# zsc/MOSS-TTSD

Hardware: AMD Instinct MI355X
Metric: audio codec tokens/sec/node (decode, bf16, batch 32 @ 4k ctx) (higher is better)
Workload: dtype bf16; 1 GPU; configs[2]: batch 32 synthetic dialogues/GPU, 4k-token KV context, top-k/top-p sampling on 8 channels, decode steps at full context; batch_per_gpu=32, context=4096, prompt=512, layers=28, hidden=2048, parallelism=dp1 (batch shard, no per-step collective)

## Files before the change

include/mtts.h:

```cpp
#ifndef MTTS_H
#define MTTS_H

#include <stdint.h>

#ifdef __cplusplus
extern "C" {
#endif

#define MTTS_OK 0
#define MTTS_EINVAL (-1)
#define MTTS_EHIP (-2)
#define MTTS_ENOMEM (-3)
#define MTTS_ESTATE (-4)

#define MTTS_CHANNELS 8

typedef struct MttsConfig {
    int32_t vocab_size;
    int32_t hidden_size;
    int32_t intermediate_size;
    int32_t num_hidden_layers;
    int32_t num_attention_heads;
    int32_t num_key_value_heads;
    int32_t head_dim;
    int32_t channels;
    int32_t speech_vocab_size;
    int32_t speech_pad_token;
    int32_t speech_range_lo;
    int32_t speech_range_hi;
    int32_t eos_token_id;
    int32_t max_position;
    float rms_norm_eps;
    int32_t max_batch;
    int32_t max_seq_len;
    int32_t kv_pool_pages;
    int32_t dtype;
} MttsConfig;
#define MTTS_DTYPE_BF16 0
#define MTTS_DTYPE_F32 1
#define MTTS_DTYPE_F16 2

typedef struct MttsSamplerCfg {
    int32_t do_sample;
    int32_t top_k;
    float top_p;
    float one_minus_top_p;
    float temperature;
    float repetition_penalty;
} MttsSamplerCfg;

typedef struct MttsEngine MttsEngine;

const char* mtts_last_error(void);
int32_t mtts_version(void);

int32_t mtts_engine_create(const MttsConfig* cfg, int32_t device, MttsEngine** out);
int32_t mtts_engine_destroy(MttsEngine* e);

int32_t mtts_bind_weight(MttsEngine* e, const char* name, const void* dev_bf16,
                         int64_t rows, int64_t cols, void* stream);
int32_t mtts_bind_rope(MttsEngine* e, const void* dev_cos_bf16, const void* dev_sin_bf16,
                       int32_t rows, void* stream);
int32_t mtts_weights_ready(MttsEngine* e);

int32_t mtts_generate(MttsEngine* e, const int64_t* host_input_ids, const uint8_t* host_attention_mask,
                      int32_t B, int32_t T, int32_t max_length,
                      const MttsSamplerCfg* sampler, uint64_t seed,
                      int64_t* host_out_ids, int32_t out_capacity, int32_t* out_len,
                      const int64_t* host_forced, int32_t forced_len, int64_t* host_decisions,
                      void* stream);

int32_t mtts_begin(MttsEngine* e, const int64_t* host_input_ids, const uint8_t* host_attention_mask,
                   int32_t B, int32_t T, int32_t max_length,
                   const MttsSamplerCfg* sampler, uint64_t seed, void* stream);
int32_t mtts_step(MttsEngine* e, int32_t n_steps, void* stream);
int32_t mtts_sync_state(MttsEngine* e, int32_t* steps_done, int32_t* all_finished, void* stream);
int32_t mtts_read_generated(MttsEngine* e, int64_t* host_gen, int32_t capacity_steps, int32_t* n_steps);
int32_t mtts_set_output_scores(MttsEngine* e, int32_t on);
int32_t mtts_read_scores(MttsEngine* e, float* host_lp, int32_t capacity_steps, int32_t* n_steps);
int32_t mtts_slot_read_scores(MttsEngine* e, int32_t slot, float* host_rows, int32_t capacity_steps, int32_t* n_steps);
int32_t mtts_read_logits(MttsEngine* e, uint16_t* host_logits0, uint16_t* host_logits17, void* stream);
int32_t mtts_read_logits_f32(MttsEngine* e, float* host_logits0, float* host_logits17, void* stream);
int32_t mtts_sched_open(MttsEngine* e, int32_t B, int32_t gen_cap, const MttsSamplerCfg* sampler, void* stream);
int32_t mtts_slot_submit(MttsEngine* e, int32_t slot, const int64_t* host_ids, int32_t T, int32_t max_length, uint64_t seed,
                         void* stream);
int32_t mtts_slot_submit_row(MttsEngine* e, int32_t slot, const int64_t* host_ids, int32_t T, int32_t max_length, uint64_t seed,
                             int32_t row_id, void* stream);
int32_t mtts_set_row_ids(MttsEngine* e, const int32_t* host_row_ids, int32_t n);
int32_t mtts_set_takes(MttsEngine* e, int32_t n);
int32_t mtts_slot_fork(MttsEngine* e, int32_t src_slot, int32_t dst_slot, uint64_t seed, int32_t row_id, void* stream);
int32_t mtts_slot_states(MttsEngine* e, int32_t* host_state, void* stream);
int32_t mtts_slot_read(MttsEngine* e, int32_t slot, int64_t* host_rows, int32_t capacity_steps, int32_t* n_steps);
int32_t mtts_read_seq_state(MttsEngine* e, int32_t* host_nas, int32_t* host_unfinished, int32_t* host_kv_len, void* stream);
int32_t mtts_slot_evict(MttsEngine* e, int32_t slot, void* stream);
int32_t mtts_kv_pool_state(MttsEngine* e, int32_t* total_pages, int32_t* free_pages, int32_t* max_pages_per_seq);
int32_t mtts_read_page_table(MttsEngine* e, int32_t* host_table, int32_t* host_n_pages);
int32_t mtts_set_forced_mode(MttsEngine* e, int32_t as_draw);
int32_t mtts_debug_read_device_page_table(MttsEngine* e, int32_t* host_table, void* stream);
int32_t mtts_export_codes(MttsEngine* e, int32_t first, int32_t n, int64_t* dev_codes, void* stream);
int32_t mtts_profile_enable(MttsEngine* e, int32_t on);
int32_t mtts_profile_read(MttsEngine* e, int32_t which, double* total_ms, int64_t* launches, int64_t* bytes);

int32_t mtts_debug_set_kv_len(MttsEngine* e, int32_t kv_len);
int32_t mtts_debug_kv_pack_stats(MttsEngine* e, int64_t* out6);
int32_t mtts_k_attn_bench(MttsEngine* e, int32_t phase, int32_t iters, float* avg_ms, int64_t* bytes_per_launch);
int32_t mtts_k_gemm_bench(int32_t N, int32_t K, int32_t epi, int32_t ksplit, int32_t waves, int32_t copies,
                          int32_t iters, float* avg_us);

int32_t mtts_k_gemm_bf16(const void* dev_w, const void* dev_x, void* dev_y,
                         int32_t M, int32_t N, int32_t K, int32_t ksplit, void* stream);
int64_t mtts_debug_gemm_depth_launches(void);
int32_t mtts_k_gemm_swiglu_bf16(const void* dev_w, const void* dev_x, void* dev_y,
                                int32_t M, int32_t N, int32_t K, void* stream);
int32_t mtts_k_rmsnorm(const void* dev_x, const void* dev_w, void* dev_y,
                       int32_t rows, int32_t n, float eps, void* stream);
int32_t mtts_k_rope_kvwrite(const void* dev_qkv, const int32_t* host_pos, const void* dev_qnorm, const void* dev_knorm,
                            const void* dev_cos, const void* dev_sin, int32_t R, int32_t nq, int32_t nkv, float eps,
                            void* dev_q, void* dev_k, void* dev_v, void* stream);
int32_t mtts_k_paged_attn_decode(const void* dev_q, const void* dev_k, const void* dev_v, const int32_t* host_lens,
                                 const int32_t* host_page_table, int32_t R, int32_t Lmax, int32_t nq, int32_t nkv,
                                 void* dev_out, void* stream);
int32_t mtts_k_kv_seal(const void* dev_pages, int32_t npages, void* dev_sealed, int32_t as_k, void* stream);
int32_t mtts_k_sample(const void* dev_logits_bf16, int32_t rows, int32_t vocab,
                      const void* dev_history_bitmap, const MttsSamplerCfg* cfg,
                      int32_t mask_id, uint64_t seed, int32_t step, int32_t channel,
                      int32_t* dev_tokens, void* stream);
int32_t mtts_k_sample_scores(const void* dev_logits_bf16, int32_t rows, int32_t vocab,
                             const void* dev_history_bitmap, const MttsSamplerCfg* cfg,
                             int32_t mask_id, uint64_t seed, int32_t step, int32_t channel,
                             int32_t* dev_tokens, float* dev_logp, void* stream);

typedef struct MttsCodecConfig {
    int32_t nq, codebook_size, rvq_dim, quant_out_dim;
    int32_t adapter_layers, adapter_dim, adapter_heads, adapter_ffn, adapter_max_pos;
    int32_t up_stride;
    int32_t dec_layers, dec_dim, dec_heads, dec_ffn, dec_max_pos, mel_bins;
    int32_t voc_dim, voc_inter, voc_layers, n_fft, hop;
    int32_t mel_n_fft, mel_hop, mel_frames;
    int32_t enc_layers, enc_dim, enc_heads, enc_ffn, enc_max_pos;
    int32_t sem_adapter_layers, pre_rvq_layers, down_pool;
} MttsCodecConfig;

typedef struct MttsCodec MttsCodec;
const char* mtts_codec_last_error(void);
int32_t mtts_codec_create(const MttsCodecConfig* cfg, int32_t device, MttsCodec** out);
int32_t mtts_codec_destroy(MttsCodec* c);
int32_t mtts_codec_bind(MttsCodec* c, const char* role, const float* dev_f32, int64_t n, void* stream);
int32_t mtts_codec_detokenize(MttsCodec* c, const int64_t* dev_codes, const int32_t* host_lens, int32_t B, int32_t T,
                              float* dev_wav, void* stream);
int32_t mtts_codec_detokenize_async(MttsCodec* c, const int64_t* dev_codes, const int32_t* host_lens, int32_t B, int32_t T,
                                    float* dev_wav, void* stream);
int32_t mtts_codec_check(MttsCodec* c, void* stream);
int32_t mtts_codec_tokenize(MttsCodec* c, const float* dev_wav, const int32_t* host_lens, int32_t B, int32_t nsamp,
                            int64_t* dev_codes, int32_t* host_code_lens, void* stream);
int32_t mtts_k_gemm_f32(const float* dev_a, const float* dev_w, const float* dev_bias, float* dev_c,
                        int32_t M, int32_t N, int32_t K, int32_t act, void* stream);
int32_t mtts_k_gemm_planes_bench(int32_t M, int32_t N, int32_t K, int32_t flags, int32_t tile_code, int32_t iters,
                                 float* avg_us, int32_t* code_used);

#ifdef __cplusplus
}
#endif
#endif
```

moss-ttsd_amd/csrc/attn.hip:

```cpp
#include "launch.h"
#include <cstdlib>
#ifndef MTTS_PK_WAVES
#define MTTS_PK_WAVES 0
#endif
#if MTTS_PK_WAVES
#define PK_OCC(PK) __attribute__((amdgpu_waves_per_eu((PK) ? MTTS_PK_WAVES : 1, (PK) ? MTTS_PK_WAVES : 8)))
#else
#define PK_OCC(PK)
#endif

__device__ __forceinline__ uint32_t u4c(const u32x4_t& v, int c) { return c == 0 ? v.x : c == 1 ? v.y : c == 2 ? v.z : v.w; }
__device__ __forceinline__ void pk_unit(const u32x4_t* pk, int j, uint32_t w[4]) {
    const uint32_t L0 = u4c(pk[j >> 1], 2 * (j & 1)), L1 = u4c(pk[j >> 1], 2 * (j & 1) + 1);
    const uint32_t N = u4c(pk[8 + (j >> 2)], j & 3);
    const uint32_t lo = pk[12].x, hi = pk[12].y;
    const uint32_t HA = ((N & 0x08080808u) << 4) | __builtin_amdgcn_perm(hi, lo, N & 0x07070707u);
    const uint32_t HB = (N & 0x80808080u) | __builtin_amdgcn_perm(hi, lo, (N >> 4) & 0x07070707u);
    w[0] = __builtin_amdgcn_perm(HA, L0, 0x05010400u);
    w[1] = __builtin_amdgcn_perm(HA, L0, 0x07030602u);
    w[2] = __builtin_amdgcn_perm(HB, L1, 0x05010400u);
    w[3] = __builtin_amdgcn_perm(HB, L1, 0x07030602u);
}

__host__ __device__ constexpr int pk_order(int i) { return i == 0 ? 12 : (i - 1) % 3 == 0 ? 8 + (i - 1) / 3 : 2 * ((i - 1) / 3) + (i - 1) % 3 - 1; }
__device__ bool seal_encode(const u32x4_t (&v)[16], u32x4_t* __restrict__ pk, uint32_t spare, bool unfit) {
    unsigned long long b0 = 0ull, b1 = 0ull;
#pragma unroll
    for (int j = 0; j < 16; ++j)
#pragma unroll
        for (int c = 0; c < 4; ++c)
#pragma unroll
            for (int h = 0; h < 2; ++h) {
                const uint32_t e = (u4c(v[j], c) >> (8 + 16 * h)) & 0x7fu;
                if (e & 64u) b1 |= 1ull << (e & 63u);
                else b0 |= 1ull << e;
            }
    const int n0 = __popcll(b0), n = n0 + __popcll(b1);
    if (n > 8 || unfit) {
        pk[12 * 64] = u32x4_t{0u, 0u, spare, 1u};
        return false;
    }
    unsigned long long dict = 0ull;
    {
        unsigned long long t0 = b0, t1 = b1;
        for (int i = 0; i < n; ++i) {
            uint32_t e;
            if (t0) { e = __ffsll((long long)t0) - 1; t0 &= t0 - 1; }
            else { e = 64 + __ffsll((long long)t1) - 1; t1 &= t1 - 1; }
            dict |= (unsigned long long)e << (8 * i);
        }
    }
    auto code = [&](uint32_t half) -> uint32_t {
        const uint32_t e = (half >> 8) & 0x7fu;
        const uint32_t rank = (e & 64u) ? n0 + __popcll(b1 & ((1ull << (e & 63u)) - 1ull)) : __popcll(b0 & ((1ull << e) - 1ull));
        return ((half >> 12) & 8u) | rank;
    };
    uint32_t lowp[32], nib[16];
#pragma unroll
    for (int j = 0; j < 16; ++j) {
        uint32_t N = 0u;
#pragma unroll
        for (int g = 0; g < 2; ++g) {
            uint32_t L = 0u;
#pragma unroll
            for (int k = 0; k < 4; ++k) {
                const uint32_t half = (u4c(v[j], 2 * g + (k >> 1)) >> (16 * (k & 1))) & 0xffffu;
                L |= (half & 0xffu) << (8 * k);
                N |= code(half) << (8 * k + 4 * g);
            }
            lowp[2 * j + g] = L;
        }
        nib[j] = N;
    }
#pragma unroll
    for (int u = 0; u < 8; ++u) pk[u * 64] = u32x4_t{lowp[4 * u], lowp[4 * u + 1], lowp[4 * u + 2], lowp[4 * u + 3]};
#pragma unroll
    for (int u = 0; u < 4; ++u) pk[(8 + u) * 64] = u32x4_t{nib[4 * u], nib[4 * u + 1], nib[4 * u + 2], nib[4 * u + 3]};
    pk[12 * 64] = u32x4_t{(uint32_t)dict, (uint32_t)(dict >> 32), spare, 0u};
    return true;
}
__device__ bool seal_lane(const u32x4_t* __restrict__ raw, u32x4_t* __restrict__ pk) {
    u32x4_t v[16];
#pragma unroll
    for (int j = 0; j < 16; ++j) v[j] = raw[j * 64];
    return seal_encode(v, pk, 0u, false);
}
__device__ bool seal_lane_k(const u32x4_t* __restrict__ raw, u32x4_t* __restrict__ pk, uint8_t* __restrict__ lds, int lane) {
    u32x4_t v[16];
#pragma unroll
    for (int j = 0; j < 16; ++j) v[j] = raw[j * 64];
    __builtin_amdgcn_wave_barrier();
    uint32_t* row = (uint32_t*)(lds + lane * 128);
#pragma unroll
    for (int j = 0; j < 16; ++j)
#pragma unroll
        for (int c = 0; c < 4; c += 2) {
            const uint32_t a = u4c(v[j], c), b = u4c(v[j], c + 1);
            row[2 * j + (c >> 1)] = ((a >> 7) & 0xffu) | (((a >> 23) & 0xffu) << 8) | (((b >> 7) & 0xffu) << 16) | (((b >> 23) & 0xffu) << 24);
        }
    __builtin_amdgcn_wave_barrier();
    uint32_t a0 = 0u, a1 = 0u, n0 = 0u, n1 = 0u;
    for (int t = 0; t < 64; ++t) {
        const uint32_t e = *(const uint16_t*)(lds + t * 128 + 2 * lane);
        a0 += e & 0xffu; n0 += (e & 0xffu) ? 1u : 0u;
        a1 += e >> 8; n1 += (e >> 8) ? 1u : 0u;
    }
    const int s0 = n0 ? min(max((int)((a0 + n0 / 2) / n0) - 125, -127), 127) : 0;
    const int s1 = n1 ? min(max((int)((a1 + n1 / 2) / n1) - 125, -127), 127) : 0;
    int8_t* sv = (int8_t*)(lds + 8192);
    sv[2 * lane] = (int8_t)s0;
    sv[2 * lane + 1] = (int8_t)s1;
    __builtin_amdgcn_wave_barrier();
    bool unfit = false;
#pragma unroll
    for (int j = 0; j < 16; ++j) {
        uint32_t w[4] = {v[j].x, v[j].y, v[j].z, v[j].w};
#pragma unroll
        for (int c = 0; c < 4; ++c) {
            const uint32_t sh = *(const uint16_t*)(sv + 8 * j + 2 * c);
            uint32_t out = 0u;
#pragma unroll
            for (int h = 0; h < 2; ++h) {
                uint32_t b = (w[c] >> (16 * h)) & 0xffffu;
                const int sft = (int)(int8_t)((sh >> (8 * h)) & 0xffu);
                const int e = (int)((b >> 7) & 0xffu);
                if (e == 0) {
                    if ((b & 0x7fu) && sft) unfit = true;
                } else {
                    const int e2 = e - sft;
                    if (e == 255 ? sft != 0 : (e2 < 1 || e2 > 254)) unfit = true;
                    else b = (b - ((uint32_t)sft << 7)) & 0xffffu;
                }
                out |= b << (16 * h);
            }
            w[c] = out;
        }
        v[j] = u32x4_t{w[0], w[1], w[2], w[3]};
    }
    return seal_encode(v, pk, ((uint32_t)s0 & 0xffu) | (((uint32_t)s1 & 0xffu) << 8), unfit);
}
__device__ bool seal_lane_v(const u32x4_t* __restrict__ raw, u32x4_t* __restrict__ pk, uint8_t* __restrict__ lds, int lane) {
    u32x4_t v[16];
#pragma unroll
    for (int j = 0; j < 16; ++j) v[j] = raw[j * 64];
    const int sub = lane >> 5;
    __builtin_amdgcn_wave_barrier();
    uint32_t* row = (uint32_t*)(lds + lane * 128);
#pragma unroll
    for (int it = 0; it < 16; ++it)
#pragma unroll
        for (int h = 0; h < 2; ++h) {
            uint32_t sum = 0u, cnt = 0u;
#pragma unroll
// ... 442 lines not shown
    if (pre_v) fuse_reduce_request(f, r, (nq + nkv + kvh) * MTTS_HD, lane, vta, vtb);
    if (pg < npages) load_page();
    if (own_wave) {
        float a, b;
        if (pre_v) fuse_reduce_sum(f, vta, vtb, a, b);
        else fuse_reduce(f, r, (nq + nkv + kvh) * MTTS_HD, lane, a, b);
        vnew[lane] = f2bf(a);
        vnew[lane + 64] = f2bf(b);
        const int page = page_table[(size_t)m.seq * max_pages + own_pg];
        const int tok = m.pos & 63;
        uint16_t* dst = (uint16_t*)vcache + ((size_t)kvh * total_pages + page) * (MTTS_PAGE * MTTS_HD) + (size_t)(tok >> 1) * (MTTS_HD * 2) + (tok & 1);
        dst[2 * lane] = f2bf(a);
        dst[2 * (lane + 64)] = f2bf(b);
    }
    float M[G], S[G];
#pragma unroll
    for (int g = 0; g < G; ++g) {
        const float* st = stats + ((size_t)r * nq + kvh * G + g) * max_pages * 2;
        float mx = -INFINITY;
        if (SF) mx = fmaxf(mx, s0[g].x);
        for (int p = lane + (SF ? 64 : 0); p < npages; p += 64) mx = fmaxf(mx, st[2 * p]);
        mx = wave_max(mx);
        float sm = 0.f;
        if (SF && lane < npages) sm += s0[g].y * expf(s0[g].x - mx);
        for (int p = lane + (SF ? 64 : 0); p < npages; p += 64) sm += st[2 * p + 1] * expf(st[2 * p] - mx);
        sm = wave_sum(sm);
        M[g] = mx;
        S[g] = sm;
    }
    float acc[G][4];
#pragma unroll
    for (int g = 0; g < G; ++g)
#pragma unroll
        for (int i = 0; i < 4; ++i) acc[g][i] = 0.f;
#pragma unroll 1
    for (int pp = 0; pp < ATT_PB / PV_WAVES; ++pp, ++pg) {
        if (pg >= npages) break;
        if (pp > 0) load_page();
        if (own_wave && pg == own_pg) {
            __builtin_amdgcn_wave_barrier();
            const int tp = (m.pos & 63) >> 1;
            if (sub == (tp & 1)) {
                const uint32_t w01 = ((const uint32_t*)vnew)[2 * dl], w23 = ((const uint32_t*)vnew)[2 * dl + 1];
                const uint32_t nv[4] = {w01 & 0xffffu, w01 >> 16, w23 & 0xffffu, w23 >> 16};
                const bool hi = m.pos & 1;
#pragma unroll
                for (int it = 0; it < 16; ++it)
                    if (it == (tp >> 1)) {
                        vv[it].x = hi ? (vv[it].x & 0xffffu) | (nv[0] << 16) : (vv[it].x & 0xffff0000u) | nv[0];
                        vv[it].y = hi ? (vv[it].y & 0xffffu) | (nv[1] << 16) : (vv[it].y & 0xffff0000u) | nv[1];
                        vv[it].z = hi ? (vv[it].z & 0xffffu) | (nv[2] << 16) : (vv[it].z & 0xffff0000u) | nv[2];
                        vv[it].w = hi ? (vv[it].w & 0xffffu) | (nv[3] << 16) : (vv[it].w & 0xffff0000u) | nv[3];
                    }
            }
        }
        uint16_t pun[G];
        bool pok = true;
        {
            const int tok = pg * MTTS_PAGE + lane;
            const int sv = (PK && packed) ? (int)(vv[12].z & 0xffu) : 0;
#pragma unroll
            for (int g = 0; g < G; ++g) {
                float p = 0.f;
                if (tok < len) {
                    float s = bf2f(SF ? sraw[g] : scores[((size_t)r * nq + kvh * G + g) * Lmax + tok]);
                    p = expf(s - M[g]) / S[g];
                }
                uint32_t pb = f2bf(p);
                pun[g] = (uint16_t)pb;
                if (sv && (pb & 0x7fffu)) {
                    if (((pb >> 7) & 0xffu) == 0u) pok = false;
                    else pb += (uint32_t)sv << 7;
                }
                pbuf[wave][g][lane] = (uint16_t)pb;
            }
        }
        __builtin_amdgcn_wave_barrier();
        if (PK && packed && __any(vv[12].w != 0u || !pok)) {
            packed = false;
#pragma unroll
            for (int it = 0; it < 16; ++it) vv[it] = __builtin_nontemporal_load(vp + it * 64);
#pragma unroll
            for (int g = 0; g < G; ++g) pbuf[wave][g][lane] = pun[g];
            __builtin_amdgcn_wave_barrier();
        }
        if (PK && packed) {
#pragma unroll
            for (int it = 0; it < 16; ++it) {
                uint32_t w[4];
                pk_unit(vv, it, w);
#pragma unroll
                for (int g = 0; g < G; ++g) {
                    const uint32_t pp2 = ((const uint32_t*)&pbuf[wave][g][0])[it * 2 + sub];
                    acc[g][0] = dot2bf(w[0], pp2, acc[g][0]);
                    acc[g][1] = dot2bf(w[1], pp2, acc[g][1]);
                    acc[g][2] = dot2bf(w[2], pp2, acc[g][2]);
                    acc[g][3] = dot2bf(w[3], pp2, acc[g][3]);
                }
            }
        } else {
#pragma unroll
            for (int it = 0; it < 16; ++it) {
#pragma unroll
                for (int g = 0; g < G; ++g) {
                    const uint32_t pp2 = ((const uint32_t*)&pbuf[wave][g][0])[it * 2 + sub];
                    acc[g][0] = dot2bf(vv[it].x, pp2, acc[g][0]);
                    acc[g][1] = dot2bf(vv[it].y, pp2, acc[g][1]);
                    acc[g][2] = dot2bf(vv[it].z, pp2, acc[g][2]);
                    acc[g][3] = dot2bf(vv[it].w, pp2, acc[g][3]);
                }
            }
        }
        __builtin_amdgcn_wave_barrier();
    }
#pragma unroll
    for (int g = 0; g < G; ++g)
#pragma unroll
        for (int i = 0; i < 4; ++i) {
            float v = acc[g][i];
            v = add_xor32(v);
            if (sub == 0) red[wave][g][dl * 4 + i] = v;
        }
    __syncthreads();
    for (int i = threadIdx.x; i < G * MTTS_HD; i += PV_WAVES * 64) {
        int g = i / MTTS_HD, d = i % MTTS_HD;
        float v = red[0][g][d];
#pragma unroll
        for (int w = 1; w < PV_WAVES; ++w) v += red[w][g][d];
        opart[(((size_t)r * nq + kvh * G + g) * nchunks_max + chunk) * MTTS_HD + d] = v;
    }
}

__global__ __launch_bounds__(512) void attn_combine_kernel(const float* __restrict__ opart, const RowMeta* __restrict__ meta,
                                                           uint16_t* __restrict__ out_packed, int nchunks_max, int nq,
                                                           int pages_per_chunk) {
    const int r = blockIdx.x, h = blockIdx.y * 4 + (threadIdx.x >> 7), d = threadIdx.x & 127;
    if (h >= nq) return;
    const RowMeta m = meta[r];
    float s = 0.f;
    const int npages = m.seq >= 0 ? (m.pos + 1 + MTTS_PAGE - 1) / MTTS_PAGE : 0;
    const int nch = (npages + pages_per_chunk - 1) / pages_per_chunk;
    const float* p = opart + ((size_t)r * nq + h) * nchunks_max * MTTS_HD + d;
    for (int c0 = 0; c0 < nch; c0 += 8) {
        float t[8];
#pragma unroll
        for (int j = 0; j < 8; ++j) t[j] = p[(size_t)min(c0 + j, nch - 1) * MTTS_HD];
#pragma unroll
        for (int j = 0; j < 8; ++j)
            if (c0 + j < nch) s += t[j];
    }
    out_packed[xpack_off(r, h * MTTS_HD + d, nq * MTTS_HD)] = f2bf(s);
}


template <int G>
__global__ __launch_bounds__(256) void attn_prefill_scores_kernel(
    const uint16_t* __restrict__ qbuf, const u32x4_t* __restrict__ kcache, const int32_t* __restrict__ page_table,
    const RowMeta* __restrict__ meta, uint16_t* __restrict__ scores, float* __restrict__ stats, int max_pages,
    int total_pages, int nq, int nkv, float scale) {
    const int tile = blockIdx.z, kvh = blockIdx.y;
    const int wave = threadIdx.x >> 6, lane = threadIdx.x & 63;
    const int row = tile * MTTS_MAXR + (lane & 31);
    const RowMeta m0 = meta[tile * MTTS_MAXR];
    if (m0.seq < 0) return;
    const RowMeta mr = meta[row];
    const int pos = mr.seq >= 0 ? mr.pos : -1;
    int maxpos = pos;
#pragma unroll
    for (int o = 16; o > 0; o >>= 1) maxpos = max(maxpos, __shfl_xor(maxpos, o, 64));
    const int npages = (maxpos + 1 + MTTS_PAGE - 1) / MTTS_PAGE;
    const int pg = blockIdx.x * 4 + wave;
    if (pg >= npages) return;
    const int page = page_table[(size_t)m0.seq * max_pages + pg];
    const u32x4_t* kp = kcache + ((size_t)kvh * total_pages + page) * (MTTS_PAGE * MTTS_HD / 8);
    u32x4_t ka[2][8];
#pragma unroll
    for (int th = 0; th < 2; ++th)
#pragma unroll
        for (int ks = 0; ks < 8; ++ks) ka[th][ks] = kp[(2 * ks + (lane >> 5)) * 64 + th * 32 + (lane & 31)];
    const int Lmax = max_pages * MTTS_PAGE;
#pragma unroll 1
    for (int g = 0; g < G; ++g) {
        const int h = kvh * G + g;
        const u32x4_t* qp = (const u32x4_t*)(qbuf + ((size_t)row * nq + h) * MTTS_HD);
        u32x4_t qb[8];
#pragma unroll
        for (int ks = 0; ks < 8; ++ks) qb[ks] = qp[2 * ks + (lane >> 5)];
        float mx = -INFINITY;
        f32x16_t acc[2];
#pragma unroll
        for (int th = 0; th < 2; ++th) {
#pragma unroll
            for (int i = 0; i < 16; ++i) acc[th][i] = 0.f;
#pragma unroll
            for (int ks = 0; ks < 8; ++ks)
                acc[th] = __builtin_amdgcn_mfma_f32_32x32x16_bf16(*(bf16x8_t*)&ka[th][ks], *(bf16x8_t*)&qb[ks], acc[th], 0, 0, 0);
#pragma unroll
            for (int i = 0; i < 16; ++i) {
                const int tok = pg * MTTS_PAGE + th * 32 + (i & 3) + 8 * (i >> 2) + 4 * (lane >> 5);
                const float sc = rbf(rbf(acc[th][i]) * scale);
                const bool valid = tok <= pos;
                if (valid) scores[((size_t)row * nq + h) * Lmax + tok] = f2bf(sc);
                acc[th][i] = valid ? sc : -INFINITY;
                mx = fmaxf(mx, acc[th][i]);
            }
        }
        mx = max_xor32(mx);
        float sm = 0.f;
#pragma unroll
        for (int th = 0; th < 2; ++th)
#pragma unroll
            for (int i = 0; i < 16; ++i) sm += (acc[th][i] > -INFINITY) ? expf(acc[th][i] - mx) : 0.f;
        sm = add_xor32(sm);
        if (lane < 32 && mr.seq >= 0) {
            float* st = stats + (((size_t)row * nq + h) * max_pages + pg) * 2;
            st[0] = mx;
            st[1] = sm;
        }
    }
}

template <int G>
__global__ __launch_bounds__(256) void attn_prefill_pv_kernel(
    const uint16_t* __restrict__ scores, const float* __restrict__ stats, const uint32_t* __restrict__ vcache,
    const int32_t* __restrict__ page_table, const RowMeta* __restrict__ meta, float* __restrict__ opart,
    int max_pages, int total_pages, int nchunks_pf, int nq, int nkv) {
    constexpr int GP = G > 2 ? 2 : G;
    const int tile = blockIdx.z, kvh = blockIdx.y;
    const int wave = threadIdx.x >> 6, lane = threadIdx.x & 63, half = lane >> 5;
    const int chunk = blockIdx.x * 4 + wave;
    const int row = tile * MTTS_MAXR + (lane & 31);
    const RowMeta m0 = meta[tile * MTTS_MAXR];
    if (m0.seq < 0) return;
    const RowMeta mr = meta[row];
    const int pos = mr.seq >= 0 ? mr.pos : -1;
    int maxpos = pos;
#pragma unroll
    for (int o = 16; o > 0; o >>= 1) maxpos = max(maxpos, __shfl_xor(maxpos, o, 64));
    const int npages = (maxpos + 1 + MTTS_PAGE - 1) / MTTS_PAGE;
    if (chunk * ATT_PF >= npages) return;
    const int rpages = (pos + 1 + MTTS_PAGE - 1) / MTTS_PAGE;
    const int Lmax = max_pages * MTTS_PAGE;
    const int pg_end = min(npages, (chunk + 1) * ATT_PF);
#pragma unroll 1
    for (int g0 = 0; g0 < G; g0 += GP) {
        float M[GP], S[GP];
#pragma unroll
        for (int g = 0; g < GP; ++g) {
            const float* st = stats + ((size_t)row * nq + kvh * G + g0 + g) * max_pages * 2;
            float mx = -INFINITY;
            for (int p = half; p < rpages; p += 8) {
                float t[4];
#pragma unroll
                for (int j = 0; j < 4; ++j) t[j] = st[2 * min(p + 2 * j, rpages - 1)];
#pragma unroll
                for (int j = 0; j < 4; ++j) mx = fmaxf(mx, t[j]);
            }
            mx = max_xor32(mx);
            float sm = 0.f;
            for (int p = half; p < rpages; p += 8) {
                float2 t[4];
#pragma unroll
                for (int j = 0; j < 4; ++j) t[j] = *(const float2*)(st + 2 * min(p + 2 * j, rpages - 1));
#pragma unroll
                for (int j = 0; j < 4; ++j)
                    if (p + 2 * j < rpages) sm += t[j].y * expf(t[j].x - mx);
            }
            sm = add_xor32(sm);
            M[g] = mx;
            S[g] = sm;
        }
        f32x16_t acc[GP][4];
#pragma unroll
        for (int g = 0; g < GP; ++g)
#pragma unroll
            for (int db = 0; db < 4; ++db)
#pragma unroll
                for (int i = 0; i < 16; ++i) acc[g][db][i] = 0.f;
#pragma unroll 1
        for (int pg = chunk * ATT_PF; pg < pg_end; ++pg) {
            const int page = page_table[(size_t)m0.seq * max_pages + pg];
            const uint32_t* vp = vcache + ((size_t)kvh * total_pages + page) * (MTTS_PAGE * MTTS_HD / 2) + (lane & 31);
            u32x4_t sv[4][GP];
#pragma unroll
            for (int ts = 0; ts < 4; ++ts) {
                const int tok0 = pg * MTTS_PAGE + ts * 16 + 8 * half;
#pragma unroll
                for (int g = 0; g < GP; ++g) {
                    sv[ts][g] = u32x4_t{0u, 0u, 0u, 0u};
                    if (tok0 <= pos) sv[ts][g] = *(const u32x4_t*)(scores + ((size_t)row * nq + kvh * G + g0 + g) * Lmax + tok0);
                }
            }
#pragma unroll
            for (int ts = 0; ts < 4; ++ts) {
                const int t0 = ts * 16 + 8 * half;
                u32x4_t va[4];
#pragma unroll
                for (int db = 0; db < 4; ++db) {
                    const uint32_t* q = vp + db * 32 + (size_t)(t0 / 2) * MTTS_HD;
                    va[db].x = q[0];
                    va[db].y = q[MTTS_HD];
                    va[db].z = q[2 * MTTS_HD];
                    va[db].w = q[3 * MTTS_HD];
                }
                const int tok0 = pg * MTTS_PAGE + t0;
#pragma unroll
                for (int g = 0; g < GP; ++g) {
                    const uint32_t sw[4] = {sv[ts][g].x, sv[ts][g].y, sv[ts][g].z, sv[ts][g].w};
                    uint32_t pw[4];
#pragma unroll
                    for (int j = 0; j < 4; ++j) {
                        const float p0 = (tok0 + 2 * j <= pos) ? expf(bflo(sw[j]) - M[g]) / S[g] : 0.f;
                        const float p1 = (tok0 + 2 * j + 1 <= pos) ? expf(bfhi(sw[j]) - M[g]) / S[g] : 0.f;
                        pw[j] = pack2(p0, p1);
                    }
                    u32x4_t pb = {pw[0], pw[1], pw[2], pw[3]};
#pragma unroll
                    for (int db = 0; db < 4; ++db)
                        acc[g][db] = __builtin_amdgcn_mfma_f32_32x32x16_bf16(*(bf16x8_t*)&va[db], *(bf16x8_t*)&pb, acc[g][db], 0, 0, 0);
                }
            }
        }
        if (mr.seq >= 0) {
#pragma unroll
            for (int g = 0; g < GP; ++g) {
                float* o = opart + (((size_t)row * nq + kvh * G + g0 + g) * nchunks_pf + chunk) * MTTS_HD + 4 * half;
#pragma unroll
                for (int db = 0; db < 4; ++db)
#pragma unroll
                    for (int q = 0; q < 4; ++q) {
                        const float4 v4 = make_float4(acc[g][db][4 * q], acc[g][db][4 * q + 1], acc[g][db][4 * q + 2], acc[g][db][4 * q + 3]);
                        *(float4*)(o + db * 32 + 8 * q) = v4;
                    }
            }
        }
    }
}

static bool pv_stats_first() {
    static int v = -1;
    if (v < 0) {
        const char* g = getenv("MTTS_PV_STATS_FIRST");
        v = (g && atoi(g) == 0) ? 0 : 1;
    }
    return v != 0;
}
template <int G>
static void launch_attn_g(const void* qbuf, void* kcache, void* vcache, const int32_t* page_table,
                          const RowMeta* meta, void* scores, float* stats, float* opart, void* out_packed, int R,
                          int pages_bound, int max_pages, int total_pages, int nchunks_max, int nq, int nkv, float scale,
                          const QkvFuse* fuse, AttnPhase phase, hipStream_t st, const KvPack* pack) {
    if (phase == ATTN_PF_SCORES) {
        dim3 ga((pages_bound + 3) / 4, nkv, R / MTTS_MAXR);
        hipLaunchKernelGGL((attn_prefill_scores_kernel<G>), ga, dim3(256), 0, st, (const uint16_t*)qbuf, (const u32x4_t*)kcache,
                           page_table, meta, (uint16_t*)scores, stats, max_pages, total_pages, nq, nkv, scale);
        return;
    }
    const int nchunks_pf = (max_pages + ATT_PF - 1) / ATT_PF;
    if (phase == ATTN_PF_PV) {
        dim3 gb((pages_bound + 4 * ATT_PF - 1) / (4 * ATT_PF), nkv, R / MTTS_MAXR);
        hipLaunchKernelGGL((attn_prefill_pv_kernel<G>), gb, dim3(256), 0, st, (const uint16_t*)scores, (const float*)stats,
                           (const uint32_t*)vcache, page_table, meta, opart, max_pages, total_pages, nchunks_pf, nq, nkv);
        return;
    }
    if (phase == ATTN_PF_COMBINE) {
        hipLaunchKernelGGL(attn_combine_kernel, dim3(R, (nq + 3) / 4), dim3(512), 0, st, (const float*)opart, meta,
                           (uint16_t*)out_packed, nchunks_pf, nq, ATT_PF);
        return;
    }
    const QkvFuse f = fuse ? *fuse : QkvFuse{nullptr, 0, 0, nullptr, nullptr, nullptr, nullptr, 0.f};
    const u32x4_t* kpk = pack ? (const u32x4_t*)pack->k : nullptr;
    const u32x4_t* vpk = pack ? (const u32x4_t*)pack->v : nullptr;
#define MTTS_SC(FU, PK)                                                                                                  \
    hipLaunchKernelGGL((attn_scores_kernel<G, FU, PK>), ga, dim3(256), 0, st, (const uint16_t*)qbuf, (u32x4_t*)kcache, \
                       page_table, meta, (uint16_t*)scores, stats, max_pages, total_pages, nq, nkv, scale, f, kpk)
#define MTTS_PV2(FU, PK, SF)                                                                                                        \
    hipLaunchKernelGGL((attn_pv_kernel<G, FU, PK, SF>), gb, dim3(PV_WAVES * 64), 0, st, (const uint16_t*)scores, (const float*)stats, \
                       (u32x4_t*)vcache, page_table, meta, opart, max_pages, total_pages, nchunks_max, nq, nkv, f, vpk)
#define MTTS_PV(FU, PK)                        \
    do {                                       \
        if (pv_stats_first()) MTTS_PV2(FU, PK, true); \
        else MTTS_PV2(FU, PK, false);          \
    } while (0)
    if (phase == ATTN_ALL || phase == ATTN_SCORES) {
        dim3 ga((pages_bound + 3) / 4, nkv, R);
        if (fuse) { if (kpk) MTTS_SC(true, true); else MTTS_SC(true, false); }
        else { if (kpk) MTTS_SC(false, true); else MTTS_SC(false, false); }
    }
    if (phase == ATTN_ALL || phase == ATTN_PV) {
        dim3 gb((pages_bound + ATT_PB - 1) / ATT_PB, nkv, R);
        if (fuse) { if (vpk) MTTS_PV(true, true); else MTTS_PV(true, false); }
        else { if (vpk) MTTS_PV(false, true); else MTTS_PV(false, false); }
    }
#undef MTTS_SC
#undef MTTS_PV
#undef MTTS_PV2
    if (phase == ATTN_ALL || phase == ATTN_COMBINE)
        hipLaunchKernelGGL(attn_combine_kernel, dim3(R, (nq + 3) / 4), dim3(512), 0, st, (const float*)opart, meta,
                           (uint16_t*)out_packed, nchunks_max, nq, ATT_PB);
}

int launch_attn(const void* qbuf, void* kcache, void* vcache, const int32_t* page_table,
                const RowMeta* meta, void* scores, float* stats, float* opart, void* out_packed, int R,
                int pages_bound, int max_pages, int total_pages, int nchunks_max, int nq, int nkv, float scale,
                const QkvFuse* fuse, AttnPhase phase, hipStream_t st, const KvPack* pack) {
    int G = nq / nkv;
#define MTTS_ATT(GG)                                                                                              \
    launch_attn_g<GG>(qbuf, kcache, vcache, page_table, meta, scores, stats, opart, out_packed, R, pages_bound,   \
                      max_pages, total_pages, nchunks_max, nq, nkv, scale, fuse, phase, st, pack)
    if (G == 1) MTTS_ATT(1);
    else if (G == 2) MTTS_ATT(2);
    else if (G == 4) MTTS_ATT(4);
    else return -1;
#undef MTTS_ATT
    return 0;
}
```

moss-ttsd_amd/csrc/engine.h:

```cpp
#pragma once
#include <hip/hip_runtime.h>

#include <algorithm>
#include <cstdarg>
#include <cstdio>
#include <cstdlib>
#include <cstring>
#include <memory>
#include <string>
#include <vector>

#include "launch.h"

#define MTTS_LOCAL __attribute__((visibility("hidden")))
extern MTTS_LOCAL thread_local char g_err[512];
MTTS_LOCAL int fail(int code, const char* fmt, ...) __attribute__((format(printf, 2, 3)));
#define HIPCHK(x)                                                                          \
    do {                                                                                   \
        hipError_t _e = (x);                                                               \
        if (_e != hipSuccess) return fail(MTTS_EHIP, "%s: %s (%s:%d)", #x, hipGetErrorString(_e), __FILE__, __LINE__); \
    } while (0)
#define TRY(x)             \
    do {                   \
        int _r = (x);      \
// ... 19 lines not shown
    std::vector<Buf> bufs;
    std::string free_error;
    DevBufs() = default;
    DevBufs(const DevBufs&) = delete;
    DevBufs& operator=(const DevBufs&) = delete;
    ~DevBufs() { free_all(); }
    template <typename T>
    int get(T** out, size_t n, bool zero = true) {
        TRY(dalloc(out, n, zero));
        bufs.push_back({(void*)*out, false});
        return 0;
    }
    template <typename T>
    int get_pinned(T** out, size_t n) {
        HIPCHK(hipHostMalloc((void**)out, n * sizeof(T)));
        bufs.push_back({(void*)*out, true});
        memset((void*)*out, 0, n * sizeof(T));
        return 0;
    }
    template <typename T>
    void release(T*& p) {
        if (!p) return;
        auto it = std::find_if(bufs.begin(), bufs.end(), [&](const Buf& b) { return b.p == (void*)p; });
        if (it == bufs.end()) note(hipErrorInvalidValue, (void*)p);
        else { free_one(*it); bufs.erase(it); }
        p = nullptr;
    }
    void free_all() {
        for (const Buf& b : bufs) free_one(b);
        bufs.clear();
    }
private:
    void free_one(const Buf& b) {
        const hipError_t r = b.pinned ? hipHostFree(b.p) : hipFree(b.p);
        if (r != hipSuccess) note(r, b.p);
    }
    void note(hipError_t r, void* p) {
        if (!free_error.empty()) return;
        char msg[160];
        snprintf(msg, sizeof(msg), "freeing %p: %s", p, hipGetErrorString(r));
        free_error = msg;
    }
};

static inline int full_cap_for(int vocab) { int p = 1; while (p < vocab) p <<= 1; return vocab > SAMP_CAND ? p : 0; }
static inline int alloc_scratch(DevBufs& m, SampleScratch& sc, int rows, int vocab) {
    const int fc = full_cap_for(vocab);
    TRY(m.get(&sc.overflow, (size_t)rows));
    if (fc) {
        TRY(m.get(&sc.full_val, (size_t)rows * fc, false));
        TRY(m.get(&sc.full_idx, (size_t)rows * fc, false));
        TRY(m.get(&sc.nuc_cnt, (size_t)rows * 2048));
        TRY(m.get(&sc.nuc_mass, (size_t)rows * 2048));
    }
    TRY(m.get(&sc.hist, (size_t)rows * 2048));
    TRY(m.get(&sc.slice_val, (size_t)rows * SAMP_NS));
    TRY(m.get(&sc.slice_idx, (size_t)rows * SAMP_NS));
    TRY(m.get(&sc.cand_val, (size_t)rows * SAMP_CAND));
    TRY(m.get(&sc.cand_idx, (size_t)rows * SAMP_CAND));
    TRY(m.get(&sc.cand_n, (size_t)rows));
    return 0;
}
static inline int alloc_lp_scratch(DevBufs& m, SampleScratch& sc, int rows) {
    if (sc.lp) return 0;
    TRY(m.get(&sc.slice_sum, (size_t)rows * SAMP_NS));
    TRY(m.get(&sc.lp, (size_t)rows * 8));
    return 0;
}

struct Layer {
    void *wqkv = nullptr, *wo = nullptr, *wgu = nullptr, *wd = nullptr;
    void *ln_in = nullptr, *ln_post = nullptr, *qn = nullptr, *kn = nullptr;
    int bound = 0;
};

enum { PROF_SCORES = 0, PROF_PV = 1, PROF_GEMM = 2, PROF_STEP = 3, PROF_N = 4 };

struct MttsEngine {
    DevBufs mem;
    MttsConfig cfg;
    int device = 0;
    int H, I, L, nq, nkv, V0, Vs, Vs_pad, V0_pad, qkv_rows;
    std::vector<Layer> layers;
    void* emb[8] = {nullptr};
    void* head0 = nullptr;
    void* heads17 = nullptr;
    void* final_norm = nullptr;
    uint16_t *rope_cos = nullptr, *rope_sin = nullptr;
    int rope_rows = 0;
    int emb_bound = 0, norm_bound = 0;
    const uint16_t** d_tables = nullptr;
    GemmPlan p_qkv, p_o, p_gu, p_d, p_h0, p_h17;
    float* partial = nullptr;
    float* partial2 = nullptr;
    void *x2 = nullptr, *act_rm = nullptr;
    int small_rows = SMALL_RP;
    int gemm_depth = 1;
    void *x = nullptr, *xn = nullptr, *attn_p = nullptr, *act_p = nullptr, *qbuf = nullptr, *hlast = nullptr, *xh = nullptr;
    void *logits0 = nullptr, *logits17 = nullptr, *join_logits0 = nullptr, *join_logits17 = nullptr;
    void* scores = nullptr;
    float *stats = nullptr, *opart = nullptr;
    void *kcache = nullptr, *vcache = nullptr;
    size_t layer_stride = 0;
    int total_pages = 0, max_pages = 0, nchunks_max = 0;
    int32_t* d_page_table = nullptr;
    std::vector<int32_t> h_page_table;
    std::vector<int32_t> free_pages;
    std::vector<int32_t> n_pages;
    std::vector<int32_t> page_owners;
    std::vector<char> slot_live;
    PageEdits pending_edits;
    int forced_draw = 0;
    std::vector<int32_t> next_row_ids;
    int next_takes = 1;
    int takes = 1;
    bool f32 = false;
    int h16 = 0;
    struct LayerF32 { float *wqkv = nullptr, *wo = nullptr, *wgu = nullptr, *wd = nullptr, *ln_in = nullptr, *ln_post = nullptr, *qn = nullptr, *kn = nullptr; };
    std::vector<LayerF32> lf;
    float* embf[8] = {nullptr};
    const float** d_tables_f = nullptr;
    float *final_norm_f = nullptr, *rope_cos_f = nullptr, *rope_sin_f = nullptr;
    float *kcache_f = nullptr, *vcache_f = nullptr;
    float *xf = nullptr, *xnf = nullptr, *qkvf = nullptr, *qbuf_f = nullptr, *attnf = nullptr, *yf = nullptr, *guf = nullptr,
          *actf = nullptr, *hlast_f = nullptr, *scores_f = nullptr;
    SeqState* d_seqs = nullptr;
    RowMeta* d_meta = nullptr;
    LoopState* d_ls = nullptr;
    LoopState* h_ls = nullptr;
    SeqState* h_seqs = nullptr;
    int32_t *d_decisions = nullptr, *d_cur = nullptr, *d_gen = nullptr, *d_declog = nullptr, *d_forced = nullptr,
            *d_tf = nullptr;
    uint32_t* d_bitmaps = nullptr;
    int bm_words = 0;
    MttsSamplerCfg* d_scfg = nullptr;
    SampleScratch sscr;
    int ch0_sampled = 0;
    float* d_lp = nullptr;
    int lp_cap = 0;
    int scores_next = 0;
    int scores_on = 0;
    bool run_open = false;
    int32_t* d_pf_tokens = nullptr;
    RowMeta* d_pf_meta = nullptr;
    size_t pf_cap_rows = 0;
    int gen_cap = 0;
    int B = 0, T = 0, base_length = 0, max_length = 0, max_steps = 0, steps_issued = 0;
    bool continuous = false;
    std::vector<int> join_step;
    std::vector<int> n_real;
    int max_real = 0;
    uint64_t seed = 0;
    bool began = false, has_forced = false;
    struct StepGraph { int B, pages, forced, ch0, scores; hipGraphExec_t exec; };
    std::vector<StepGraph> graphs;
    hipStream_t cap_stream = nullptr;
    bool use_graphs = true;
    int kv_pack = 1;
    void *kpack = nullptr, *vpack = nullptr;
    size_t pk_layer_stride = 0;
    unsigned long long *d_seal_cnt = nullptr, *h_seal_cnt = nullptr;
    std::vector<char> pack_k_on, pack_v_on;
    int pack_min_work = 512;
    int fuse_qkv_max = 2560;
    int pf_mfma_pages = 0;
    bool prof = false;
    std::vector<std::pair<hipEvent_t, hipEvent_t>> ev[PROF_N];
    int64_t prof_bytes[PROF_N] = {0, 0, 0, 0};
};

static inline KvPack layer_pack(MttsEngine* e, int n, int pages_bound) {
    KvPack pk{nullptr, nullptr};
    if (e->B * pages_bound < e->pack_min_work) return pk;
    if (e->kpack && e->pack_k_on[n]) pk.k = (uint8_t*)e->kpack + e->pk_layer_stride * n;
    if (e->vpack && e->pack_v_on[n]) pk.v = (uint8_t*)e->vpack + e->pk_layer_stride * n;
    return pk;
}
```

moss-ttsd_amd/csrc/engine.hip:

```cpp
#include "engine.h"

#define FLUSH_STEPS 7
#define LINGER_STEPS 14
static inline int linger_bound(int B) { return 6 * B + 8; }

thread_local char g_err[512] = "";
int fail(int code, const char* fmt, ...) {
    va_list ap;
    va_start(ap, fmt);
    vsnprintf(g_err, sizeof(g_err), fmt, ap);
    va_end(ap);
    return code;
}

const char* mtts_last_error(void) { return g_err; }
int32_t mtts_version(void) { return 202; }

static void pool_reset(MttsEngine* e) {
    e->free_pages.resize(e->total_pages);
    for (int i = 0; i < e->total_pages; ++i) e->free_pages[i] = e->total_pages - 1 - i;
    if (const char* g = getenv("MTTS_PAGE_SHUFFLE")) {
        uint64_t x = 0x9E3779B97F4A7C15ull ^ (uint64_t)atoll(g);
        for (int i = e->total_pages - 1; i > 0; --i) {
            x = x * 6364136223846793005ull + 1442695040888963407ull;
// ... 3 lines not shown
    std::fill(e->n_pages.begin(), e->n_pages.end(), 0);
    e->page_owners.assign(e->total_pages, 0);
    e->pending_edits.n = 0;
}
static int pool_flush(MttsEngine* e, hipStream_t st) {
    if (e->pending_edits.n) {
        launch_set_pages(e->d_page_table, e->pending_edits, st);
        e->pending_edits.n = 0;
        HIPCHK(hipGetLastError());
    }
    return 0;
}
static int pool_append(MttsEngine* e, int b, int page, hipStream_t st) {
    const int at = b * e->max_pages + e->n_pages[b]++;
    e->h_page_table[at] = page;
    for (int i = 0; i < e->pending_edits.n; ++i)
        if (e->pending_edits.idx[i] == at) { e->pending_edits.val[i] = page; return 0; }
    if (e->pending_edits.n == 31) TRY(pool_flush(e, st));
    e->pending_edits.idx[e->pending_edits.n] = at;
    e->pending_edits.val[e->pending_edits.n++] = page;
    return 0;
}
static int pool_grow(MttsEngine* e, int b, int need, hipStream_t st) {
    if (need > e->max_pages) return fail(MTTS_ENOMEM, "slot %d needs %d KV pages, a sequence holds at most %d (max_seq_len %d)", b, need, e->max_pages, e->cfg.max_seq_len);
    while (e->n_pages[b] < need) {
        if (e->free_pages.empty()) return fail(MTTS_ENOMEM, "KV page pool exhausted (%d pages of %d tokens): slot %d needs page %d", e->total_pages, MTTS_PAGE, b, e->n_pages[b]);
        const int page = e->free_pages.back();
        e->free_pages.pop_back();
        e->page_owners[page] = 1;
        TRY(pool_append(e, b, page, st));
    }
    return 0;
}
static int pool_share(MttsEngine* e, int src, int dst, int npages, hipStream_t st) {
    for (int i = 0; i < npages; ++i) {
        const int page = e->h_page_table[(size_t)src * e->max_pages + i];
        e->page_owners[page]++;
        TRY(pool_append(e, dst, page, st));
    }
    return 0;
}
static void pool_release(MttsEngine* e, int b) {
    for (int i = e->n_pages[b] - 1; i >= 0; --i) {
        const int page = e->h_page_table[(size_t)b * e->max_pages + i];
        if (--e->page_owners[page] == 0) e->free_pages.push_back(page);
    }
    e->n_pages[b] = 0;
    int k = 0;
    for (int i = 0; i < e->pending_edits.n; ++i)
        if (e->pending_edits.idx[i] / e->max_pages != b) {
            e->pending_edits.idx[k] = e->pending_edits.idx[i];
            e->pending_edits.val[k++] = e->pending_edits.val[i];
        }
    e->pending_edits.n = k;
}

static int create_f32(MttsEngine* e) {
    const size_t H = e->H, I = e->I, D = MTTS_HD;
    e->lf.resize(e->L);
    for (auto& l : e->lf) {
        TRY(e->mem.get(&l.wqkv, (size_t)e->qkv_rows * H, false));
        TRY(e->mem.get(&l.wo, H * e->nq * D, false));
        TRY(e->mem.get(&l.wgu, 2 * I * H, false));
        TRY(e->mem.get(&l.wd, H * I, false));
        TRY(e->mem.get(&l.ln_in, H)); TRY(e->mem.get(&l.ln_post, H)); TRY(e->mem.get(&l.qn, D)); TRY(e->mem.get(&l.kn, D));
    }
    TRY(e->mem.get(&e->embf[0], (size_t)e->V0 * H, false));
    for (int ch = 1; ch < 8; ++ch) TRY(e->mem.get(&e->embf[ch], (size_t)e->Vs * H, false));
    TRY(e->mem.get(&e->final_norm_f, H));
    TRY(e->mem.get(&e->d_tables_f, 8));
    HIPCHK(hipMemcpy((void*)e->d_tables_f, e->embf, 8 * sizeof(void*), hipMemcpyHostToDevice));
    const size_t P = MTTS_PF32CAP;
    TRY(e->mem.get(&e->xf, P * H)); TRY(e->mem.get(&e->xnf, P * H)); TRY(e->mem.get(&e->yf, P * H));
    TRY(e->mem.get(&e->qkvf, P * e->qkv_rows)); TRY(e->mem.get(&e->qbuf_f, P * e->nq * D)); TRY(e->mem.get(&e->attnf, P * e->nq * D));
    TRY(e->mem.get(&e->guf, P * 2 * I)); TRY(e->mem.get(&e->actf, P * I));
    TRY(e->mem.get(&e->hlast_f, (size_t)MTTS_RCAP * H));
    TRY(e->mem.get((float**)&e->logits0, (size_t)MTTS_RCAP * e->V0_pad));
    TRY(e->mem.get((float**)&e->logits17, (size_t)MTTS_RCAP * 7 * e->Vs_pad));
    return 0;
}

static int forward_rows_f32(MttsEngine* e, const int32_t* d_tokens, const RowMeta* d_meta, int R, int heads, hipStream_t st) {
    const int H = e->H, I = e->I, nq = e->nq, nkv = e->nkv;
    const float eps = e->cfg.rms_norm_eps, scale = 1.0f / sqrtf((float)MTTS_HD);
    const int Lmax = e->max_pages * MTTS_PAGE, h16 = e->h16;
    const bool dec = heads == 1;
    launch_f32_embed_norm(d_tokens, d_meta, e->d_tables_f, e->lf[0].ln_in, e->xf, e->xnf, R, H, eps, h16, st);
    for (int n = 0; n < e->L; ++n) {
        auto& l = e->lf[n];
        float* kc = e->kcache_f + e->layer_stride * n;
        float* vc = e->vcache_f + e->layer_stride * n;
        launch_f32_linear(l.wqkv, e->xnf, e->qkvf, R, e->qkv_rows, H, e->qkv_rows, h16, dec, st);
        launch_f32_qkv_post(e->qkvf, e->qkv_rows, d_meta, l.qn, l.kn, e->rope_cos_f, e->rope_sin_f, e->qbuf_f, kc, vc,
                            e->d_page_table, e->max_pages, e->total_pages, R, nq, nkv, eps, h16, st);
        launch_f32_attn(e->qbuf_f, kc, vc, e->d_page_table, d_meta, e->scores_f, e->attnf, R, e->max_pages, e->total_pages, nq,
                        nkv, scale, Lmax, h16, st);
        launch_f32_linear(l.wo, e->attnf, e->yf, R, H, nq * MTTS_HD, H, h16, dec, st);
        launch_f32_resid_norm(e->yf, e->xf, l.ln_post, e->xnf, nullptr, d_meta, R, H, eps, h16, st);
        launch_f32_linear(l.wgu, e->xnf, e->guf, R, 2 * I, H, 2 * I, h16, dec, st);
        launch_f32_swiglu(e->guf, e->actf, R, I, h16, st);
        launch_f32_linear(l.wd, e->actf, e->yf, R, H, I, H, h16, dec, st);
        const bool lastl = n == e->L - 1;
        launch_f32_resid_norm(e->yf, e->xf, lastl ? e->final_norm_f : e->lf[n + 1].ln_in, e->xnf, lastl ? e->hlast_f : nullptr,
                              d_meta, R, H, eps, h16, st);
    }
    if (heads) {
        const float* xin = heads == 1 ? e->xnf : e->hlast_f;
        launch_f32_linear(e->embf[0], xin, (float*)e->logits0, e->B, e->V0, H, e->V0_pad, h16, true, st);
        for (int c = 1; c < 8; ++c)
            launch_f32_linear(e->embf[c], xin, (float*)e->logits17 + (size_t)(c - 1) * e->Vs_pad, e->B, e->Vs, H, 7 * e->Vs_pad, h16, true, st);
    }
    HIPCHK(hipGetLastError());
    return MTTS_OK;
}

static void drop_graphs(MttsEngine* e) {
    for (auto& g : e->graphs) hipGraphExecDestroy(g.exec);
    e->graphs.clear();
}

int32_t mtts_engine_create(const MttsConfig* c, int32_t device, MttsEngine** out) {
    if (!c || !out) return fail(MTTS_EINVAL, "null argument");
    if (c->head_dim != MTTS_HD) return fail(MTTS_EINVAL, "head_dim must be 128 (got %d)", c->head_dim);
    if (c->channels != 8) return fail(MTTS_EINVAL, "channels must be 8");
    if (c->hidden_size % 16 || c->intermediate_size % 16) return fail(MTTS_EINVAL, "hidden/intermediate must be multiples of 16");
    if (c->hidden_size > 8192) return fail(MTTS_EINVAL, "hidden_size > 8192 not built (resid_norm keeps a row in registers)");
    if (c->num_attention_heads % c->num_key_value_heads) return fail(MTTS_EINVAL, "bad GQA ratio");
    int G = c->num_attention_heads / c->num_key_value_heads;
    if (G != 1 && G != 2 && G != 4) return fail(MTTS_EINVAL, "GQA group %d not built (1,2,4)", G);
    if (c->max_batch < 1 || c->max_batch > MTTS_RCAP) return fail(MTTS_EINVAL, "max_batch must be 1..128");
    if (c->vocab_size <= 152694 || c->speech_vocab_size <= 1024)
        return fail(MTTS_EINVAL, "vocab too small for the reference's hard-coded mask ids 152694 / 1024");
    if (c->dtype != MTTS_DTYPE_BF16 && c->dtype != MTTS_DTYPE_F32 && c->dtype != MTTS_DTYPE_F16)
        return fail(MTTS_EINVAL, "dtype %d not built (bf16 = 0, fp32 = 1, fp16 = 2)", c->dtype);
    if (c->kv_pool_pages < 0) return fail(MTTS_EINVAL, "kv_pool_pages must be >= 0");
    HIPCHK(hipSetDevice(device));
    struct Destroy {
        void operator()(MttsEngine* p) const {
            const std::string keep = g_err;
            mtts_engine_destroy(p);
            snprintf(g_err, sizeof(g_err), "%s", keep.c_str());
        }
    };
    std::unique_ptr<MttsEngine, Destroy> holder(new MttsEngine());
    MttsEngine* e = holder.get();
    DevBufs& m = e->mem;
    e->cfg = *c;
    e->device = device;
    if (const char* g = getenv("MTTS_GRAPHS")) e->use_graphs = atoi(g) != 0;
    if (const char* g = getenv("MTTS_FUSE_QKV_MAX")) e->fuse_qkv_max = atoi(g);
    if (const char* g = getenv("MTTS_KV_PACK")) e->kv_pack = atoi(g);
    if (const char* g = getenv("MTTS_KV_PACK_MIN")) e->pack_min_work = atoi(g);
    if (const char* g = getenv("MTTS_PREFILL_MFMA_PAGES")) e->pf_mfma_pages = atoi(g);
    if (const char* g = getenv("MTTS_SMALL_ROWS")) e->small_rows = std::min(std::max(atoi(g), 0), SMALL_RP);
    e->gemm_depth = gemm_depth_env();
    e->H = c->hidden_size; e->I = c->intermediate_size; e->L = c->num_hidden_layers;
    e->nq = c->num_attention_heads; e->nkv = c->num_key_value_heads;
    e->V0 = c->vocab_size; e->Vs = c->speech_vocab_size;
    e->V0_pad = round_up(e->V0, 32); e->Vs_pad = round_up(e->Vs, 32);
    e->qkv_rows = (e->nq + 2 * e->nkv) * MTTS_HD;
    e->layers.resize(e->L);
    const int H = e->H, I = e->I;
    e->f32 = c->dtype != MTTS_DTYPE_BF16;
    e->h16 = c->dtype == MTTS_DTYPE_F16;
    if (e->f32) TRY(create_f32(e));
    if (!e->f32) {
        for (auto& l : e->layers) {
            TRY(m.get((uint16_t**)&l.wqkv, (size_t)e->qkv_rows * H));
            TRY(m.get((uint16_t**)&l.wo, (size_t)H * e->nq * MTTS_HD));
            TRY(m.get((uint16_t**)&l.wgu, (size_t)2 * I * H));
            TRY(m.get((uint16_t**)&l.wd, (size_t)round_up(H, 32) * I));
            TRY(m.get((uint16_t**)&l.ln_in, (size_t)H));
            TRY(m.get((uint16_t**)&l.ln_post, (size_t)H));
            TRY(m.get((uint16_t**)&l.qn, (size_t)MTTS_HD));
            TRY(m.get((uint16_t**)&l.kn, (size_t)MTTS_HD));
        }
        TRY(m.get((uint16_t**)&e->emb[0], (size_t)e->V0 * H, false));
        for (int ch = 1; ch < 8; ++ch) TRY(m.get((uint16_t**)&e->emb[ch], (size_t)e->Vs * H, false));
        TRY(m.get((uint16_t**)&e->head0, (size_t)e->V0_pad * H));
        TRY(m.get((uint16_t**)&e->heads17, (size_t)7 * e->Vs_pad * H));
        TRY(m.get((uint16_t**)&e->final_norm, (size_t)H));
        TRY(m.get(&e->d_tables, 8));
        HIPCHK(hipMemcpy((void*)e->d_tables, e->emb, 8 * sizeof(void*), hipMemcpyHostToDevice));
    }
    e->p_qkv = mtts_plan_gemm(e->qkv_rows, H, 0);
    e->p_o = mtts_plan_gemm(round_up(H, 32), e->nq * MTTS_HD, 0);
    e->p_gu = mtts_plan_gemm(2 * I, H, 1);
    e->p_d = mtts_plan_gemm(round_up(H, 32), I, 0);
    e->p_h0 = mtts_plan_gemm(e->V0_pad, H, 1);
    e->p_h17 = mtts_plan_gemm(7 * e->Vs_pad, H, 1);
    for (GemmPlan* p : {&e->p_qkv, &e->p_o, &e->p_gu, &e->p_d, &e->p_h0, &e->p_h17}) p->depth = e->gemm_depth;
    size_t pmax = (size_t)8 * std::max(e->qkv_rows, round_up(H, 32));
    if (!e->f32) {
        TRY(m.get(&e->partial, pmax * MTTS_PFCAP));
        TRY(m.get(&e->partial2, (size_t)8 * round_up(H, 32) * MTTS_PFCAP));
        TRY(m.get((uint16_t**)&e->x2, (size_t)MTTS_MAXR * H));
        TRY(m.get((uint16_t**)&e->act_rm, (size_t)MTTS_MAXR * I));
        TRY(m.get((uint16_t**)&e->x, (size_t)MTTS_PFCAP * H));
        TRY(m.get((uint16_t**)&e->xn, (size_t)MTTS_PFCAP * H));
        TRY(m.get((uint16_t**)&e->xh, (size_t)MTTS_RCAP * H));
        TRY(m.get((uint16_t**)&e->hlast, (size_t)MTTS_RCAP * H));
        TRY(m.get((uint16_t**)&e->attn_p, (size_t)MTTS_PFCAP * e->nq * MTTS_HD));
        TRY(m.get((uint16_t**)&e->act_p, (size_t)MTTS_PFCAP * I));
        TRY(m.get((uint16_t**)&e->qbuf, (size_t)MTTS_PFCAP * e->nq * MTTS_HD));
        TRY(m.get((uint16_t**)&e->logits0, (size_t)MTTS_RCAP * e->V0_pad));
        TRY(m.get((uint16_t**)&e->logits17, (size_t)MTTS_RCAP * 7 * e->Vs_pad));
        TRY(m.get((uint16_t**)&e->join_logits0, (size_t)MTTS_MAXR * e->V0_pad));
        TRY(m.get((uint16_t**)&e->join_logits17, (size_t)MTTS_MAXR * 7 * e->Vs_pad));
    }
    e->max_pages = (c->max_seq_len + MTTS_PAGE - 1) / MTTS_PAGE + 1;
    e->total_pages = c->kv_pool_pages > 0 ? c->kv_pool_pages : e->max_pages * c->max_batch;
    e->nchunks_max = (e->max_pages + ATT_PB - 1) / ATT_PB;
    e->layer_stride = (size_t)e->total_pages * e->nkv * MTTS_PAGE * MTTS_HD;
    if (e->f32) {
        TRY(m.get(&e->kcache_f, e->layer_stride * e->L));
        TRY(m.get(&e->vcache_f, e->layer_stride * e->L));
        TRY(m.get(&e->scores_f, (size_t)MTTS_PF32CAP * e->nq * e->max_pages * MTTS_PAGE, false));
    } else {
        TRY(m.get((uint16_t**)&e->kcache, e->layer_stride * e->L));
        TRY(m.get((uint16_t**)&e->vcache, e->layer_stride * e->L));
        if (e->kv_pack) {
            e->pk_layer_stride = (size_t)e->total_pages * e->nkv * MTTS_PKU * 64 * 16;
            size_t free_b = 0, total_b = 0;
            const size_t need = 2 * e->pk_layer_stride * e->L;
            if (hipMemGetInfo(&free_b, &total_b) != hipSuccess || need + ((size_t)8 << 30) > free_b) {
                fprintf(stderr, "mtts: sealed KV pages off: %.1f GB needed, %.1f GB free (8 GB kept for the run)\n", need / 1e9, free_b / 1e9);
                e->kv_pack = 0;
            }
        }
        if (e->kv_pack) {
            TRY(m.get((uint8_t**)&e->kpack, e->pk_layer_stride * e->L));
            TRY(m.get((uint8_t**)&e->vpack, e->pk_layer_stride * e->L));
            TRY(m.get(&e->d_seal_cnt, (size_t)e->L * 4));
            TRY(m.get_pinned(&e->h_seal_cnt, (size_t)e->L * 4));
            e->pack_k_on.assign(e->L, 1);
            e->pack_v_on.assign(e->L, 1);
        }
    }
    TRY(m.get(&e->d_page_table, (size_t)c->max_batch * e->max_pages));
    e->h_page_table.assign((size_t)c->max_batch * e->max_pages, 0);
    e->n_pages.assign(c->max_batch, 0);
    e->slot_live.assign(c->max_batch, 0);
    e->pending_edits.n = 0;
    pool_reset(e);
    if (!e->f32) {
        TRY(m.get((uint16_t**)&e->scores, (size_t)MTTS_PFCAP * e->nq * e->max_pages * MTTS_PAGE));
        TRY(m.get(&e->stats, (size_t)MTTS_PFCAP * e->nq * e->max_pages * 2));
        TRY(m.get(&e->opart, (size_t)MTTS_PFCAP * e->nq * ((e->max_pages + ATT_PF - 1) / ATT_PF) * MTTS_HD));
    }
    TRY(m.get(&e->d_seqs, MTTS_RCAP));
    TRY(m.get(&e->d_meta, MTTS_RCAP));
    TRY(m.get(&e->d_ls, 1));
    TRY(m.get_pinned(&e->h_ls, 1));
    TRY(m.get_pinned(&e->h_seqs, MTTS_RCAP));
    TRY(m.get(&e->d_decisions, MTTS_RCAP * 8));
    TRY(m.get(&e->d_cur, MTTS_RCAP * 8));
    TRY(m.get(&e->d_tf, MTTS_RCAP * 7 * 8));
    e->bm_words = (e->V0 + 31) / 32;
    TRY(m.get(&e->d_bitmaps, (size_t)MTTS_RCAP * 8 * e->bm_words));
    TRY(m.get(&e->d_scfg, 8));
    TRY(alloc_scratch(m, e->sscr, c->max_batch, e->V0));
    *out = holder.release();
    return MTTS_OK;
}

int32_t mtts_engine_destroy(MttsEngine* e) {
    if (!e) return MTTS_OK;
    hipSetDevice(e->device);
    hipDeviceSynchronize();
    drop_graphs(e);
    if (e->cap_stream) hipStreamDestroy(e->cap_stream);
    for (int w = 0; w < PROF_N; ++w) for (auto& pr : e->ev[w]) { hipEventDestroy(pr.first); hipEventDestroy(pr.second); }
    e->mem.free_all();
    const std::string err = e->mem.free_error;
    delete e;
    return err.empty() ? MTTS_OK : fail(MTTS_EHIP, "mtts_engine_destroy: %s", err.c_str());
}

struct WeightSlot {
    int64_t rows = 0, cols = 0;
    void* copy_to = nullptr;
    void* pack_to = nullptr;
    int rows_pad = 0, row_mul = 1, row_off = 0;
    float* f32_to = nullptr;
    int64_t f32_row = 0;
    int* bound = nullptr;
    int bit = 0;
};

static int resolve_weight(MttsEngine* e, const char* name_c, WeightSlot& w) {
    const std::string name(name_c);
    const int64_t H = e->H, I = e->I, D = MTTS_HD, Hp = round_up(e->H, 32), QD = e->nq * D, KD = e->nkv * D;
    int ch = -1;
    if (sscanf(name_c, "model.embedding_list.%d.weight", &ch) == 1 && name.size() > 7 && name.compare(name.size() - 7, 7, ".weight") == 0) {
        if (ch < 0 || ch > 7) return fail(MTTS_EINVAL, "bad channel in %s", name_c);
        w.rows = ch == 0 ? e->V0 : e->Vs; w.cols = H;
        w.copy_to = e->emb[ch]; w.f32_to = e->embf[ch];
        w.pack_to = ch == 0 ? e->head0 : e->heads17;
        w.rows_pad = ch == 0 ? e->V0_pad : 7 * e->Vs_pad;
        w.row_off = ch == 0 ? 0 : (ch - 1) * e->Vs_pad;
        w.bound = &e->emb_bound; w.bit = 1 << ch;
        return MTTS_OK;
    }
    if (name == "model.language_model.norm.weight") {
        w.rows = H; w.cols = 1; w.copy_to = e->final_norm; w.f32_to = e->final_norm_f; w.bound = &e->norm_bound; w.bit = 1;
        return MTTS_OK;
    }
    if (name.find("lm_heads.") == 0 || name == "model.language_model.embed_tokens.weight") return MTTS_OK;
    int n = -1;
    char rest[128];
    if (sscanf(name_c, "model.language_model.layers.%d.%127s", &n, rest) != 2) return fail(MTTS_EINVAL, "unknown tensor %s", name_c);
    if (n < 0 || n >= e->L) return fail(MTTS_EINVAL, "layer index out of range in %s", name_c);
    Layer& l = e->layers[n];
    const MttsEngine::LayerF32 f = e->f32 ? e->lf[n] : MttsEngine::LayerF32{};
    const struct { const char* name; int64_t rows, cols; void* bf; float* f32; int rows_pad, row_mul, row_off; int64_t f32_row; } t[] = {
        {"input_layernorm.weight", H, 1, l.ln_in, f.ln_in, 0, 1, 0, 0},
        {"post_attention_layernorm.weight", H, 1, l.ln_post, f.ln_post, 0, 1, 0, 0},
        {"self_attn.q_norm.weight", D, 1, l.qn, f.qn, 0, 1, 0, 0},
        {"self_attn.k_norm.weight", D, 1, l.kn, f.kn, 0, 1, 0, 0},
        {"self_attn.q_proj.weight", QD, H, l.wqkv, f.wqkv, e->qkv_rows, 1, 0, 0},
        {"self_attn.k_proj.weight", KD, H, l.wqkv, f.wqkv, e->qkv_rows, 1, (int)QD, QD},
        {"self_attn.v_proj.weight", KD, H, l.wqkv, f.wqkv, e->qkv_rows, 1, (int)(QD + KD), QD + KD},
        {"self_attn.o_proj.weight", H, QD, l.wo, f.wo, (int)Hp, 1, 0, 0},
        {"mlp.gate_proj.weight", I, H, l.wgu, f.wgu, (int)(2 * I), 2, 0, 0},
        {"mlp.up_proj.weight", I, H, l.wgu, f.wgu, (int)(2 * I), 2, 1, I},
        {"mlp.down_proj.weight", H, I, l.wd, f.wd, (int)Hp, 1, 0, 0},
    };
    for (int i = 0; i < 11; ++i)
        if (!strcmp(rest, t[i].name)) {
            w.rows = t[i].rows; w.cols = t[i].cols;
            (t[i].cols == 1 ? w.copy_to : w.pack_to) = t[i].bf;
            w.rows_pad = t[i].rows_pad; w.row_mul = t[i].row_mul; w.row_off = t[i].row_off;
            w.f32_to = t[i].f32; w.f32_row = t[i].f32_row;
            w.bound = &l.bound; w.bit = 1 << i;
            return MTTS_OK;
        }
    return fail(MTTS_EINVAL, "unknown tensor %s", name_c);
}

int32_t mtts_bind_weight(MttsEngine* e, const char* name_c, const void* src, int64_t rows, int64_t cols, void* stream) {
    if (!e || !name_c || !src) return fail(MTTS_EINVAL, "null argument");
    HIPCHK(hipSetDevice(e->device));
    drop_graphs(e);
    hipStream_t st = S(stream);
    WeightSlot w;
    TRY(resolve_weight(e, name_c, w));
    if (!w.bound) return MTTS_OK;
    const bool shape_ok = w.cols == 1 ? (rows == w.rows && cols == 1) || (rows == 1 && cols == w.rows) : rows == w.rows && cols == w.cols;
    if (!shape_ok)
        return fail(MTTS_EINVAL, "%s: expected [%lld,%lld] got [%lld,%lld]", name_c, (long long)w.rows, (long long)w.cols, (long long)rows, (long long)cols);
    const size_t n = (size_t)w.rows * w.cols;
    if (e->f32) {
        HIPCHK(hipMemcpyAsync(w.f32_to + w.f32_row * w.cols, src, n * 4, hipMemcpyDeviceToDevice, st));
    } else {
        if (w.copy_to) HIPCHK(hipMemcpyAsync(w.copy_to, src, n * 2, hipMemcpyDeviceToDevice, st));
        if (w.pack_to) launch_pack_weight(src, w.pack_to, (int)w.rows, (int)w.cols, w.rows_pad, w.row_mul, w.row_off, st);
        HIPCHK(hipGetLastError());
    }
    *w.bound |= w.bit;
    return MTTS_OK;
}

template <typename T>
static int bind_rope_tables(MttsEngine* e, T*& c, T*& s, const void* cosb, const void* sinb, int rows, hipStream_t st) {
    e->mem.release(c);
    e->mem.release(s);
    TRY(e->mem.get(&c, (size_t)rows * 64, false));
    TRY(e->mem.get(&s, (size_t)rows * 64, false));
    HIPCHK(hipMemcpyAsync(c, cosb, (size_t)rows * 64 * sizeof(T), hipMemcpyDeviceToDevice, st));
    HIPCHK(hipMemcpyAsync(s, sinb, (size_t)rows * 64 * sizeof(T), hipMemcpyDeviceToDevice, st));
    e->rope_rows = rows;
    return MTTS_OK;
}
int32_t mtts_bind_rope(MttsEngine* e, const void* cosb, const void* sinb, int32_t rows, void* stream) {
    if (!e || !cosb || !sinb || rows < 1) return fail(MTTS_EINVAL, "bad rope table");
    HIPCHK(hipSetDevice(e->device));
    drop_graphs(e);
    if (e->f32) return bind_rope_tables(e, e->rope_cos_f, e->rope_sin_f, cosb, sinb, rows, S(stream));
    return bind_rope_tables(e, e->rope_cos, e->rope_sin, cosb, sinb, rows, S(stream));
}

int32_t mtts_weights_ready(MttsEngine* e) {
    if (!e) return fail(MTTS_EINVAL, "null engine");
    if (e->emb_bound != 0xff) return fail(MTTS_ESTATE, "embedding tables missing (mask %x)", e->emb_bound);
    if (!e->norm_bound) return fail(MTTS_ESTATE, "final norm missing");
    if (!e->rope_rows) return fail(MTTS_ESTATE, "rope table missing");
    for (int n = 0; n < e->L; ++n)
        if (e->layers[n].bound != 2047) return fail(MTTS_ESTATE, "layer %d incomplete (mask %x)", n, e->layers[n].bound);
    return MTTS_OK;
}

static void prof_begin(MttsEngine* e, int which, hipStream_t st, hipEvent_t* a) {
    if (!e->prof) return;
    hipEvent_t s0, s1;
    hipEventCreate(&s0); hipEventCreate(&s1);
    hipEventRecord(s0, st);
    e->ev[which].push_back({s0, s1});
    *a = s1;
}
static void prof_end(MttsEngine* e, hipStream_t st, hipEvent_t a) {
    if (!e->prof) return;
    hipEventRecord(a, st);
}

static int pack_policy_reset(MttsEngine* e, hipStream_t st) {
    if (!e->d_seal_cnt) return 0;
    HIPCHK(hipMemsetAsync(e->d_seal_cnt, 0, (size_t)e->L * 4 * sizeof(unsigned long long), st));
    bool changed = false;
    for (int n = 0; n < e->L; ++n) { changed |= !e->pack_k_on[n] || !e->pack_v_on[n]; e->pack_k_on[n] = 1; e->pack_v_on[n] = 1; }
    if (changed) drop_graphs(e);
    return 0;
}
static int attend_layer(MttsEngine* e, int n, const RowMeta* d_meta, int R, int pages_bound, int ks_qkv, int nphases, bool prefill,
                        bool fused, bool sealed, hipStream_t st, int64_t kv_tokens_hint) {
    static const AttnPhase decode_ph[3] = {ATTN_SCORES, ATTN_PV, ATTN_COMBINE}, prefill_ph[3] = {ATTN_PF_SCORES, ATTN_PF_PV, ATTN_PF_COMBINE};
    Layer& l = e->layers[n];
    const float eps = e->cfg.rms_norm_eps, scale = 1.0f / sqrtf((float)MTTS_HD);
    uint16_t* kc = (uint16_t*)e->kcache + e->layer_stride * n;
    uint16_t* vc = (uint16_t*)e->vcache + e->layer_stride * n;
    const QkvFuse fz{e->partial, ks_qkv, e->qkv_rows, (const uint16_t*)l.qn, (const uint16_t*)l.kn, e->rope_cos, e->rope_sin, eps};
    const KvPack pk = layer_pack(e, n, pages_bound);
    if (!fused)
        launch_qkv_post(e->partial, ks_qkv, e->qkv_rows, d_meta, l.qn, l.kn, e->rope_cos, e->rope_sin, e->qbuf,
                        kc, vc, e->d_page_table, e->max_pages, e->total_pages, R, e->nq, e->nkv, eps, st);
    for (int i = 0; i < nphases; ++i) {
        hipEvent_t ev = nullptr;
        if (i < 2) prof_begin(e, i == 0 ? PROF_SCORES : PROF_PV, st, &ev);
        if (launch_attn(e->qbuf, kc, vc, e->d_page_table, d_meta, e->scores, e->stats, e->opart, e->attn_p, R,
                        pages_bound, e->max_pages, e->total_pages, e->nchunks_max, e->nq, e->nkv, scale,
                        fused ? &fz : nullptr, (prefill ? prefill_ph : decode_ph)[i], st, (sealed && (pk.k || pk.v)) ? &pk : nullptr))
            return fail(MTTS_EINVAL, "attention group size not built");
        if (i < 2) prof_end(e, st, ev);
    }
    if (e->prof) {
        e->prof_bytes[PROF_SCORES] += kv_tokens_hint * e->nkv * MTTS_HD * 2;
        e->prof_bytes[PROF_PV] += kv_tokens_hint * e->nkv * MTTS_HD * 2;
    }
    return 0;
}
static bool small_path_fits(MttsEngine* e) {
    const int H = e->H;
    if (H > 8192 || H % 8 || e->I % 8) return false;
    const int lim = 64 * 1024 - 33 * 1024;
    return mtts_small_lds_bytes(e->p_qkv, H, PRO_NORM) <= lim && mtts_small_lds_bytes(e->p_d, e->I, PRO_ROWS) <= lim &&
           mtts_small_lds_bytes(e->p_o, e->nq * MTTS_HD, PRO_COMBINE) <= lim;
}
static int forward_small(MttsEngine* e, const RowMeta* d_meta, int pages_bound, hipStream_t st, int64_t kv_tokens_hint) {
    const int H = e->H, I = e->I, nq = e->nq, nkv = e->nkv, Hp = round_up(H, 32), R = MTTS_MAXR;
    const float eps = e->cfg.rms_norm_eps;
    uint16_t* xa = (uint16_t*)e->x;
    uint16_t* xb = (uint16_t*)e->x2;
    SmallPro base{};
    base.rows = e->B; base.eps = eps; base.slab_npad = Hp;
    for (int n = 0; n < e->L; ++n) {
        Layer& l = e->layers[n];
        SmallPro pq = base;
        pq.x_in = xa; pq.x_out = xb; pq.slabs = e->partial2; pq.ksplit = n ? e->p_d.ksplit : 0; pq.norm_w = (const uint16_t*)l.ln_in;
        launch_gemv_small(EPI_PARTIAL, PRO_NORM, e->p_qkv, l.wqkv, H, e->qkv_rows, e->qkv_rows, e->partial, nullptr, pq, st);
        TRY(attend_layer(e, n, d_meta, R, pages_bound, e->p_qkv.ksplit, 2, false, e->B * pages_bound <= e->fuse_qkv_max, true, st,
                         kv_tokens_hint));
        SmallPro po = base;
        po.opart = e->opart; po.meta = d_meta; po.nchunks_max = e->nchunks_max; po.nq = nq; po.pages_per_chunk = ATT_PB;
        launch_gemv_small(EPI_PARTIAL, PRO_COMBINE, e->p_o, l.wo, nq * MTTS_HD, Hp, Hp, e->partial2, nullptr, po, st);
        SmallPro pg = base;
        pg.x_in = xb; pg.x_out = xa; pg.slabs = e->partial2; pg.ksplit = e->p_o.ksplit; pg.norm_w = (const uint16_t*)l.ln_post;
        launch_gemv_small(EPI_SILU_RM, PRO_NORM, e->p_gu, l.wgu, H, 2 * I, 2 * I, nullptr, (uint16_t*)e->act_rm, pg, st);
        SmallPro pd = base;
        pd.xrows = (const uint16_t*)e->act_rm;
        launch_gemv_small(EPI_PARTIAL, PRO_ROWS, e->p_d, l.wd, I, Hp, Hp, e->partial2, nullptr, pd, st);
    }
    if (e->kpack)
        launch_kv_seal_rows(e->kcache, e->vcache, e->kpack, e->vpack, e->d_page_table, d_meta, R, e->max_pages, e->total_pages, nkv, e->L, e->d_seal_cnt, st);
    SmallPro ph = base;
    ph.x_in = xa; ph.x_out = nullptr; ph.slabs = e->partial2; ph.ksplit = e->p_d.ksplit; ph.norm_w = (const uint16_t*)e->final_norm;
    launch_gemv_small(EPI_BF16, PRO_NORM, e->p_h0, e->head0, H, e->V0_pad, e->V0, nullptr, (uint16_t*)e->logits0, ph, st);
    launch_gemv_small(EPI_BF16, PRO_NORM, e->p_h17, e->heads17, H, 7 * e->Vs_pad, 7 * e->Vs_pad, nullptr, (uint16_t*)e->logits17, ph, st);
    HIPCHK(hipGetLastError());
    return MTTS_OK;
}

static int forward_rows(MttsEngine* e, const int32_t* d_tokens, const RowMeta* d_meta, int R, int pages_bound,
                        int heads, hipStream_t st, int64_t kv_tokens_hint) {
    const int H = e->H, I = e->I, nq = e->nq, nkv = e->nkv;
    const float eps = e->cfg.rms_norm_eps;
    const int Hp = round_up(H, 32);
    const int mb = (R + 31) / 32;
    const bool tiled = heads != 1;
    if (e->f32) return forward_rows_f32(e, d_tokens, d_meta, heads == 1 ? e->B : R, heads, st);
    launch_embed_norm(d_tokens, d_meta, e->d_tables, e->layers[0].ln_in, e->x, e->xn, R, H, eps, st);
    if (heads == 1 && e->B <= e->small_rows && small_path_fits(e)) return forward_small(e, d_meta, pages_bound, st, kv_tokens_hint);
    for (int n = 0; n < e->L; ++n) {
        Layer& l = e->layers[n];
        const int ks_qkv = tiled ? mtts_tile_ksplit(e->qkv_rows, H, 1024) : e->p_qkv.ksplit;
        const int ks_o = tiled ? mtts_tile_ksplit(Hp, nq * MTTS_HD, 1024) : e->p_o.ksplit;
        const int ks_d = tiled ? mtts_tile_ksplit(Hp, I, 1024) : e->p_d.ksplit;
        if (tiled) launch_gemm_tile(EPI_PARTIAL, R, ks_qkv, l.wqkv, e->xn, H, e->qkv_rows, e->qkv_rows, e->partial, nullptr, st);
        else launch_gemm(EPI_PARTIAL, mb, e->p_qkv, l.wqkv, e->xn, H, e->qkv_rows, e->qkv_rows, e->partial, nullptr, st);
        TRY(attend_layer(e, n, d_meta, R, pages_bound, ks_qkv, 3, heads != 1 && pages_bound >= e->pf_mfma_pages,
                         heads == 1 && e->B * pages_bound <= e->fuse_qkv_max, heads == 1, st, kv_tokens_hint));
        if (tiled) launch_gemm_tile(EPI_PARTIAL, R, ks_o, l.wo, e->attn_p, nq * MTTS_HD, Hp, Hp, e->partial, nullptr, st);
        else launch_gemm(EPI_PARTIAL, mb, e->p_o, l.wo, e->attn_p, nq * MTTS_HD, Hp, Hp, e->partial, nullptr, st);
        launch_resid_norm(e->partial, ks_o, Hp, e->x, l.ln_post, e->xn, nullptr, d_meta, R, H, eps, st);
        if (tiled) {
            launch_gemm_tile(EPI_SILU, R, 1, l.wgu, e->xn, H, 2 * I, 2 * I, nullptr, (uint16_t*)e->act_p, st);
            launch_gemm_tile(EPI_PARTIAL, R, ks_d, l.wd, e->act_p, I, Hp, Hp, e->partial, nullptr, st);
        } else {
            launch_gemm(EPI_SILU, mb, e->p_gu, l.wgu, e->xn, H, 2 * I, 2 * I, nullptr, (uint16_t*)e->act_p, st);
            launch_gemm(EPI_PARTIAL, mb, e->p_d, l.wd, e->act_p, I, Hp, Hp, e->partial, nullptr, st);
        }
        const bool lastl = (n == e->L - 1);
        const void* nw = lastl ? e->final_norm : e->layers[n + 1].ln_in;
        launch_resid_norm(e->partial, ks_d, Hp, e->x, nw, e->xn, lastl ? e->hlast : nullptr, d_meta, R, H, eps, st);
    }
    if (e->kpack)
        launch_kv_seal_rows(e->kcache, e->vcache, e->kpack, e->vpack, e->d_page_table, d_meta, R, e->max_pages, e->total_pages, nkv, e->L, e->d_seal_cnt, st);
    if (heads) {
        const void* xin = e->xn;
        int hmb = mb;
        if (heads == 2) {
            hmb = (e->B + 31) / 32;
            launch_pack_rows(e->hlast, e->xh, e->B, H, hmb, st);
            xin = e->xh;
        }
        launch_gemm(EPI_BF16, hmb, e->p_h0, e->head0, xin, H, e->V0_pad, e->V0, nullptr, (uint16_t*)e->logits0, st);
        launch_gemm(EPI_BF16, hmb, e->p_h17, e->heads17, xin, H, 7 * e->Vs_pad, 7 * e->Vs_pad, nullptr, (uint16_t*)e->logits17, st);
    }
    HIPCHK(hipGetLastError());
    return MTTS_OK;
}

static int prefill_staged(MttsEngine* e, size_t Mpad, int pages_bound, int last_heads, hipStream_t st) {
    const size_t pfcap = e->f32 ? MTTS_PF32CAP : MTTS_PFCAP;
    for (size_t off = 0; off < Mpad; off += pfcap) {
        const int rows = (int)std::min<size_t>(pfcap, Mpad - off);
        TRY(forward_rows(e, e->d_pf_tokens + off * 8, e->d_pf_meta + off, rows, pages_bound, off + rows >= Mpad ? last_heads : 0, st, 0));
    }
    return 0;
}

static int ensure_gen_storage(MttsEngine* e, int steps) {
    if (steps <= e->gen_cap) return 0;
    e->mem.release(e->d_gen); e->mem.release(e->d_declog); e->mem.release(e->d_forced);
    drop_graphs(e);
    e->gen_cap = steps;
    const size_t n = (size_t)e->cfg.max_batch * steps * 8;
    TRY(e->mem.get(&e->d_gen, n));
    TRY(e->mem.get(&e->d_declog, n));
    TRY(e->mem.get(&e->d_forced, n, false));
    return 0;
}

static int start_scores(MttsEngine* e, hipStream_t st) {
    e->scores_on = e->scores_next;
    if (!e->scores_on) return 0;
    if (!e->sscr.lp) {
        drop_graphs(e);
        TRY(alloc_lp_scratch(e->mem, e->sscr, e->cfg.max_batch));
    }
    const size_t n = (size_t)e->cfg.max_batch * e->gen_cap * 8;
    if (!e->d_lp || e->lp_cap != e->gen_cap) {
        e->mem.release(e->d_lp);
        drop_graphs(e);
        TRY(e->mem.get(&e->d_lp, n, false));
        e->lp_cap = e->gen_cap;
    }
    HIPCHK(hipMemsetAsync(e->d_lp, 0xff, n * sizeof(float), st));
    return 0;
}

static int grow_prefill_staging(MttsEngine* e, size_t rows) {
    if (rows <= e->pf_cap_rows) return 0;
    e->mem.release(e->d_pf_tokens); e->mem.release(e->d_pf_meta);
    e->pf_cap_rows = 0;
    TRY(e->mem.get(&e->d_pf_tokens, rows * 8, false));
    TRY(e->mem.get(&e->d_pf_meta, rows, false));
    e->pf_cap_rows = rows;
    return 0;
}

static const SeqState IDLE_SEQ{-1, 0, 0, 0, 0, 0, 0, 0, 0};
static int reset_run_state(MttsEngine* e, const std::vector<SeqState>& seqs, bool continuous, const MttsSamplerCfg* sampler, hipStream_t st) {
    HIPCHK(hipMemcpyAsync(e->d_seqs, seqs.data(), seqs.size() * sizeof(SeqState), hipMemcpyHostToDevice, st));
    if (continuous) e->forced_draw = 0;
// ... 26 lines not shown
        arr(e->d_tf, (size_t)7 * 8 * 4, (size_t)7 * 8 * 4);
    }
    for (int i = 0; i < job.np; ++i)
        if (job.psrc[i] < 0 || job.psrc[i] >= e->total_pages || job.pdst[i] < 0 || job.pdst[i] >= e->total_pages)
            return fail(MTTS_EINVAL, "fork: page outside the pool");
    for (int i = 0; i < job.nr; ++i)
        if (job.rsrc[i] < 0 || job.rsrc[i] >= e->cfg.max_batch || job.rdst[i] < 0 || job.rdst[i] >= e->cfg.max_batch)
            return fail(MTTS_EINVAL, "fork: row outside the batch");
    const size_t blk = (size_t)MTTS_PAGE * MTTS_HD * (e->f32 ? 4 : 2), layer = e->layer_stride * (e->f32 ? 4 : 2);
    void* kc = e->f32 ? (void*)e->kcache_f : e->kcache;
    void* vc = e->f32 ? (void*)e->vcache_f : e->vcache;
    launch_fork(kc, vc, layer, (size_t)e->total_pages * blk, (int)blk, e->L, e->nkv, job, st);
    HIPCHK(hipGetLastError());
    return 0;
}

static int begin_run(MttsEngine* e, const int64_t* ids, const uint8_t* mask, int32_t B, int32_t T, int32_t max_length,
                     const MttsSamplerCfg* sampler, uint64_t seed, int takes, void* stream) {
    if (!e || !ids || !mask || !sampler) return fail(MTTS_EINVAL, "null argument");
    TRY(mtts_weights_ready(e));
    HIPCHK(hipSetDevice(e->device));
    hipStream_t st = S(stream);
    const int R = B * takes;
    if (B < 1 || B > e->cfg.max_batch || R > e->cfg.max_batch) return fail(MTTS_EINVAL, "batch %d x %d takes exceeds max_batch %d", B, takes, e->cfg.max_batch);
    if (T < 8) return fail(MTTS_EINVAL, "T must be >= 8 (delay pattern adds 7 slots)");
    const int base = T - 7;
    if (max_length <= base) return fail(MTTS_EINVAL, "max_length %d leaves no room to generate (prompt slots %d)", max_length, base);
    int max_steps = max_length - base + LINGER_STEPS;
    e->B = R; e->T = T; e->base_length = base; e->max_length = max_length; e->takes = takes;
    e->seed = seed; e->steps_issued = 0; e->has_forced = false;
    e->n_real.assign(R, 0);
    e->max_real = 0;
    std::vector<int> pad(B, 0);
    for (int b = 0; b < B; ++b) {
        int p = 0;
        while (p < base && !mask[(size_t)b * T + p]) ++p;
        for (int t = p; t < base; ++t)
            if (!mask[(size_t)b * T + t]) return fail(MTTS_EINVAL, "attention_mask of row %d is not left-padded", b);
        if (p >= base) return fail(MTTS_EINVAL, "row %d has no real token in the first T-7 slots", b);
        pad[b] = p;
        for (int j = 0; j < takes; ++j) e->n_real[b * takes + j] = base - p;
        e->max_real = std::max(e->max_real, base - p);
    }
    for (int b = 0; b < e->cfg.max_batch; ++b) { pool_release(e, b); e->slot_live[b] = b < R; }
    e->pending_edits.n = 0;
    TRY(pack_policy_reset(e, st));
    ForkJob fork;
    fork.np = 0; fork.nr = 0;
    for (int b = 0; b < B; ++b) {
        const int src = b * takes, len = e->n_real[src];
        const int need = (len + max_steps + MTTS_PAGE - 1) / MTTS_PAGE;
        if (need > e->max_pages) return fail(MTTS_ENOMEM, "row %d needs %d KV pages, a sequence holds at most %d (max_seq_len %d)", src, need, e->max_pages, e->cfg.max_seq_len);
        TRY(pool_grow(e, src, (len + MTTS_PAGE - 1) / MTTS_PAGE, st));
        for (int j = 1; j < takes; ++j) {
            const int dst = src + j;
            TRY(pool_share(e, src, dst, len / MTTS_PAGE, st));
            if (len % MTTS_PAGE) {
                TRY(pool_grow(e, dst, len / MTTS_PAGE + 1, st));
                fork.psrc[fork.np] = e->h_page_table[(size_t)src * e->max_pages + len / MTTS_PAGE];
                fork.pdst[fork.np++] = e->h_page_table[(size_t)dst * e->max_pages + len / MTTS_PAGE];
            }
            fork.rsrc[fork.nr] = src;
            fork.rdst[fork.nr++] = dst;
        }
    }
    TRY(pool_flush(e, st));
    if (e->max_real + max_steps > e->rope_rows)
        return fail(MTTS_EINVAL, "rope table has %d rows, need %d", e->rope_rows, e->max_real + max_steps);
    max_steps = std::max(max_steps, std::min(max_length - base + linger_bound(R),
                                             std::min(e->max_pages * MTTS_PAGE, e->rope_rows) - e->max_real));
    e->max_steps = max_steps;
    TRY(ensure_gen_storage(e, max_steps));
    TRY(start_scores(e, st));
    size_t Mtot = 0;
    for (int b = 0; b < B; ++b) Mtot += (size_t)round_up(e->n_real[b * takes], MTTS_MAXR);
    size_t Mpad = (Mtot + MTTS_RCAP - 1) / MTTS_RCAP * MTTS_RCAP;
    std::vector<int32_t> toks(Mpad * 8, 0);
    std::vector<RowMeta> metas(Mpad, RowMeta{-1, 0, 0, 0});
    size_t r = 0;
    for (int b = 0; b < B; r = (r + MTTS_MAXR - 1) / MTTS_MAXR * MTTS_MAXR, ++b)
        for (int i = 0; i < e->n_real[b * takes]; ++i, ++r) {
            const int64_t* src = ids + ((size_t)b * T + pad[b] + i) * 8;
            for (int c = 0; c < 8; ++c) {
                int64_t t = src[c];
                int64_t V = c == 0 ? e->V0 : e->Vs;
                if (t < 0 || t >= V) return fail(MTTS_EINVAL, "token %lld out of range on channel %d", (long long)t, c);
                toks[r * 8 + c] = (int32_t)t;
            }
            metas[r] = RowMeta{b * takes, i, i == e->n_real[b * takes] - 1 ? 1 : 0, 0};
        }
    TRY(grow_prefill_staging(e, Mpad));
    HIPCHK(hipMemcpyAsync(e->d_pf_tokens, toks.data(), Mpad * 8 * 4, hipMemcpyHostToDevice, st));
    HIPCHK(hipMemcpyAsync(e->d_pf_meta, metas.data(), Mpad * sizeof(RowMeta), hipMemcpyHostToDevice, st));
    {
        std::vector<uint32_t> bm((size_t)MTTS_RCAP * 8 * e->bm_words, 0u);
        for (int rw = 0; rw < R; ++rw)
            for (int t = 0, b = rw / takes; t < base; ++t)
                for (int c = 0; c < 8; ++c) {
                    int64_t tk = ids[((size_t)b * T + t) * 8 + c];
                    if (tk >= 0 && tk < (int64_t)e->bm_words * 32) bm[((size_t)rw * 8 + c) * e->bm_words + (tk >> 5)] |= 1u << (tk & 31);
                }
        HIPCHK(hipMemcpyAsync(e->d_bitmaps, bm.data(), bm.size() * 4, hipMemcpyHostToDevice, st));
        std::vector<int32_t> tf((size_t)MTTS_RCAP * 7 * 8, 0);
        for (int rw = 0; rw < R; ++rw)
            for (int s = 0, b = rw / takes; s < 7; ++s)
                for (int c = 0; c < 8; ++c) {
                    int64_t tk = ids[((size_t)b * T + base + s) * 8 + c];
                    if (tk < 0 || tk >= (c == 0 ? e->V0 : e->Vs)) return fail(MTTS_EINVAL, "token %lld out of range on channel %d (delayed tail)", (long long)tk, c);
                    tf[((size_t)rw * 7 + s) * 8 + c] = (int32_t)tk;
                }
        HIPCHK(hipMemcpyAsync(e->d_tf, tf.data(), tf.size() * 4, hipMemcpyHostToDevice, st));
        std::vector<SeqState> ss(MTTS_RCAP, IDLE_SEQ);
        if (!e->next_row_ids.empty() && (int)e->next_row_ids.size() != R)
            return fail(MTTS_EINVAL, "mtts_set_row_ids gave %d ids, the batch has %d rows", (int)e->next_row_ids.size(), R);
        for (int b = 0; b < R; ++b)
            ss[b] = SeqState{-1, 1, e->n_real[b], 0, base, max_length, e->next_row_ids.empty() ? b : e->next_row_ids[b], 1, seed};
        e->next_row_ids.clear();
        TRY(reset_run_state(e, ss, false, sampler, st));
    }
    TRY(prefill_staged(e, Mpad, (e->max_real + MTTS_PAGE - 1) / MTTS_PAGE, 2, st));
    if (fork.nr) TRY(launch_fork_job(e, fork, false, st));
    e->began = true;
    e->run_open = true;
    return MTTS_OK;
}

int32_t mtts_set_takes(MttsEngine* e, int32_t n) {
    if (!e) return fail(MTTS_EINVAL, "null engine");
    if (n < 1 || n > MTTS_RCAP) return fail(MTTS_EINVAL, "takes must be 1..%d (got %d)", MTTS_RCAP, n);
    e->next_takes = n;
    return MTTS_OK;
}

int32_t mtts_begin(MttsEngine* e, const int64_t* ids, const uint8_t* mask, int32_t B, int32_t T, int32_t max_length,
                   const MttsSamplerCfg* sampler, uint64_t seed, void* stream) {
    if (!e) return fail(MTTS_EINVAL, "null argument");
    const int takes = e->next_takes;
    e->next_takes = 1;
    return begin_run(e, ids, mask, B, T, max_length, sampler, seed, takes, stream);
}

static int step_body(MttsEngine* e, int pages_bound, hipStream_t st, int64_t kvtok) {
    launch_sample(e->logits0, e->logits17, e->V0, e->Vs, e->Vs_pad, e->d_bitmaps, e->bm_words, e->d_scfg, e->d_ls,
                  e->d_seqs, e->seed, e->d_decisions, &e->d_ls->error, e->B, e->sscr, e->ch0_sampled,
                  full_cap_for(e->V0), e->scores_on, st);
    launch_update(e->d_decisions, e->d_declog, e->has_forced ? e->d_forced : nullptr, e->d_tf, e->d_gen, e->d_cur,
                  e->d_seqs, e->d_meta, e->d_bitmaps, e->bm_words, e->d_ls, e->cfg.eos_token_id,
                  e->cfg.speech_pad_token, e->cfg.speech_range_lo, e->cfg.speech_range_hi,
                  e->scores_on ? e->sscr.lp : nullptr, e->scores_on ? e->d_lp : nullptr, st);
    return forward_rows(e, e->d_cur, e->d_meta, round_up(e->B, 32), pages_bound, 1, st, kvtok);
}

static int step_graph(MttsEngine* e, int pages, hipGraphExec_t* out) {
    const int forced = e->has_forced ? 1 : 0;
    for (auto& g : e->graphs)
        if (g.B == e->B && g.pages == pages && g.forced == forced && g.ch0 == e->ch0_sampled && g.scores == e->scores_on) {
            *out = g.exec;
            return MTTS_OK;
        }
    if (e->graphs.size() >= 256) drop_graphs(e);
    if (!e->cap_stream) HIPCHK(hipStreamCreateWithFlags(&e->cap_stream, hipStreamNonBlocking));
    hipGraph_t g = nullptr;
    HIPCHK(hipStreamBeginCapture(e->cap_stream, hipStreamCaptureModeRelaxed));
    int rc = step_body(e, pages, e->cap_stream, 0);
    hipError_t ce = hipStreamEndCapture(e->cap_stream, &g);
    if (rc) { if (g) hipGraphDestroy(g); return rc; }
    HIPCHK(ce);
    hipGraphExec_t exec = nullptr;
    hipError_t ie = hipGraphInstantiate(&exec, g, nullptr, nullptr, 0);
    hipGraphDestroy(g);
    HIPCHK(ie);
    e->graphs.push_back({e->B, pages, forced, e->ch0_sampled, e->scores_on, exec});
    *out = exec;
    return MTTS_OK;
}

static int issue_steps(MttsEngine* e, int n, hipStream_t st) {
    for (int i = 0; i < n; ++i) {
        if (e->steps_issued >= e->max_steps) break;
        int len_bound = 1;
        for (int b = 0; b < e->B; ++b) {
            if (!e->slot_live[b]) continue;
            const int len = e->n_real[b] + e->steps_issued + 1;
            len_bound = std::max(len_bound, len);
            TRY(pool_grow(e, b, (len + MTTS_PAGE - 1) / MTTS_PAGE, st));
        }
        TRY(pool_flush(e, st));
        const int pages_bound = (len_bound + MTTS_PAGE - 1) / MTTS_PAGE;
        if (e->use_graphs && !e->prof) {
            hipGraphExec_t exec = nullptr;
            TRY(step_graph(e, std::min(round_up(pages_bound, ATT_PB), e->max_pages), &exec));
            HIPCHK(hipGraphLaunch(exec, st));
        } else {
            hipEvent_t ev = nullptr;
            prof_begin(e, PROF_STEP, st, &ev);
            int64_t kvtok = 0;
            for (int b = 0; b < e->B; ++b) if (e->slot_live[b]) kvtok += e->n_real[b] + e->steps_issued + 1;
            TRY(step_body(e, pages_bound, st, kvtok));
            prof_end(e, st, ev);
        }
        e->steps_issued++;
    }
    return MTTS_OK;
}

int32_t mtts_step(MttsEngine* e, int32_t n_steps, void* stream) {
    if (!e || !e->began) return fail(MTTS_ESTATE, "mtts_begin has not run");
    HIPCHK(hipSetDevice(e->device));
    return issue_steps(e, n_steps, S(stream));
}

int32_t mtts_sync_state(MttsEngine* e, int32_t* steps_done, int32_t* all_finished, void* stream) {
    if (!e || !e->began) return fail(MTTS_ESTATE, "mtts_begin has not run");
    HIPCHK(hipSetDevice(e->device));
    HIPCHK(hipMemcpyAsync(e->h_ls, e->d_ls, sizeof(LoopState), hipMemcpyDeviceToHost, S(stream)));
    if (!e->continuous) HIPCHK(hipMemcpyAsync(e->h_seqs, e->d_seqs, e->B * sizeof(SeqState), hipMemcpyDeviceToHost, S(stream)));
    if (e->d_seal_cnt) HIPCHK(hipMemcpyAsync(e->h_seal_cnt, e->d_seal_cnt, (size_t)e->L * 4 * sizeof(unsigned long long), hipMemcpyDeviceToHost, S(stream)));
    HIPCHK(hipStreamSynchronize(S(stream)));
    if (e->d_seal_cnt && e->kv_pack == 1) {
        bool changed = false;
        for (int n = 0; n < e->L; ++n) {
            const unsigned long long* c = e->h_seal_cnt + (size_t)n * 4;
            const bool k_on = c[0] + c[1] < 16 || c[1] * 8 <= c[0] + c[1], v_on = c[2] + c[3] < 16 || c[3] * 8 <= c[2] + c[3];
            changed |= (k_on != (bool)e->pack_k_on[n]) || (v_on != (bool)e->pack_v_on[n]);
            e->pack_k_on[n] = k_on; e->pack_v_on[n] = v_on;
        }
        if (changed) drop_graphs(e);
    }
    if (e->h_ls->error) return fail(MTTS_EINVAL, "device sampler error %d: more than 4096 candidate tokens (set top_k so that the k-th score's radix bin holds <= 4096 tokens)", e->h_ls->error);
    if (!e->continuous) {
        const SeqState* ss = e->h_seqs;
        for (int b = 0; b < e->B; ++b)
            if (e->slot_live[b] && ss[b].step > 0 && !ss[b].unfinished && ss[b].active != 2) { e->slot_live[b] = 0; pool_release(e, b); }
    }
    if (steps_done) *steps_done = e->h_ls->step;
    if (all_finished) *all_finished = e->h_ls->done;
    if (e->h_ls->done && !e->continuous) e->run_open = false;
    return MTTS_OK;
}

template <typename Src, typename Dst>
static int read_slots(MttsEngine* e, const Src* d_src, int slot0, int nslots, int steps, Dst* host) {
    std::vector<Src> tmp((size_t)std::max(steps, 1) * 8);
    for (int b = 0; b < nslots; ++b) {
        if (steps) HIPCHK(hipMemcpy(tmp.data(), d_src + (size_t)(slot0 + b) * e->gen_cap * 8, (size_t)steps * 8 * sizeof(Src), hipMemcpyDeviceToHost));
        for (int s = 0; s < steps; ++s)
            for (int c = 0; c < 8; ++c) host[((size_t)s * nslots + b) * 8 + c] = tmp[(size_t)s * 8 + c];
    }
    return MTTS_OK;
}
template <typename Src, typename Dst>
static int read_rows(MttsEngine* e, const Src* d_src, Dst* host, int capacity_steps, int* n_steps) {
    const int steps = e->h_ls->step;
    if (steps > capacity_steps) return fail(MTTS_EINVAL, "output buffer holds %d steps, need %d", capacity_steps, steps);
    TRY(read_slots(e, d_src, 0, e->B, steps, host));
    if (n_steps) *n_steps = steps;
    return MTTS_OK;
}
template <typename Src, typename Dst>
static int slot_read(MttsEngine* e, const Src* d_src, int slot, Dst* host_rows, int capacity_steps, int* n_steps) {
    HIPCHK(hipSetDevice(e->device));
    HIPCHK(hipDeviceSynchronize());
    SeqState cur;
    HIPCHK(hipMemcpy(&cur, e->d_seqs + slot, sizeof(cur), hipMemcpyDeviceToHost));
    if (cur.step > capacity_steps) return fail(MTTS_EINVAL, "buffer holds %d steps, need %d", capacity_steps, cur.step);
    TRY(read_slots(e, d_src, slot, 1, cur.step, host_rows));
    if (n_steps) *n_steps = cur.step;
    return MTTS_OK;
}
template <typename T>
static int read_logits(MttsEngine* e, T* l0, T* l17, void* stream) {
    HIPCHK(hipSetDevice(e->device));
    HIPCHK(hipStreamSynchronize(S(stream)));
    if (l0) HIPCHK(hipMemcpy2D(l0, (size_t)e->V0 * sizeof(T), e->logits0, (size_t)e->V0_pad * sizeof(T), (size_t)e->V0 * sizeof(T), e->B, hipMemcpyDeviceToHost));
    if (l17) {
        std::vector<T> tmp((size_t)MTTS_RCAP * 7 * e->Vs_pad);
        HIPCHK(hipMemcpy(tmp.data(), e->logits17, tmp.size() * sizeof(T), hipMemcpyDeviceToHost));
        for (int c = 0; c < 7; ++c)
            for (int b = 0; b < e->B; ++b)
                memcpy(l17 + ((size_t)c * e->B + b) * e->Vs, tmp.data() + ((size_t)b * 7 + c) * e->Vs_pad, (size_t)e->Vs * sizeof(T));
    }
    return MTTS_OK;
}

int32_t mtts_read_generated(MttsEngine* e, int64_t* host_gen, int32_t capacity_steps, int32_t* n_steps) {
    if (!e || !e->began || !host_gen) return fail(MTTS_ESTATE, "nothing generated");
    HIPCHK(hipSetDevice(e->device));
    TRY(mtts_sync_state(e, nullptr, nullptr, nullptr));
    return read_rows(e, e->d_gen, host_gen, capacity_steps, n_steps);
}

int32_t mtts_set_output_scores(MttsEngine* e, int32_t on) {
    if (!e) return fail(MTTS_EINVAL, "null engine");
    on = on ? 1 : 0;
    if (on == e->scores_next) return MTTS_OK;
    if (e->run_open) {
        HIPCHK(hipSetDevice(e->device));
        HIPCHK(hipDeviceSynchronize());
        LoopState ls;
        std::vector<SeqState> ss(MTTS_RCAP);
        HIPCHK(hipMemcpy(&ls, e->d_ls, sizeof(ls), hipMemcpyDeviceToHost));
        HIPCHK(hipMemcpy(ss.data(), e->d_seqs, ss.size() * sizeof(SeqState), hipMemcpyDeviceToHost));
        bool live = false;
        for (int b = 0; b < e->B; ++b) live |= ss[b].active != 0;
        if (live && !ls.done)
            return fail(MTTS_ESTATE, "output_scores cannot change while a run is open (it is read when a run begins)");
        e->run_open = false;
    }
    e->scores_next = on;
    return MTTS_OK;
}

int32_t mtts_read_scores(MttsEngine* e, float* host_lp, int32_t capacity_steps, int32_t* n_steps) {
    if (!e || !e->began || !host_lp) return fail(MTTS_ESTATE, "nothing generated");
    if (!e->scores_on) return fail(MTTS_ESTATE, "the run was started with output_scores off (mtts_set_output_scores)");
    HIPCHK(hipSetDevice(e->device));
    TRY(mtts_sync_state(e, nullptr, nullptr, nullptr));
    return read_rows(e, e->d_lp, host_lp, capacity_steps, n_steps);
}

int32_t mtts_read_logits_f32(MttsEngine* e, float* l0, float* l17, void* stream) {
    if (!e || !e->began) return fail(MTTS_ESTATE, "mtts_begin has not run");
    if (!e->f32) return fail(MTTS_ESTATE, "bf16 engine: use mtts_read_logits");
    return read_logits(e, l0, l17, stream);
}
// ... 324 lines not shown
```

moss-ttsd_amd/csrc/hooks.hip:

```cpp
#include "engine.h"

int32_t mtts_k_gemm_bf16(const void* w, const void* x, void* y, int32_t M, int32_t N, int32_t K, int32_t ksplit, void* stream) {
    if (!w || !x || !y || M < 1 || M > MTTS_PFCAP || K % 16 || N < 1) return fail(MTTS_EINVAL, "gemm: need 1<=M<=MTTS_PFCAP, K%%16==0");
    hipStream_t st = S(stream);
    int Npad = round_up(N, 32);
    void *wp = nullptr, *xp = nullptr;
    float* part = nullptr;
    GemmPlan p = mtts_plan_gemm(Npad, K, ksplit);
    p.depth = gemm_depth_env();
    DevBufs hb;
    TRY(hb.get((uint16_t**)&wp, (size_t)Npad * K));
    const bool tiled = M > MTTS_RCAP;
    const int ks = tiled ? (ksplit > 0 ? ksplit : mtts_tile_ksplit(Npad, K, M)) : p.ksplit;
    TRY(hb.get((uint16_t**)&xp, (size_t)MTTS_PFCAP * K));
    TRY(hb.get(&part, (size_t)ks * MTTS_PFCAP * Npad));
    launch_pack_weight(w, wp, N, K, Npad, 1, 0, st);
    const int tiles = (M + 31) / 32;
    launch_pack_rows(x, xp, M, K, tiles == 3 ? 4 : tiles, st);
    if (tiled) launch_gemm_tile(EPI_PARTIAL, M, ks, wp, xp, K, Npad, Npad, part, nullptr, st);
    else launch_gemm(EPI_PARTIAL, tiles, p, wp, xp, K, Npad, Npad, part, nullptr, st);
    launch_reduce_partial_bf16(part, y, ks, Npad, N, M, st);
    HIPCHK(hipGetLastError());
    HIPCHK(hipStreamSynchronize(st));
    return MTTS_OK;
// ... 21 lines not shown
}

int32_t mtts_k_rmsnorm(const void* x, const void* w, void* y, int32_t rows, int32_t n, float eps, void* stream) {
    if (!x || !w || !y || rows < 1 || n < 1) return fail(MTTS_EINVAL, "rmsnorm: bad argument");
    launch_rmsnorm_rows(x, w, y, rows, n, eps, S(stream));
    HIPCHK(hipGetLastError());
    return MTTS_OK;
}

static int k_sample(const void* logits, int32_t rows, int32_t vocab, const void* bitmap, const MttsSamplerCfg* cfg,
                    int32_t mask_id, uint64_t seed, int32_t step, int32_t channel, int32_t* dev_tokens, float* dev_logp, void* stream) {
    if (!logits || !cfg || !dev_tokens || rows < 1 || vocab < 1 || channel < 0 || channel > 7) return fail(MTTS_EINVAL, "sample: bad argument");
    hipStream_t st = S(stream);
    MttsSamplerCfg h[8];
    for (int i = 0; i < 8; ++i) h[i] = *cfg;
    MttsSamplerCfg* d = nullptr;
    int32_t *err = nullptr, *dec = nullptr;
    if (rows > MTTS_RCAP) return fail(MTTS_EINVAL, "sample: at most 128 rows");
    DevBufs hb;
    TRY(hb.get(&d, 8));
    TRY(hb.get(&err, 1));
    TRY(hb.get(&dec, (size_t)rows * 8));
    HIPCHK(hipMemcpy(d, h, sizeof(h), hipMemcpyHostToDevice));
    SampleScratch sc;
    TRY(alloc_scratch(hb, sc, rows, vocab));
    if (dev_logp) TRY(alloc_lp_scratch(hb, sc, rows));
    launch_sample_single(logits, rows, vocab, (const uint32_t*)bitmap, (vocab + 31) / 32, d, mask_id, seed, step, channel, dec, err, sc,
                         full_cap_for(vocab), dev_logp ? 1 : 0, st);
    HIPCHK(hipGetLastError());
    HIPCHK(hipStreamSynchronize(st));
    std::vector<int32_t> hd((size_t)rows * 8);
    int32_t herr = 0;
    HIPCHK(hipMemcpy(hd.data(), dec, hd.size() * 4, hipMemcpyDeviceToHost));
    HIPCHK(hipMemcpy(&herr, err, 4, hipMemcpyDeviceToHost));
    std::vector<int32_t> outv(rows);
    for (int r = 0; r < rows; ++r) outv[r] = hd[(size_t)r * 8 + channel];
    HIPCHK(hipMemcpy(dev_tokens, outv.data(), rows * 4, hipMemcpyHostToDevice));
    if (dev_logp) {
        std::vector<float> hl((size_t)rows * 8), outl(rows);
        HIPCHK(hipMemcpy(hl.data(), sc.lp, hl.size() * 4, hipMemcpyDeviceToHost));
        for (int r = 0; r < rows; ++r) outl[r] = hl[(size_t)r * 8 + channel];
        HIPCHK(hipMemcpy(dev_logp, outl.data(), rows * 4, hipMemcpyHostToDevice));
    }
    if (herr) return fail(MTTS_EINVAL, "sample: more than 4096 candidate tokens");
    return MTTS_OK;
}

int32_t mtts_k_sample(const void* logits, int32_t rows, int32_t vocab, const void* bitmap, const MttsSamplerCfg* cfg,
                      int32_t mask_id, uint64_t seed, int32_t step, int32_t channel, int32_t* dev_tokens, void* stream) {
    return k_sample(logits, rows, vocab, bitmap, cfg, mask_id, seed, step, channel, dev_tokens, nullptr, stream);
}

int32_t mtts_k_sample_scores(const void* logits, int32_t rows, int32_t vocab, const void* bitmap, const MttsSamplerCfg* cfg,
                             int32_t mask_id, uint64_t seed, int32_t step, int32_t channel, int32_t* dev_tokens, float* dev_logp,
                             void* stream) {
    if (!dev_logp) return fail(MTTS_EINVAL, "sample: null dev_logp");
    return k_sample(logits, rows, vocab, bitmap, cfg, mask_id, seed, step, channel, dev_tokens, dev_logp, stream);
}


int32_t mtts_k_rope_kvwrite(const void* dev_qkv, const int32_t* host_pos, const void* dev_qnorm, const void* dev_knorm,
                            const void* dev_cos, const void* dev_sin, int32_t R, int32_t nq, int32_t nkv, float eps,
                            void* dev_q, void* dev_k, void* dev_v, void* stream) {
    if (!dev_qkv || !host_pos || !dev_q || !dev_k || !dev_v || R < 1 || R > MTTS_RCAP || nq < 1 || nkv < 1) return fail(MTTS_EINVAL, "rope_kvwrite: bad argument");
    hipStream_t st = S(stream);
    const int N = (nq + 2 * nkv) * MTTS_HD;
    int maxpos = 0;
    for (int r = 0; r < R; ++r) { if (host_pos[r] < 0) return fail(MTTS_EINVAL, "negative position"); maxpos = std::max(maxpos, host_pos[r]); }
    const int max_pages = maxpos / MTTS_PAGE + 1, total_pages = R * max_pages;
    float* slab = nullptr; RowMeta* meta = nullptr; int32_t* pt = nullptr; uint16_t *kc = nullptr, *vc = nullptr;
    DevBufs hb;
    TRY(hb.get(&slab, (size_t)MTTS_PFCAP * N));
    TRY(hb.get(&meta, R)); TRY(hb.get(&pt, (size_t)R * max_pages));
    TRY(hb.get(&kc, (size_t)total_pages * nkv * MTTS_PAGE * MTTS_HD)); TRY(hb.get(&vc, (size_t)total_pages * nkv * MTTS_PAGE * MTTS_HD));
    std::vector<RowMeta> hm(R);
    std::vector<int32_t> hpt((size_t)R * max_pages);
    for (int r = 0; r < R; ++r) { hm[r] = RowMeta{r, host_pos[r], 1, 0}; for (int p = 0; p < max_pages; ++p) hpt[(size_t)r * max_pages + p] = r * max_pages + p; }
    HIPCHK(hipMemcpy(meta, hm.data(), R * sizeof(RowMeta), hipMemcpyHostToDevice));
    HIPCHK(hipMemcpy(pt, hpt.data(), hpt.size() * 4, hipMemcpyHostToDevice));
    launch_bf16_to_f32(dev_qkv, slab, (size_t)R * N, st);
    launch_qkv_post(slab, 1, N, meta, dev_qnorm, dev_knorm, dev_cos, dev_sin, dev_q, kc, vc, pt, max_pages, total_pages, R, nq, nkv, eps, st);
    HIPCHK(hipGetLastError());
    HIPCHK(hipStreamSynchronize(st));
    std::vector<uint16_t> hk((size_t)total_pages * nkv * MTTS_PAGE * MTTS_HD), hv(hk.size()), ok((size_t)R * nkv * MTTS_HD), ov(ok.size());
    HIPCHK(hipMemcpy(hk.data(), kc, hk.size() * 2, hipMemcpyDeviceToHost));
    HIPCHK(hipMemcpy(hv.data(), vc, hv.size() * 2, hipMemcpyDeviceToHost));
    for (int r = 0; r < R; ++r)
        for (int h = 0; h < nkv; ++h)
            for (int d = 0; d < MTTS_HD; ++d) {
                const int page = r * max_pages + host_pos[r] / MTTS_PAGE, t = host_pos[r] % MTTS_PAGE;
                const size_t base = ((size_t)h * total_pages + page) * (MTTS_PAGE * MTTS_HD);
                ok[((size_t)r * nkv + h) * MTTS_HD + d] = hk[base + (((d >> 3) * 64) + t) * 8 + (d & 7)];
                ov[((size_t)r * nkv + h) * MTTS_HD + d] = hv[base + ((size_t)(t >> 1) * MTTS_HD + d) * 2 + (t & 1)];
            }
    HIPCHK(hipMemcpy(dev_k, ok.data(), ok.size() * 2, hipMemcpyHostToDevice));
    HIPCHK(hipMemcpy(dev_v, ov.data(), ov.size() * 2, hipMemcpyHostToDevice));
    return MTTS_OK;
}

int32_t mtts_k_paged_attn_decode(const void* dev_q, const void* dev_k, const void* dev_v, const int32_t* host_lens,
                                 const int32_t* host_page_table, int32_t R, int32_t Lmax, int32_t nq, int32_t nkv,
                                 void* dev_out, void* stream) {
    if (!dev_q || !dev_k || !dev_v || !host_lens || !dev_out || R < 1 || R > MTTS_MAXR || Lmax < 1 || nq < 1 || nkv < 1 || nq % nkv)
        return fail(MTTS_EINVAL, "paged_attn_decode: bad argument (1..32 rows)");
    hipStream_t st = S(stream);
    const int max_pages = (Lmax + MTTS_PAGE - 1) / MTTS_PAGE, total_pages = R * max_pages, nch = (max_pages + ATT_PB - 1) / ATT_PB;
    std::vector<int32_t> hpt((size_t)R * max_pages);
    std::vector<char> seen(total_pages, 0);
    for (size_t i = 0; i < hpt.size(); ++i) {
        hpt[i] = host_page_table ? host_page_table[i] : (int32_t)i;
        if (hpt[i] < 0 || hpt[i] >= total_pages || seen[hpt[i]]) return fail(MTTS_EINVAL, "page table must be a permutation of 0..%d", total_pages - 1);
        seen[hpt[i]] = 1;
    }
    std::vector<RowMeta> hm(MTTS_MAXR, RowMeta{-1, 0, 0, 0});
    int pages_bound = 1;
    for (int r = 0; r < R; ++r) {
        if (host_lens[r] < 1 || host_lens[r] > Lmax) return fail(MTTS_EINVAL, "row %d: length %d outside 1..%d", r, host_lens[r], Lmax);
        hm[r] = RowMeta{r, host_lens[r] - 1, 1, 0};
        pages_bound = std::max(pages_bound, (host_lens[r] + MTTS_PAGE - 1) / MTTS_PAGE);
    }
    RowMeta* meta = nullptr; int32_t *pt = nullptr, *lens = nullptr; uint16_t *kc = nullptr, *vc = nullptr, *scores = nullptr, *outp = nullptr;
    float *stats = nullptr, *opart = nullptr;
    const size_t cache_n = (size_t)total_pages * nkv * MTTS_PAGE * MTTS_HD;
    DevBufs hb;
    TRY(hb.get(&meta, MTTS_MAXR)); TRY(hb.get(&pt, hpt.size())); TRY(hb.get(&lens, R));
    TRY(hb.get(&kc, cache_n)); TRY(hb.get(&vc, cache_n));
    TRY(hb.get(&scores, (size_t)MTTS_MAXR * nq * max_pages * MTTS_PAGE));
    TRY(hb.get(&stats, (size_t)MTTS_MAXR * nq * max_pages * 2));
    TRY(hb.get(&opart, (size_t)MTTS_MAXR * nq * nch * MTTS_HD));
    TRY(hb.get(&outp, (size_t)MTTS_MAXR * nq * MTTS_HD));
    HIPCHK(hipMemcpy(meta, hm.data(), hm.size() * sizeof(RowMeta), hipMemcpyHostToDevice));
    HIPCHK(hipMemcpy(pt, hpt.data(), hpt.size() * 4, hipMemcpyHostToDevice));
    HIPCHK(hipMemcpy(lens, host_lens, R * 4, hipMemcpyHostToDevice));
    launch_pack_kv_pages(dev_k, dev_v, kc, vc, pt, lens, R, Lmax, nkv, max_pages, total_pages, st);
    KvPack pk{nullptr, nullptr};
    const char* g = getenv("MTTS_KV_PACK");
    if (!g || atoi(g) != 0) {
        uint8_t *kp = nullptr, *vp = nullptr;
        const size_t pk_n = (size_t)total_pages * nkv * MTTS_PKU * 64 * 16;
        TRY(hb.get(&kp, pk_n)); TRY(hb.get(&vp, pk_n));
        launch_kv_seal_all(kc, vc, kp, vp, total_pages, nkv, 1, nullptr, st);
        pk = KvPack{kp, vp};
    }
    const float scale = 1.0f / sqrtf((float)MTTS_HD);
    if (launch_attn(dev_q, kc, vc, pt, meta, scores, stats, opart, outp, MTTS_MAXR, pages_bound, max_pages, total_pages, nch, nq, nkv,
                    scale, nullptr, ATTN_ALL, st, pk.k ? &pk : nullptr))
        return fail(MTTS_EINVAL, "attention group size not built (1, 2, 4)");
    launch_unpack_rows(outp, dev_out, R, nq * MTTS_HD, st);
    HIPCHK(hipGetLastError());
    HIPCHK(hipStreamSynchronize(st));
    return MTTS_OK;
}

int32_t mtts_k_kv_seal(const void* dev_pages, int32_t npages, void* dev_sealed, int32_t as_k, void* stream) {
    if (!dev_pages || !dev_sealed || npages < 1) return fail(MTTS_EINVAL, "kv_seal: bad argument");
    launch_kv_seal_pages(dev_pages, dev_sealed, npages, as_k, S(stream));
    HIPCHK(hipGetLastError());
    HIPCHK(hipStreamSynchronize(S(stream)));
    return MTTS_OK;
}

int32_t mtts_debug_kv_pack_stats(MttsEngine* e, int64_t* out6) {
    if (!e || !out6) return fail(MTTS_EINVAL, "null argument");
    if (!e->kpack) return fail(MTTS_ESTATE, "the engine keeps no sealed pages (fp32 / fp16 engine, or MTTS_KV_PACK=0)");
    HIPCHK(hipSetDevice(e->device));
    HIPCHK(hipDeviceSynchronize());
    std::vector<SeqState> ss(MTTS_RCAP);
    HIPCHK(hipMemcpy(ss.data(), e->d_seqs, ss.size() * sizeof(SeqState), hipMemcpyDeviceToHost));
    std::vector<int32_t> complete(e->B, 0);
    for (int b = 0; b < e->B; ++b)
        if (e->slot_live[b]) complete[b] = std::min(ss[b].kv_len >> 6, e->n_pages[b]);
    DevBufs hb;
    int32_t* dc = nullptr; unsigned long long* dout = nullptr;
    TRY(hb.get(&dc, e->B)); TRY(hb.get(&dout, 4));
    HIPCHK(hipMemcpy(dc, complete.data(), e->B * 4, hipMemcpyHostToDevice));
    HIPCHK(hipMemset(dout, 0, 32));
    launch_kv_pack_count(e->kpack, e->vpack, e->d_page_table, dc, e->B, e->max_pages, e->total_pages, e->nkv, e->L, dout, nullptr);
    HIPCHK(hipGetLastError());
    unsigned long long h[4];
    HIPCHK(hipMemcpy(h, dout, 32, hipMemcpyDeviceToHost));
    for (int i = 0; i < 4; ++i) out6[i] = (int64_t)h[i];
    out6[4] = out6[5] = 0;
    for (int n = 0; n < e->L; ++n) { out6[4] += e->pack_k_on[n]; out6[5] += e->pack_v_on[n]; }
    return MTTS_OK;
}

int32_t mtts_debug_set_kv_len(MttsEngine* e, int32_t kv_len) {
    if (!e || !e->began) return fail(MTTS_ESTATE, "mtts_begin has not run");
    if (e->f32) return fail(MTTS_EINVAL, "measurement hook of the bf16 engine");
    HIPCHK(hipSetDevice(e->device));
    HIPCHK(hipDeviceSynchronize());
    const int cap = std::min(e->max_pages * MTTS_PAGE, e->rope_rows);
    const int limit = cap - MTTS_PAGE;
    if (kv_len < 1 || kv_len > limit) return fail(MTTS_EINVAL, "kv_len %d outside 1..%d", kv_len, limit);
    e->max_steps = std::min(e->max_steps, e->steps_issued + cap - kv_len);
    std::vector<SeqState> ss(MTTS_RCAP);
    HIPCHK(hipMemcpy(ss.data(), e->d_seqs, ss.size() * sizeof(SeqState), hipMemcpyDeviceToHost));
    for (int b = 0; b < e->B; ++b) { ss[b].kv_len = kv_len; e->n_real[b] = kv_len - e->steps_issued; }
    e->max_real = kv_len - e->steps_issued;
    HIPCHK(hipMemcpy(e->d_seqs, ss.data(), ss.size() * sizeof(SeqState), hipMemcpyHostToDevice));
    launch_fill_random_bf16(e->kcache, e->layer_stride * e->L, 0x1234u, nullptr);
    launch_fill_random_bf16(e->vcache, e->layer_stride * e->L, 0x9876u, nullptr);
    if (e->kpack) launch_kv_seal_all(e->kcache, e->vcache, e->kpack, e->vpack, e->total_pages, e->nkv, e->L, nullptr, nullptr);
    HIPCHK(hipDeviceSynchronize());
    return MTTS_OK;
}

int32_t mtts_k_attn_bench(MttsEngine* e, int32_t phase, int32_t iters, float* avg_ms, int64_t* bytes_per_launch) {
    if (!e || !e->began || (phase != ATTN_SCORES && phase != ATTN_PV) || iters < 1 || !avg_ms) return fail(MTTS_EINVAL, "attn_bench: bad argument");
    if (e->f32) return fail(MTTS_EINVAL, "measurement hook of the bf16 engine");
    HIPCHK(hipSetDevice(e->device));
    HIPCHK(hipDeviceSynchronize());
    const float scale = 1.0f / sqrtf((float)MTTS_HD);
    const int R = round_up(e->B, 32);
    const int len_bound = e->max_real + e->steps_issued + 1;
    const int pages_bound = (len_bound + MTTS_PAGE - 1) / MTTS_PAGE;
    hipEvent_t e0, e1;
    hipEventCreate(&e0); hipEventCreate(&e1);
    auto run = [&](int n) {
        for (int i = 0; i < n; ++i) {
            const int layer = i % e->L;
            uint16_t* kc = (uint16_t*)e->kcache + e->layer_stride * layer;
            uint16_t* vc = (uint16_t*)e->vcache + e->layer_stride * layer;
            const QkvFuse fz{e->partial, e->p_qkv.ksplit, e->qkv_rows, (const uint16_t*)e->layers[layer].qn,
                             (const uint16_t*)e->layers[layer].kn, e->rope_cos, e->rope_sin, e->cfg.rms_norm_eps};
            const KvPack pk = layer_pack(e, layer, pages_bound);
            launch_attn(e->qbuf, kc, vc, e->d_page_table, e->d_meta, e->scores, e->stats, e->opart, e->attn_p, R, pages_bound,
                        e->max_pages, e->total_pages, e->nchunks_max, e->nq, e->nkv, scale, e->B * pages_bound <= e->fuse_qkv_max ? &fz : nullptr, (AttnPhase)phase, nullptr,
                        (pk.k || pk.v) ? &pk : nullptr);
        }
    };
    run(e->L);
    hipEventRecord(e0, nullptr);
    run(iters);
    hipEventRecord(e1, nullptr);
    HIPCHK(hipEventSynchronize(e1));
    float ms = 0;
    hipEventElapsedTime(&ms, e0, e1);
    *avg_ms = ms / iters;
    if (bytes_per_launch) {
        std::vector<RowMeta> m(MTTS_RCAP);
        HIPCHK(hipMemcpy(m.data(), e->d_meta, m.size() * sizeof(RowMeta), hipMemcpyDeviceToHost));
        int64_t tok = 0;
        for (int b = 0; b < R; ++b) if (m[b].seq >= 0) tok += m[b].pos + 1;
        *bytes_per_launch = tok * e->nkv * MTTS_HD * 2;
    }
    hipEventDestroy(e0); hipEventDestroy(e1);
    return MTTS_OK;
}

int32_t mtts_k_gemm_bench(int32_t N, int32_t K, int32_t epi, int32_t ksplit, int32_t waves, int32_t copies,
                                     int32_t iters, float* avg_us) {
    if (N % 32 || K % 16 || copies < 1 || iters < 1 || !avg_us) return fail(MTTS_EINVAL, "gemm_bench: bad argument");
    const int tile_rows = waves < 0 ? -waves : 0;
    if (tile_rows > MTTS_PFCAP) return fail(MTTS_EINVAL, "gemm_bench: at most MTTS_PFCAP rows");
    GemmPlan p = (ksplit > 0 && waves > 0) ? mtts_plan_gemm_forced(N, K, ksplit, waves) : mtts_plan_gemm(N, K, tile_rows ? std::max(ksplit, 1) : ksplit);
    if (tile_rows) p.ksplit = std::max(ksplit, 1);
    p.depth = gemm_depth_env();
    DevBufs hb;
    std::vector<uint16_t*> w(copies, nullptr);
    for (auto& q : w) { TRY(hb.get(&q, (size_t)N * K, false)); HIPCHK(hipMemset(q, 0x3c, (size_t)N * K * 2)); }
    uint16_t *x = nullptr, *out = nullptr;
    float* part = nullptr;
    TRY(hb.get(&x, (size_t)MTTS_PFCAP * K, false));
    HIPCHK(hipMemset(x, 0x3c, (size_t)MTTS_PFCAP * K * 2));
    TRY(hb.get(&out, (size_t)MTTS_PFCAP * N));
    TRY(hb.get(&part, (size_t)p.ksplit * MTTS_PFCAP * N));
    hipEvent_t e0, e1;
    hipEventCreate(&e0); hipEventCreate(&e1);
    auto go = [&](int i) {
        if (tile_rows) launch_gemm_tile(epi, tile_rows, p.ksplit, w[i % copies], x, K, N, N, part, out, nullptr);
        else launch_gemm(epi, 1, p, w[i % copies], x, K, N, N, part, out, nullptr);
    };
    for (int i = 0; i < copies; ++i) go(i);
    HIPCHK(hipDeviceSynchronize());
    hipEventRecord(e0, nullptr);
    for (int i = 0; i < iters; ++i) go(i);
    hipEventRecord(e1, nullptr);
    HIPCHK(hipEventSynchronize(e1));
    float ms = 0;
    hipEventElapsedTime(&ms, e0, e1);
    *avg_us = ms * 1000.f / iters;
    hipEventDestroy(e0); hipEventDestroy(e1);
    return MTTS_OK;
}
```

moss-ttsd_amd/csrc/launch.h:

```cpp
#pragma once
#include <type_traits>

#include "../../include/mtts.h"
#include "common.h"

enum { EPI_PARTIAL = 0, EPI_BF16 = 1, EPI_SILU = 2,
       EPI_SILU_RM = 3 };
struct GemmPlan {
    int waves, ksplit, kt_per_split, kt_per_wave;
    int depth;
};
GemmPlan mtts_plan_gemm(int Npad, int K, int want_ksplit);
GemmPlan mtts_plan_gemm_forced(int Npad, int K, int ksplit, int waves);
void launch_gemm(int epi, int mb, const GemmPlan& p, const void* Wp, const void* Xp, int K, int Npad, int n_valid,
                 float* partial, uint16_t* out, hipStream_t st);
int mtts_tile_ksplit(int Npad, int K, int R);
void launch_gemm_tile(int epi, int R, int ksplit, const void* Wp, const void* Xp, int K, int Npad, int n_valid,
                      float* partial, uint16_t* out, hipStream_t st);
int mtts_small_lds_bytes(const GemmPlan& p, int K, int pro);
void launch_gemv_small(int epi, int pro, const GemmPlan& p, const void* Wp, int K, int Npad, int n_valid, float* partial,
                       uint16_t* out, const SmallPro& pr, hipStream_t st);
long long mtts_gemm_depth_launches();
void launch_pack_weight(const void* src, void* dst, int rows, int cols, int rows_pad, int row_mul, int row_off, hipStream_t st);
void launch_pack_rows(const void* src, void* dst, int R, int K, int tiles, hipStream_t st);
void launch_reduce_partial_bf16(const float* partial, void* out, int ksplit, int Npad, int n_valid, int R, hipStream_t st);

struct PageEdits { int32_t n; int32_t idx[31]; int32_t val[31]; };
static_assert(sizeof(PageEdits) == 252, "PageEdits is a kernel argument: one 32-bit count + 31 (index, value) pairs");
void launch_embed_norm(const int32_t* tokens, const RowMeta* meta, const uint16_t* const* tables, const void* norm_w,
                       void* x, void* xn_packed, int R, int H, float eps, hipStream_t st);
void launch_resid_norm(const float* partial, int ksplit, int Npad, void* x, const void* norm_w, void* xn_packed,
                       void* hlast, const RowMeta* meta, int R, int H, float eps, hipStream_t st);
void launch_qkv_post(const float* partial, int ksplit, int Npad, const RowMeta* meta, const void* qnw, const void* knw,
                     const void* cosb, const void* sinb, void* qbuf, void* kcache, void* vcache,
                     const int32_t* page_table, int max_pages, int total_pages, int R, int nq, int nkv, float eps,
                     hipStream_t st);
void launch_rmsnorm_rows(const void* x, const void* w, void* y, int rows, int n, float eps, hipStream_t st);
void launch_fill_random_bf16(void* p, size_t n, uint32_t seed, hipStream_t st);
void launch_set_pages(int32_t* table, const PageEdits& ed, hipStream_t st);
void launch_fork(void* kc, void* vc, size_t layer_bytes, size_t head_bytes, int blk_bytes, int L, int nkv, const ForkJob& job,
                 hipStream_t st);
void launch_pack_kv_pages(const void* K, const void* V, void* kcache, void* vcache, const int32_t* page_table, const int32_t* lens,
                          int S, int Lmax, int nkv, int max_pages, int total_pages, hipStream_t st);
void launch_bf16_to_f32(const void* a, float* b, size_t n, hipStream_t st);
void launch_unpack_rows(const void* packed, void* out, int R, int K, hipStream_t st);

enum AttnPhase { ATTN_ALL = 0, ATTN_SCORES = 1, ATTN_PV = 2, ATTN_COMBINE = 3,
                 ATTN_PF_SCORES = 11, ATTN_PF_PV = 12, ATTN_PF_COMBINE = 13 };
int launch_attn(const void* qbuf, void* kcache, void* vcache, const int32_t* page_table,
                const RowMeta* meta, void* scores, float* stats, float* opart, void* out_packed, int R,
                int pages_bound, int max_pages, int total_pages, int nchunks_max, int nq, int nkv, float scale,
                const QkvFuse* fuse, AttnPhase phase, hipStream_t st, const KvPack* pack = nullptr);
void launch_kv_seal_rows(const void* kcache, const void* vcache, void* kpack, void* vpack, const int32_t* page_table,
                         const RowMeta* meta, int R, int max_pages, int total_pages, int nkv, int L, unsigned long long* cnt, hipStream_t st);
void launch_kv_seal_all(const void* kcache, const void* vcache, void* kpack, void* vpack, int total_pages, int nkv, int L,
                        unsigned long long* cnt, hipStream_t st);
void launch_kv_seal_pages(const void* raw, void* pk, int npages, int as_k, hipStream_t st);
void launch_kv_pack_count(const void* kpack, const void* vpack, const int32_t* page_table, const int32_t* complete, int B, int max_pages,
                          int total_pages, int nkv, int L, unsigned long long* out, hipStream_t st);

struct SeqState {
    int32_t nas;
    int32_t unfinished;
    int32_t kv_len;
    int32_t step;
    int32_t base_length;
    int32_t max_length;
    int32_t row_id;
    int32_t active;
    uint64_t seed;
};

struct LoopState {
    int32_t step;
    int32_t done;
    int32_t continuous;
    int32_t B;
    int32_t error;
    int32_t gen_cap;
    int32_t forced_draw;
    int32_t logits_f32;
};
static_assert(sizeof(SeqState) == 40 && std::is_trivially_copyable<SeqState>::value, "SeqState layout");
static_assert(sizeof(LoopState) == 32 && std::is_trivially_copyable<LoopState>::value, "LoopState layout");

#define SAMP_CAND 4096
#define SAMP_NS 32
struct SampleScratch {
    uint32_t* hist = nullptr;
    float* slice_val = nullptr;
    int32_t* slice_idx = nullptr;
    float* cand_val = nullptr;
    int32_t* cand_idx = nullptr;
    uint32_t* cand_n = nullptr;
    int32_t* overflow = nullptr;
    float* full_val = nullptr;
    int32_t* full_idx = nullptr;
    uint32_t* nuc_cnt = nullptr;
    unsigned long long* nuc_mass = nullptr;
    float* slice_sum = nullptr;
    float* lp = nullptr;
};
void launch_sample(const void* logits0, const void* logits17, int V0, int Vs, int Vs_pad, const uint32_t* bitmaps,
                   int bm_words, const MttsSamplerCfg* cfgs, const LoopState* ls, const SeqState* seqs, uint64_t seed,
                   int32_t* decisions, int32_t* err, int B, const SampleScratch& sc, int ch0_sampled, int full_cap,
                   int emit_lp, hipStream_t st);
void launch_sample_single(const void* logits, int rows, int vocab, const uint32_t* bitmap, int bm_words,
                          const MttsSamplerCfg* cfgs8, int mask_id, uint64_t seed, int step, int channel,
                          int32_t* decisions, int32_t* err, const SampleScratch& sc, int full_cap, int emit_lp, hipStream_t st);
void launch_update(const int32_t* decisions, int32_t* dec_log, const int32_t* forced, const int32_t* tf_tail,
                   int32_t* gen, int32_t* cur_tokens, SeqState* seqs, RowMeta* meta, uint32_t* bitmaps, int bm_words,
                   LoopState* ls, int eos, int spad, int sp_lo, int sp_hi, const float* lp_in, float* lp_out, hipStream_t st);
void launch_export_codes(const int32_t* gen, int64_t* codes, int B, int first, int n, int speech_offset, int clamp_hi,
                         int cap, hipStream_t st);

#define MTTS_PF32CAP 256
void launch_f32_embed_norm(const int32_t* tokens, const RowMeta* meta, const float* const* tables, const float* norm_w, float* x,
                           float* xn, int R, int H, float eps, int h16, hipStream_t st);
void launch_f32_resid_norm(const float* y, float* x, const float* norm_w, float* xn, float* hlast, const RowMeta* meta, int R,
                           int H, float eps, int h16, hipStream_t st);
void launch_f32_linear(const float* W, const float* X, float* Y, int R, int N, int K, long ldy, int h16, bool gemv, hipStream_t st);
void launch_f32_qkv_post(const float* qkv, int ldq, const RowMeta* meta, const float* qnw, const float* knw, const float* cosb,
                         const float* sinb, float* qbuf, float* kcache, float* vcache, const int32_t* page_table, int max_pages,
                         int total_pages, int R, int nq, int nkv, float eps, int h16, hipStream_t st);
void launch_f32_attn(const float* qbuf, const float* kcache, const float* vcache, const int32_t* page_table, const RowMeta* meta,
                     float* scores, float* out, int R, int max_pages, int total_pages, int nq, int nkv, float scale, int Lmax,
                     int h16, hipStream_t st);
void launch_f32_swiglu(const float* gu, float* act, int R, int I, int h16, hipStream_t st);

void mtts_gemm_f32_exact(hipStream_t st, const float* A, const float* W, float* C, int M, int N, int K, long ldc);
void launch_split_pack_w2perm(hipStream_t st, const float* w2, uint16_t* hi, uint16_t* lo);
void launch_vocos_pw_fused(hipStream_t st, const uint16_t* xn_planes, long x_plane_elems, const uint16_t* w1_planes, const float* b1,
                           const uint16_t* w2perm_planes, long w_plane_elems, const float* b2, const float* gamma, float* h, int M);
```

moss-ttsd_amd/mtts/capi.py:

```python
from __future__ import annotations

import ctypes as C
import os

_HERE = os.path.dirname(os.path.abspath(__file__))
LIB_PATH = os.path.join(os.path.dirname(_HERE), "lib", "libmtts.so")


class MttsConfig(C.Structure):
    _fields_ = [(n, C.c_int32) for n in (
        "vocab_size", "hidden_size", "intermediate_size", "num_hidden_layers", "num_attention_heads",
        "num_key_value_heads", "head_dim", "channels", "speech_vocab_size", "speech_pad_token",
        "speech_range_lo", "speech_range_hi", "eos_token_id", "max_position")] + [
        ("rms_norm_eps", C.c_float), ("max_batch", C.c_int32), ("max_seq_len", C.c_int32), ("kv_pool_pages", C.c_int32), ("dtype", C.c_int32)]


class MttsSamplerCfg(C.Structure):
    _fields_ = [("do_sample", C.c_int32), ("top_k", C.c_int32), ("top_p", C.c_float),
                ("one_minus_top_p", C.c_float), ("temperature", C.c_float), ("repetition_penalty", C.c_float)]


class MttsCodecConfig(C.Structure):
    _fields_ = [(n, C.c_int32) for n in (
        "nq", "codebook_size", "rvq_dim", "quant_out_dim",
        "adapter_layers", "adapter_dim", "adapter_heads", "adapter_ffn", "adapter_max_pos", "up_stride",
        "dec_layers", "dec_dim", "dec_heads", "dec_ffn", "dec_max_pos", "mel_bins",
        "voc_dim", "voc_inter", "voc_layers", "n_fft", "hop",
        "mel_n_fft", "mel_hop", "mel_frames", "enc_layers", "enc_dim", "enc_heads", "enc_ffn", "enc_max_pos",
        "sem_adapter_layers", "pre_rvq_layers", "down_pool")]


class MttsError(RuntimeError):
    def __init__(self, msg, code=0):
        super().__init__(msg)
        self.code = code


ENOMEM = -3
ESTATE = -4


_lib = None

_SIGS = {
    "mtts_last_error": (C.c_char_p, []),
    "mtts_version": (C.c_int32, []),
    "mtts_engine_create": (C.c_int32, [C.POINTER(MttsConfig), C.c_int32, C.POINTER(C.c_void_p)]),
    "mtts_engine_destroy": (C.c_int32, [C.c_void_p]),
    "mtts_bind_weight": (C.c_int32, [C.c_void_p, C.c_char_p, C.c_void_p, C.c_int64, C.c_int64, C.c_void_p]),
    "mtts_bind_rope": (C.c_int32, [C.c_void_p, C.c_void_p, C.c_void_p, C.c_int32, C.c_void_p]),
    "mtts_weights_ready": (C.c_int32, [C.c_void_p]),
    "mtts_generate": (C.c_int32, [C.c_void_p, C.c_void_p, C.c_void_p, C.c_int32, C.c_int32, C.c_int32,
                                  C.POINTER(MttsSamplerCfg), C.c_uint64, C.c_void_p, C.c_int32,
                                  C.POINTER(C.c_int32), C.c_void_p, C.c_int32, C.c_void_p, C.c_void_p]),
    "mtts_begin": (C.c_int32, [C.c_void_p, C.c_void_p, C.c_void_p, C.c_int32, C.c_int32, C.c_int32,
                               C.POINTER(MttsSamplerCfg), C.c_uint64, C.c_void_p]),
    "mtts_step": (C.c_int32, [C.c_void_p, C.c_int32, C.c_void_p]),
    "mtts_sync_state": (C.c_int32, [C.c_void_p, C.POINTER(C.c_int32), C.POINTER(C.c_int32), C.c_void_p]),
    "mtts_read_generated": (C.c_int32, [C.c_void_p, C.c_void_p, C.c_int32, C.POINTER(C.c_int32)]),
    "mtts_set_output_scores": (C.c_int32, [C.c_void_p, C.c_int32]),
    "mtts_read_scores": (C.c_int32, [C.c_void_p, C.c_void_p, C.c_int32, C.POINTER(C.c_int32)]),
    "mtts_slot_read_scores": (C.c_int32, [C.c_void_p, C.c_int32, C.c_void_p, C.c_int32, C.POINTER(C.c_int32)]),
    "mtts_read_logits": (C.c_int32, [C.c_void_p, C.c_void_p, C.c_void_p, C.c_void_p]),
    "mtts_read_logits_f32": (C.c_int32, [C.c_void_p, C.c_void_p, C.c_void_p, C.c_void_p]),
    "mtts_sched_open": (C.c_int32, [C.c_void_p, C.c_int32, C.c_int32, C.POINTER(MttsSamplerCfg), C.c_void_p]),
    "mtts_slot_submit": (C.c_int32, [C.c_void_p, C.c_int32, C.c_void_p, C.c_int32, C.c_int32, C.c_uint64, C.c_void_p]),
    "mtts_slot_submit_row": (C.c_int32, [C.c_void_p, C.c_int32, C.c_void_p, C.c_int32, C.c_int32, C.c_uint64, C.c_int32, C.c_void_p]),
    "mtts_set_row_ids": (C.c_int32, [C.c_void_p, C.c_void_p, C.c_int32]),
    "mtts_set_takes": (C.c_int32, [C.c_void_p, C.c_int32]),
    "mtts_slot_fork": (C.c_int32, [C.c_void_p, C.c_int32, C.c_int32, C.c_uint64, C.c_int32, C.c_void_p]),
    "mtts_slot_states": (C.c_int32, [C.c_void_p, C.c_void_p, C.c_void_p]),
    "mtts_slot_read": (C.c_int32, [C.c_void_p, C.c_int32, C.c_void_p, C.c_int32, C.POINTER(C.c_int32)]),
    "mtts_read_seq_state": (C.c_int32, [C.c_void_p, C.c_void_p, C.c_void_p, C.c_void_p, C.c_void_p]),
    "mtts_slot_evict": (C.c_int32, [C.c_void_p, C.c_int32, C.c_void_p]),
    "mtts_kv_pool_state": (C.c_int32, [C.c_void_p, C.POINTER(C.c_int32), C.POINTER(C.c_int32), C.POINTER(C.c_int32)]),
    "mtts_read_page_table": (C.c_int32, [C.c_void_p, C.c_void_p, C.c_void_p]),
    "mtts_set_forced_mode": (C.c_int32, [C.c_void_p, C.c_int32]),
    "mtts_debug_read_device_page_table": (C.c_int32, [C.c_void_p, C.c_void_p, C.c_void_p]),
    "mtts_export_codes": (C.c_int32, [C.c_void_p, C.c_int32, C.c_int32, C.c_void_p, C.c_void_p]),
    "mtts_profile_enable": (C.c_int32, [C.c_void_p, C.c_int32]),
    "mtts_profile_read": (C.c_int32, [C.c_void_p, C.c_int32, C.POINTER(C.c_double), C.POINTER(C.c_int64),
                                      C.POINTER(C.c_int64)]),
    "mtts_debug_set_kv_len": (C.c_int32, [C.c_void_p, C.c_int32]),
    "mtts_debug_kv_pack_stats": (C.c_int32, [C.c_void_p, C.c_void_p]),
    "mtts_k_kv_seal": (C.c_int32, [C.c_void_p, C.c_int32, C.c_void_p, C.c_int32, C.c_void_p]),
    "mtts_k_attn_bench": (C.c_int32, [C.c_void_p, C.c_int32, C.c_int32, C.POINTER(C.c_float), C.POINTER(C.c_int64)]),
    "mtts_k_gemm_bench": (C.c_int32, [C.c_int32] * 7 + [C.POINTER(C.c_float)]),
    "mtts_k_gemm_bf16": (C.c_int32, [C.c_void_p, C.c_void_p, C.c_void_p, C.c_int32, C.c_int32, C.c_int32,
                                     C.c_int32, C.c_void_p]),
    "mtts_debug_gemm_depth_launches": (C.c_int64, []),
    "mtts_k_gemm_swiglu_bf16": (C.c_int32, [C.c_void_p, C.c_void_p, C.c_void_p, C.c_int32, C.c_int32, C.c_int32, C.c_void_p]),
    "mtts_k_rmsnorm": (C.c_int32, [C.c_void_p, C.c_void_p, C.c_void_p, C.c_int32, C.c_int32, C.c_float, C.c_void_p]),
    "mtts_k_rope_kvwrite": (C.c_int32, [C.c_void_p] * 6 + [C.c_int32, C.c_int32, C.c_int32, C.c_float] + [C.c_void_p] * 4),
    "mtts_k_paged_attn_decode": (C.c_int32, [C.c_void_p] * 5 + [C.c_int32] * 4 + [C.c_void_p, C.c_void_p]),
    "mtts_k_sample": (C.c_int32, [C.c_void_p, C.c_int32, C.c_int32, C.c_void_p, C.POINTER(MttsSamplerCfg),
                                  C.c_int32, C.c_uint64, C.c_int32, C.c_int32, C.c_void_p, C.c_void_p]),
    "mtts_k_sample_scores": (C.c_int32, [C.c_void_p, C.c_int32, C.c_int32, C.c_void_p, C.POINTER(MttsSamplerCfg),
                                         C.c_int32, C.c_uint64, C.c_int32, C.c_int32, C.c_void_p, C.c_void_p, C.c_void_p]),
    "mtts_codec_last_error": (C.c_char_p, []),
    "mtts_codec_create": (C.c_int32, [C.POINTER(MttsCodecConfig), C.c_int32, C.POINTER(C.c_void_p)]),
    "mtts_codec_destroy": (C.c_int32, [C.c_void_p]),
    "mtts_codec_bind": (C.c_int32, [C.c_void_p, C.c_char_p, C.c_void_p, C.c_int64, C.c_void_p]),
    "mtts_codec_detokenize": (C.c_int32, [C.c_void_p, C.c_void_p, C.c_void_p, C.c_int32, C.c_int32, C.c_void_p, C.c_void_p]),
    "mtts_codec_detokenize_async": (C.c_int32, [C.c_void_p, C.c_void_p, C.c_void_p, C.c_int32, C.c_int32, C.c_void_p, C.c_void_p]),
    "mtts_codec_check": (C.c_int32, [C.c_void_p, C.c_void_p]),
    "mtts_codec_tokenize": (C.c_int32, [C.c_void_p, C.c_void_p, C.c_void_p, C.c_int32, C.c_int32, C.c_void_p, C.c_void_p, C.c_void_p]),
    "mtts_k_gemm_f32": (C.c_int32, [C.c_void_p, C.c_void_p, C.c_void_p, C.c_void_p, C.c_int32, C.c_int32, C.c_int32,
                                    C.c_int32, C.c_void_p]),
    "mtts_k_gemm_planes_bench": (C.c_int32, [C.c_int32, C.c_int32, C.c_int32, C.c_int32, C.c_int32, C.c_int32,
                                             C.POINTER(C.c_float), C.POINTER(C.c_int32)]),
}


def exported_symbols():
    return sorted(_SIGS)


def lib():
    global _lib
    if _lib is None:
        if not os.path.exists(LIB_PATH):
            raise MttsError(f"{LIB_PATH} is missing: build it with `python moss-ttsd_amd/build.py` "
                            "(hipcc --offload-arch=gfx950); there is no CPU fallback")
        L = C.CDLL(LIB_PATH)
        for name, (res, args) in _SIGS.items():
            fn = getattr(L, name)
            fn.restype = res
            fn.argtypes = args
        _lib = L
    return _lib


def check(rc):
    if rc != 0:
        raise MttsError(f"libmtts error {rc}: {lib().mtts_last_error().decode()}", rc)
```

Baseline: 73080 codec_tokens/s.

## Add whole-row fused decode attention kernel covering QKV epilogue, scores, softmax and PV

```diff
diff --git a/include/mtts.h b/include/mtts.h
--- a/include/mtts.h
+++ b/include/mtts.h
@@ -110,6 +110,12 @@
 int32_t mtts_k_gemm_bf16(const void* dev_w, const void* dev_x, void* dev_y,
                          int32_t M, int32_t N, int32_t K, int32_t ksplit, void* stream);
 int64_t mtts_debug_gemm_depth_launches(void);
+int64_t mtts_debug_attn_row_launches(void);
+int32_t mtts_k_attn_section(const float* dev_slabs, int32_t ksplit, const void* dev_qnw, const void* dev_knw, const void* dev_cos,
+                            const void* dev_sin, float eps, const void* dev_k, const void* dev_v, const int32_t* host_lens,
+                            const int32_t* host_page_table, int32_t R, int32_t Lmax, int32_t nq, int32_t nkv, int32_t sealed,
+                            int32_t path, void* dev_out, void* dev_kcache, void* dev_vcache, void* dev_kpack, void* dev_vpack,
+                            void* stream);
 int32_t mtts_k_gemm_swiglu_bf16(const void* dev_w, const void* dev_x, void* dev_y,
                                 int32_t M, int32_t N, int32_t K, void* stream);
 int32_t mtts_k_rmsnorm(const void* dev_x, const void* dev_w, void* dev_y,
diff --git a/moss-ttsd_amd/csrc/attn.hip b/moss-ttsd_amd/csrc/attn.hip
--- a/moss-ttsd_amd/csrc/attn.hip
+++ b/moss-ttsd_amd/csrc/attn.hip
@@ -1,4 +1,6 @@
 #include "launch.h"
+#include <algorithm>
+#include <atomic>
 #include <cstdlib>
 #ifndef MTTS_PK_WAVES
 #define MTTS_PK_WAVES 0
@@ -747,6 +749,335 @@
     out_packed[xpack_off(r, h * MTTS_HD + d, nq * MTTS_HD)] = f2bf(s);
 }
 
+#ifndef ROW_WAVES
+#define ROW_WAVES 12
+#endif
+static_assert(ROW_WAVES >= 6 && ROW_WAVES <= 16, "one wave per q head + the K row + the V row; at most 1024 threads");
+static std::atomic<long long> g_row_launches{0};
+long long mtts_attn_row_launches() { return g_row_launches.load(); }
+int attn_row_lds_bytes(int G, bool pk, int pages_bound) {
+    const int nch = (pages_bound + ATT_PB - 1) / ATT_PB;
+    return G * 256 + 512 + (pk ? ROW_WAVES * G * 256 : 0) + ROW_WAVES * G * 128 + G * pages_bound * (8 + 128) + PV_WAVES * nch * G * 512;
+}
+
+template <int G, bool PK>
+__global__ __launch_bounds__(ROW_WAVES * 64) void attn_row_kernel(
+    u32x4_t* __restrict__ kcache, u32x4_t* __restrict__ vcache, const int32_t* __restrict__ page_table,
+    const RowMeta* __restrict__ meta, uint16_t* __restrict__ out_packed, int npb, int max_pages, int total_pages, int nq,
+    int nkv, float scale, QkvFuse f, const u32x4_t* __restrict__ kpack, const u32x4_t* __restrict__ vpack) {
+    constexpr int W = ROW_WAVES;
+    extern __shared__ __attribute__((aligned(16))) uint8_t row_lds[];
+    uint32_t* qs = (uint32_t*)row_lds;
+    uint16_t* knew = (uint16_t*)(row_lds + G * 256);
+    uint16_t* vnew = knew + MTTS_HD;
+    uint32_t* qw = (uint32_t*)(row_lds + G * 256 + 512);
+    uint16_t* pbuf = (uint16_t*)((uint8_t*)qw + (PK ? W * G * 256 : 0));
+    float2* st = (float2*)((uint8_t*)pbuf + W * G * 128);
+    uint16_t* sc = (uint16_t*)(st + G * npb);
+    float* items = (float*)(sc + (size_t)G * npb * MTTS_PAGE);
+    const int r = blockIdx.y, kvh = blockIdx.x;
+    const RowMeta m = meta[r];
+    if (m.seq < 0) {
+        for (int i = threadIdx.x; i < G * MTTS_HD; i += W * 64) out_packed[xpack_off(r, kvh * G * MTTS_HD + i, nq * MTTS_HD)] = f2bf(0.f);
+        return;
+    }
+    const int len = m.pos + 1;
+    const int npages = min((len + MTTS_PAGE - 1) / MTTS_PAGE, npb);
+    const int nch = (npages + ATT_PB - 1) / ATT_PB;
+    const int wave = __builtin_amdgcn_readfirstlane(threadIdx.x >> 6), lane = threadIdx.x & 63;
+    const int own_pg = m.pos >> 6;
+    const int sub = lane >> 5, dl = lane & 31;
+    const int32_t* ptab = page_table + (size_t)m.seq * max_pages;
+
+    const bool epi = wave < G + 2;
+    const int vw = epi ? wave + W - (G + 2) : wave - (G + 2);
+    if (epi) {
+        const int col = (wave < G ? kvh * G + wave : wave == G ? nq + kvh : nq + nkv + kvh) * MTTS_HD;
+        FuseVec pfv{0.f, 0.f, 0.f, 0.f};
+        if (wave <= G) pfv = fuse_load_vec(f, wave == G ? f.knorm_w : f.qnorm_w, m.pos, lane);
+        float a, b;
+        if (f.ksplit <= 8) {
+            float pta[8], ptb[8];
+            fuse_reduce_request(f, r, col, lane, pta, ptb);
+            fuse_reduce_sum(f, pta, ptb, a, b);
+        } else fuse_reduce(f, r, col, lane, a, b);
+        const int opage = ptab[own_pg], tok = m.pos & 63;
+        if (wave <= G) {
+            float o1, o2;
+            fuse_norm_rope(f, pfv, a, b, o1, o2);
+            if (wave < G) {
+                ((uint16_t*)(qs + wave * 64))[lane] = f2bf(o1);
+                ((uint16_t*)(qs + wave * 64))[lane + 64] = f2bf(o2);
+            } else {
+                knew[lane] = f2bf(o1);
+                knew[lane + 64] = f2bf(o2);
+                uint16_t* base = (uint16_t*)kcache + ((size_t)kvh * total_pages + opage) * (MTTS_PAGE * MTTS_HD);
+                base[(((lane >> 3) * 64) + tok) * 8 + (lane & 7)] = f2bf(o1);
+                base[((((lane + 64) >> 3) * 64) + tok) * 8 + (lane & 7)] = f2bf(o2);
+            }
+        } else {
+            vnew[lane] = f2bf(a);
+            vnew[lane + 64] = f2bf(b);
+            uint16_t* dst = (uint16_t*)vcache + ((size_t)kvh * total_pages + opage) * (MTTS_PAGE * MTTS_HD) + (size_t)(tok >> 1) * (MTTS_HD * 2) + (tok & 1);
+            dst[2 * lane] = f2bf(a);
+            dst[2 * (lane + 64)] = f2bf(b);
+        }
+        __builtin_amdgcn_sched_barrier(0);
+    }
+    auto stage = [&]() { __syncthreads(); };
+
+    auto finish = [&](int pg, const float* acc) {
+        const int tok = pg * MTTS_PAGE + lane;
+        const bool valid = tok < len;
+#pragma unroll
+        for (int g = 0; g < G; ++g) {
+            float s = rbf(rbf(acc[g]) * scale);
+            if (valid) sc[(size_t)g * npb * MTTS_PAGE + tok] = f2bf(s);
+            float mx = wave_max(valid ? s : -INFINITY);
+            float e = valid ? expf(s - mx) : 0.f;
+            float sm = wave_sum(e);
+            if (lane == 0) st[g * npb + pg] = float2{mx, sm};
+        }
+    };
+    auto raw_dots = [&](int pg, u32x4_t (&kv)[16]) {
+        if (pg == own_pg && lane == (m.pos & 63)) {
+#pragma unroll
+            for (int j = 0; j < 16; ++j) kv[j] = *(const u32x4_t*)&knew[8 * j];
+        }
+        float acc[G];
+#pragma unroll
+        for (int g = 0; g < G; ++g) acc[g] = 0.f;
+#pragma unroll
+        for (int j = 0; j < 16; ++j) {
+#pragma unroll
+            for (int g = 0; g < G; ++g) {
+                const u32x4_t q = *(const u32x4_t*)&qs[g * 64 + 4 * j];
+                acc[g] = dot2bf(kv[j].x, q.x, acc[g]);
+                acc[g] = dot2bf(kv[j].y, q.y, acc[g]);
+                acc[g] = dot2bf(kv[j].z, q.z, acc[g]);
+                acc[g] = dot2bf(kv[j].w, q.w, acc[g]);
+            }
+#pragma unroll
+            for (int g = 0; g < G; ++g) asm volatile("" : "+v"(acc[g]));
+            if ((j & 3) == 3) __builtin_amdgcn_sched_barrier(0);
+        }
+        finish(pg, acc);
+    };
+    auto k_page = [&](int pg, bool first) {
+        const int page = ptab[pg];
+        const u32x4_t* kp = kcache + ((size_t)kvh * total_pages + page) * (MTTS_PAGE * MTTS_HD / 8) + lane;
+        if (PK && pg < own_pg) {
+            u32x4_t pk[MTTS_PKU];
+            const u32x4_t* pp = kpack + ((size_t)kvh * total_pages + page) * (MTTS_PKU * 64) + lane;
+#pragma unroll
+            for (int j = 0; j < MTTS_PKU; ++j) pk[pk_order(j)] = __builtin_nontemporal_load(pp + pk_order(j) * 64);
+            if (first) stage();
+            bool qok = true;
+            const uint32_t sh = pk[12].z;
+            uint32_t* qwv = qw + wave * G * 64;
+            __builtin_amdgcn_wave_barrier();
+#pragma unroll
+            for (int g = 0; g < G; ++g) {
+                const uint32_t qd = qs[g * 64 + lane];
+                uint32_t out = 0u;
+#pragma unroll
+                for (int h = 0; h < 2; ++h) {
+                    uint32_t b = (qd >> (16 * h)) & 0xffffu;
+                    const int sft = (int)(int8_t)((sh >> (8 * h)) & 0xffu);
+                    if ((b & 0x7fffu) && sft) {
+                        const int e = (int)((b >> 7) & 0xffu), e2 = e + sft;
+                        if (e == 0 || e == 255 || e2 < 1 || e2 > 254) qok = false;
+                        else b = (b + ((uint32_t)sft << 7)) & 0xffffu;
+                    }
+                    out |= b << (16 * h);
+                }
+                qwv[g * 64 + lane] = out;
+            }
+            __builtin_amdgcn_wave_barrier();
+            if (__any(pk[12].w != 0u || !qok)) {
+                u32x4_t kv[16];
+#pragma unroll
+                for (int j = 0; j < 16; ++j) kv[j] = __builtin_nontemporal_load(kp + j * 64);
+                raw_dots(pg, kv);
+                return;
+            }
+            float acc[G];
+#pragma unroll
+            for (int g = 0; g < G; ++g) acc[g] = 0.f;
+#pragma unroll
+            for (int j = 0; j < 16; ++j) {
+                uint32_t w[4];
+                pk_unit(pk, j, w);
+#pragma unroll
+                for (int g = 0; g < G; ++g) {
+                    const u32x4_t q = *(const u32x4_t*)&qwv[g * 64 + 4 * j];
+                    acc[g] = dot2bf(w[0], q.x, acc[g]);
+                    acc[g] = dot2bf(w[1], q.y, acc[g]);
+                    acc[g] = dot2bf(w[2], q.z, acc[g]);
+                    acc[g] = dot2bf(w[3], q.w, acc[g]);
+                }
+#pragma unroll
+                for (int g = 0; g < G; ++g) asm volatile("" : "+v"(acc[g]));
+                if ((j & 3) == 3) __builtin_amdgcn_sched_barrier(0);
+            }
+            finish(pg, acc);
+        } else {
+            u32x4_t kv[16];
+#pragma unroll
+            for (int j = 0; j < 16; ++j) kv[j] = __builtin_nontemporal_load(kp + j * 64);
+            if (first) stage();
+            raw_dots(pg, kv);
+        }
+    };
+    if (vw < npages) k_page(vw, true);
+    else stage();
+#pragma unroll 1
+    for (int pg = vw + W; pg < npages; pg += W) k_page(pg, false);
+
+    u32x4_t vv[16];
+    bool packed = false;
+    const u32x4_t* vp = nullptr;
+    auto load_page = [&](int pg) {
+        const int page = ptab[pg];
+        vp = vcache + ((size_t)kvh * total_pages + page) * (MTTS_PAGE * MTTS_HD / 8) + lane;
+        packed = PK && pg < own_pg;
+        if (packed) {
+            const u32x4_t* pp = vpack + ((size_t)kvh * total_pages + page) * (MTTS_PKU * 64) + lane;
+#pragma unroll
+            for (int it = 0; it < MTTS_PKU; ++it) vv[pk_order(it)] = __builtin_nontemporal_load(pp + pk_order(it) * 64);
+        } else {
+#pragma unroll
+            for (int it = 0; it < 16; ++it) vv[it] = __builtin_nontemporal_load(vp + it * 64);
+        }
+    };
+    if (2 * wave < npages) load_page(2 * wave);
+    __syncthreads();
+    float M[G], S[G];
+#pragma unroll
+    for (int g = 0; g < G; ++g) {
+        const float2* sg = st + g * npb;
+        const float2 s0 = lane < npages ? sg[lane] : float2{-INFINITY, 0.f};
+        float mx = -INFINITY;
+        mx = fmaxf(mx, s0.x);
+        for (int p = lane + 64; p < npages; p += 64) mx = fmaxf(mx, sg[p].x);
+        mx = wave_max(mx);
+        float sm = 0.f;
+        if (lane < npages) sm += s0.y * expf(s0.x - mx);
+        for (int p = lane + 64; p < npages; p += 64) sm += sg[p].y * expf(sg[p].x - mx);
+        sm = wave_sum(sm);
+        M[g] = mx;
+        S[g] = sm;
+    }
+    uint16_t* pb = pbuf + wave * G * MTTS_PAGE;
+#pragma unroll 1
+    for (int item = wave; item < PV_WAVES * nch; item += W) {
+        float acc[G][4];
+#pragma unroll
+        for (int g = 0; g < G; ++g)
+#pragma unroll
+            for (int i = 0; i < 4; ++i) acc[g][i] = 0.f;
+#pragma unroll 1
+        for (int pp = 0; pp < ATT_PB / PV_WAVES; ++pp) {
+            const int pg = item * (ATT_PB / PV_WAVES) + pp;
+            if (pg >= npages) break;
+            if (pp > 0 || item != wave) load_page(pg);
+            if (pg == own_pg) {
+                const int tp = (m.pos & 63) >> 1;
+                if (sub == (tp & 1)) {
+                    const uint32_t w01 = ((const uint32_t*)vnew)[2 * dl], w23 = ((const uint32_t*)vnew)[2 * dl + 1];
+                    const uint32_t nv[4] = {w01 & 0xffffu, w01 >> 16, w23 & 0xffffu, w23 >> 16};
+                    const bool hi = m.pos & 1;
+#pragma unroll
+                    for (int it = 0; it < 16; ++it)
+                        if (it == (tp >> 1)) {
+                            vv[it].x = hi ? (vv[it].x & 0xffffu) | (nv[0] << 16) : (vv[it].x & 0xffff0000u) | nv[0];
+                            vv[it].y = hi ? (vv[it].y & 0xffffu) | (nv[1] << 16) : (vv[it].y & 0xffff0000u) | nv[1];
+                            vv[it].z = hi ? (vv[it].z & 0xffffu) | (nv[2] << 16) : (vv[it].z & 0xffff0000u) | nv[2];
+                            vv[it].w = hi ? (vv[it].w & 0xffffu) | (nv[3] << 16) : (vv[it].w & 0xffff0000u) | nv[3];
+                        }
+                }
+            }
+            uint16_t pun[G];
+            bool pok = true;
+            {
+                const int tok = pg * MTTS_PAGE + lane;
+                const int sv = (PK && packed) ? (int)(vv[12].z & 0xffu) : 0;
+#pragma unroll
+                for (int g = 0; g < G; ++g) {
+                    float p = 0.f;
+                    if (tok < len) {
+                        float s = bf2f(sc[(size_t)g * npb * MTTS_PAGE + tok]);
+                        p = expf(s - M[g]) / S[g];
+                    }
+                    uint32_t pbits = f2bf(p);
+                    pun[g] = (uint16_t)pbits;
+                    if (sv && (pbits & 0x7fffu)) {
+                        if (((pbits >> 7) & 0xffu) == 0u) pok = false;
+                        else pbits += (uint32_t)sv << 7;
+                    }
+                    pb[g * MTTS_PAGE + lane] = (uint16_t)pbits;
+                }
+            }
+            __builtin_amdgcn_wave_barrier();
+            if (PK && packed && __any(vv[12].w != 0u || !pok)) {
+                packed = false;
+#pragma unroll
+                for (int it = 0; it < 16; ++it) vv[it] = __builtin_nontemporal_load(vp + it * 64);
+#pragma unroll
+                for (int g = 0; g < G; ++g) pb[g * MTTS_PAGE + lane] = pun[g];
+                __builtin_amdgcn_wave_barrier();
+            }
+            if (PK && packed) {
+#pragma unroll
+                for (int it = 0; it < 16; ++it) {
+                    uint32_t w[4];
+                    pk_unit(vv, it, w);
+#pragma unroll
+                    for (int g = 0; g < G; ++g) {
+                        const uint32_t pp2 = ((const uint32_t*)(pb + g * MTTS_PAGE))[it * 2 + sub];
+                        acc[g][0] = dot2bf(w[0], pp2, acc[g][0]);
+                        acc[g][1] = dot2bf(w[1], pp2, acc[g][1]);
+                        acc[g][2] = dot2bf(w[2], pp2, acc[g][2]);
+                        acc[g][3] = dot2bf(w[3], pp2, acc[g][3]);
+                    }
+                }
+            } else {
+#pragma unroll
+                for (int it = 0; it < 16; ++it) {
+#pragma unroll
+                    for (int g = 0; g < G; ++g) {
+                        const uint32_t pp2 = ((const uint32_t*)(pb + g * MTTS_PAGE))[it * 2 + sub];
+                        acc[g][0] = dot2bf(vv[it].x, pp2, acc[g][0]);
+                        acc[g][1] = dot2bf(vv[it].y, pp2, acc[g][1]);
+                        acc[g][2] = dot2bf(vv[it].z, pp2, acc[g][2]);
+                        acc[g][3] = dot2bf(vv[it].w, pp2, acc[g][3]);
+                    }
+                }
+            }
+            __builtin_amdgcn_wave_barrier();
+        }
+#pragma unroll
+        for (int g = 0; g < G; ++g)
+#pragma unroll
+            for (int i = 0; i < 4; ++i) {
+                const float v = add_xor32(acc[g][i]);
+                if (sub == 0) items[((size_t)item * G + g) * MTTS_HD + dl * 4 + i] = v;
+            }
+    }
+    __syncthreads();
+    for (int i = threadIdx.x; i < G * MTTS_HD; i += W * 64) {
+        float s = 0.f;
+        for (int c = 0; c < nch; ++c) {
+            const float* it4 = items + (size_t)PV_WAVES * c * G * MTTS_HD + i;
+            float v = it4[0];
+#pragma unroll
+            for (int w = 1; w < PV_WAVES; ++w) v += it4[(size_t)w * G * MTTS_HD];
+            s += v;
+        }
+        out_packed[xpack_off(r, kvh * G * MTTS_HD + i, nq * MTTS_HD)] = f2bf(s);
+    }
+}
+
 
 template <int G>
 __global__ __launch_bounds__(256) void attn_prefill_scores_kernel(
@@ -966,6 +1297,17 @@
     const QkvFuse f = fuse ? *fuse : QkvFuse{nullptr, 0, 0, nullptr, nullptr, nullptr, nullptr, 0.f};
     const u32x4_t* kpk = pack ? (const u32x4_t*)pack->k : nullptr;
     const u32x4_t* vpk = pack ? (const u32x4_t*)pack->v : nullptr;
+    if (phase == ATTN_ROW) {
+        const size_t lds = (size_t)attn_row_lds_bytes(G, kpk != nullptr, pages_bound);
+        if (kpk)
+            hipLaunchKernelGGL((attn_row_kernel<G, true>), dim3(nkv, R), dim3(ROW_WAVES * 64), lds, st, (u32x4_t*)kcache, (u32x4_t*)vcache,
+                               page_table, meta, (uint16_t*)out_packed, pages_bound, max_pages, total_pages, nq, nkv, scale, f, kpk, vpk);
+        else
+            hipLaunchKernelGGL((attn_row_kernel<G, false>), dim3(nkv, R), dim3(ROW_WAVES * 64), lds, st, (u32x4_t*)kcache, (u32x4_t*)vcache,
+                               page_table, meta, (uint16_t*)out_packed, pages_bound, max_pages, total_pages, nq, nkv, scale, f, kpk, vpk);
+        g_row_launches.fetch_add(1);
+        return;
+    }
 #define MTTS_SC(FU, PK)                                                                                                  \
     hipLaunchKernelGGL((attn_scores_kernel<G, FU, PK>), ga, dim3(256), 0, st, (const uint16_t*)qbuf, (u32x4_t*)kcache, \
                        page_table, meta, (uint16_t*)scores, stats, max_pages, total_pages, nq, nkv, scale, f, kpk)
@@ -995,11 +1337,42 @@
                            (uint16_t*)out_packed, nchunks_max, nq, ATT_PB);
 }
 
+static int g_row_lds_max = 0;
+bool attn_row_fits(int G, const QkvFuse* fuse, const KvPack* pack, int pages_bound) {
+    const bool pk = pack && pack->k;
+    if (!fuse || (G != 1 && G != 2 && G != 4) || pk != (pack && pack->v)) return false;
+    return attn_row_lds_bytes(G, pk, pages_bound) <= g_row_lds_max;
+}
+int attn_row_prepare() {
+    int dev = 0, cand[3] = {0, 0, 0};
+    if (hipGetDevice(&dev) != hipSuccess) return -1;
+    const hipDeviceAttribute_t attrs[3] = {hipDeviceAttributeMaxSharedMemoryPerMultiprocessor, hipDeviceAttributeSharedMemPerBlockOptin,
+                                           hipDeviceAttributeMaxSharedMemoryPerBlock};
+    for (int i = 0; i < 3; ++i)
+        if (hipDeviceGetAttribute(&cand[i], attrs[i], dev) != hipSuccess) { cand[i] = 0; (void)hipGetLastError(); }
+    std::sort(cand, cand + 3, [](int x, int y) { return x > y; });
+    for (int i = 0; i < 3; ++i) {
+        const int lim = cand[i];
+        if (lim <= 0 || (i && lim == cand[i - 1])) continue;
+        hipError_t e = hipSuccess;
+#define MTTS_ROWP(GG, PK) \
+    if (e == hipSuccess) e = hipFuncSetAttribute((const void*)attn_row_kernel<GG, PK>, hipFuncAttributeMaxDynamicSharedMemorySize, lim)
+        MTTS_ROWP(1, false); MTTS_ROWP(1, true); MTTS_ROWP(2, false); MTTS_ROWP(2, true); MTTS_ROWP(4, false); MTTS_ROWP(4, true);
+#undef MTTS_ROWP
+        if (e == hipSuccess) { g_row_lds_max = lim; return 0; }
+        (void)hipGetLastError();
+    }
+    return -1;
+}
+int attn_row_lds_limit() { return g_row_lds_max; }
+
 int launch_attn(const void* qbuf, void* kcache, void* vcache, const int32_t* page_table,
                 const RowMeta* meta, void* scores, float* stats, float* opart, void* out_packed, int R,
                 int pages_bound, int max_pages, int total_pages, int nchunks_max, int nq, int nkv, float scale,
                 const QkvFuse* fuse, AttnPhase phase, hipStream_t st, const KvPack* pack) {
     int G = nq / nkv;
+    if (G != 1 && G != 2 && G != 4) return -1;
+    if (phase == ATTN_ROW && !attn_row_fits(G, fuse, pack, pages_bound)) return -2;
 #define MTTS_ATT(GG)                                                                                              \
     launch_attn_g<GG>(qbuf, kcache, vcache, page_table, meta, scores, stats, opart, out_packed, R, pages_bound,   \
                       max_pages, total_pages, nchunks_max, nq, nkv, scale, fuse, phase, st, pack)
diff --git a/moss-ttsd_amd/csrc/engine.h b/moss-ttsd_amd/csrc/engine.h
--- a/moss-ttsd_amd/csrc/engine.h
+++ b/moss-ttsd_amd/csrc/engine.h
@@ -195,7 +195,7 @@
     int max_real = 0;
     uint64_t seed = 0;
     bool began = false, has_forced = false;
-    struct StepGraph { int B, pages, forced, ch0, scores; hipGraphExec_t exec; };
+    struct StepGraph { int B, pages, forced, ch0, scores, row; hipGraphExec_t exec; };
     std::vector<StepGraph> graphs;
     hipStream_t cap_stream = nullptr;
     bool use_graphs = true;
@@ -206,11 +206,22 @@
     std::vector<char> pack_k_on, pack_v_on;
     int pack_min_work = 512;
     int fuse_qkv_max = 2560;
+    int attn_row = 1;
+    int n_cus = 0;
     int pf_mfma_pages = 0;
     bool prof = false;
     std::vector<std::pair<hipEvent_t, hipEvent_t>> ev[PROF_N];
     int64_t prof_bytes[PROF_N] = {0, 0, 0, 0};
 };
+
+static inline bool attn_row_auto(int rows, int nkv, int pages_bound, int n_cus) {
+    (void)pages_bound;
+    return n_cus > 0 && rows * nkv >= n_cus;
+}
+static inline bool attn_row_shape(const MttsEngine* e, int pages_bound) {
+    if (e->attn_row == 0 || e->f32) return false;
+    return e->attn_row == 2 || attn_row_auto(e->B, e->nkv, pages_bound, e->n_cus);
+}
 
 static inline KvPack layer_pack(MttsEngine* e, int n, int pages_bound) {
     KvPack pk{nullptr, nullptr};
diff --git a/moss-ttsd_amd/csrc/engine.hip b/moss-ttsd_amd/csrc/engine.hip
--- a/moss-ttsd_amd/csrc/engine.hip
+++ b/moss-ttsd_amd/csrc/engine.hip
@@ -179,6 +179,12 @@
     if (const char* g = getenv("MTTS_KV_PACK")) e->kv_pack = atoi(g);
     if (const char* g = getenv("MTTS_KV_PACK_MIN")) e->pack_min_work = atoi(g);
     if (const char* g = getenv("MTTS_PREFILL_MFMA_PAGES")) e->pf_mfma_pages = atoi(g);
+    if (const char* g = getenv("MTTS_ATTN_ROW")) e->attn_row = std::min(std::max(atoi(g), 0), 2);
+    HIPCHK(hipDeviceGetAttribute(&e->n_cus, hipDeviceAttributeMultiprocessorCount, device));
+    if (e->attn_row && attn_row_prepare()) {
+        if (e->attn_row == 2) return fail(MTTS_EINVAL, "attn_row_kernel: the dynamic LDS limit could not be raised");
+        e->attn_row = 0;
+    }
     if (const char* g = getenv("MTTS_SMALL_ROWS")) e->small_rows = std::min(std::max(atoi(g), 0), SMALL_RP);
     e->gemm_depth = gemm_depth_env();
     e->H = c->hidden_size; e->I = c->intermediate_size; e->L = c->num_hidden_layers;
@@ -447,6 +453,17 @@
     uint16_t* vc = (uint16_t*)e->vcache + e->layer_stride * n;
     const QkvFuse fz{e->partial, ks_qkv, e->qkv_rows, (const uint16_t*)l.qn, (const uint16_t*)l.kn, e->rope_cos, e->rope_sin, eps};
     const KvPack pk = layer_pack(e, n, pages_bound);
+    const KvPack* pkp = (sealed && (pk.k || pk.v)) ? &pk : nullptr;
+    if (!prefill && sealed && nphases == 3 && attn_row_shape(e, pages_bound) && attn_row_fits(e->nq / e->nkv, &fz, pkp, pages_bound)) {
+        hipEvent_t ev = nullptr;
+        prof_begin(e, PROF_SCORES, st, &ev);
+        if (const int rc = launch_attn(e->qbuf, kc, vc, e->d_page_table, d_meta, e->scores, e->stats, e->opart, e->attn_p, R, pages_bound,
+                                       e->max_pages, e->total_pages, e->nchunks_max, e->nq, e->nkv, scale, &fz, ATTN_ROW, st, pkp))
+            return fail(MTTS_EINVAL, rc == -2 ? "the whole-row attention kernel does not take this launch" : "attention group size not built");
+        prof_end(e, st, ev);
+        if (e->prof) e->prof_bytes[PROF_SCORES] += 2 * kv_tokens_hint * e->nkv * MTTS_HD * 2;
+        return 0;
+    }
     if (!fused)
         launch_qkv_post(e->partial, ks_qkv, e->qkv_rows, d_meta, l.qn, l.kn, e->rope_cos, e->rope_sin, e->qbuf,
                         kc, vc, e->d_page_table, e->max_pages, e->total_pages, R, e->nq, e->nkv, eps, st);
@@ -455,7 +472,7 @@
         if (i < 2) prof_begin(e, i == 0 ? PROF_SCORES : PROF_PV, st, &ev);
         if (launch_attn(e->qbuf, kc, vc, e->d_page_table, d_meta, e->scores, e->stats, e->opart, e->attn_p, R,
                         pages_bound, e->max_pages, e->total_pages, e->nchunks_max, e->nq, e->nkv, scale,
-                        fused ? &fz : nullptr, (prefill ? prefill_ph : decode_ph)[i], st, (sealed && (pk.k || pk.v)) ? &pk : nullptr))
+                        fused ? &fz : nullptr, (prefill ? prefill_ph : decode_ph)[i], st, pkp))
             return fail(MTTS_EINVAL, "attention group size not built");
         if (i < 2) prof_end(e, st, ev);
     }
@@ -788,9 +805,9 @@
 }
 
 static int step_graph(MttsEngine* e, int pages, hipGraphExec_t* out) {
-    const int forced = e->has_forced ? 1 : 0;
+    const int forced = e->has_forced ? 1 : 0, row = attn_row_shape(e, pages) ? 1 : 0;
     for (auto& g : e->graphs)
-        if (g.B == e->B && g.pages == pages && g.forced == forced && g.ch0 == e->ch0_sampled && g.scores == e->scores_on) {
+        if (g.B == e->B && g.pages == pages && g.forced == forced && g.ch0 == e->ch0_sampled && g.scores == e->scores_on && g.row == row) {
             *out = g.exec;
             return MTTS_OK;
         }
@@ -806,7 +823,7 @@
     hipError_t ie = hipGraphInstantiate(&exec, g, nullptr, nullptr, 0);
     hipGraphDestroy(g);
     HIPCHK(ie);
-    e->graphs.push_back({e->B, pages, forced, e->ch0_sampled, e->scores_on, exec});
+    e->graphs.push_back({e->B, pages, forced, e->ch0_sampled, e->scores_on, row, exec});
     *out = exec;
     return MTTS_OK;
 }
diff --git a/moss-ttsd_amd/csrc/hooks.hip b/moss-ttsd_amd/csrc/hooks.hip
--- a/moss-ttsd_amd/csrc/hooks.hip
+++ b/moss-ttsd_amd/csrc/hooks.hip
@@ -197,6 +197,79 @@
     return MTTS_OK;
 }
 
+int32_t mtts_k_attn_section(const float* dev_slabs, int32_t ksplit, const void* dev_qnw, const void* dev_knw, const void* dev_cos,
+                            const void* dev_sin, float eps, const void* dev_k, const void* dev_v, const int32_t* host_lens,
+                            const int32_t* host_page_table, int32_t R, int32_t Lmax, int32_t nq, int32_t nkv, int32_t sealed,
+                            int32_t path, void* dev_out, void* dev_kcache, void* dev_vcache, void* dev_kpack, void* dev_vpack,
+                            void* stream) {
+    if (!dev_slabs || !dev_qnw || !dev_knw || !dev_cos || !dev_sin || !dev_k || !dev_v || !host_lens || !dev_out || !dev_kcache ||
+        !dev_vcache || R < 1 || R > MTTS_MAXR || Lmax < 1 || nq < 1 || nkv < 1 || nq % nkv || ksplit < 1 || (path != 0 && path != 1))
+        return fail(MTTS_EINVAL, "attn_section: bad argument (1..32 rows, path 0 or 1)");
+    hipStream_t st = S(stream);
+    const int max_pages = (Lmax + MTTS_PAGE - 1) / MTTS_PAGE, total_pages = R * max_pages, nch = (max_pages + ATT_PB - 1) / ATT_PB;
+    const int Npad = (nq + 2 * nkv) * MTTS_HD;
+    std::vector<int32_t> hpt((size_t)R * max_pages);
+    std::vector<char> seen(total_pages, 0);
+    for (size_t i = 0; i < hpt.size(); ++i) {
+        hpt[i] = host_page_table ? host_page_table[i] : (int32_t)i;
+        if (hpt[i] < 0 || hpt[i] >= total_pages || seen[hpt[i]]) return fail(MTTS_EINVAL, "page table must be a permutation of 0..%d", total_pages - 1);
+        seen[hpt[i]] = 1;
+    }
+    std::vector<RowMeta> hm(MTTS_MAXR, RowMeta{-1, 0, 0, 0});
+    std::vector<int32_t> cached(R, 0);
+    int pages_bound = 1;
+    for (int r = 0; r < R; ++r) {
+        if (host_lens[r] < 0 || host_lens[r] > Lmax) return fail(MTTS_EINVAL, "row %d: length %d outside 0..%d", r, host_lens[r], Lmax);
+        if (!host_lens[r]) continue;
+        hm[r] = RowMeta{r, host_lens[r] - 1, 1, 0};
+        cached[r] = host_lens[r] - 1;
+        pages_bound = std::max(pages_bound, (host_lens[r] + MTTS_PAGE - 1) / MTTS_PAGE);
+    }
+    pages_bound = std::min(round_up(pages_bound, ATT_PB), max_pages);
+    RowMeta* meta = nullptr; int32_t *pt = nullptr, *lens = nullptr; uint16_t *kc = nullptr, *vc = nullptr, *scores = nullptr, *outp = nullptr;
+    float *stats = nullptr, *opart = nullptr, *slabs = nullptr;
+    uint8_t *kp = nullptr, *vp = nullptr;
+    const size_t cache_n = (size_t)total_pages * nkv * MTTS_PAGE * MTTS_HD, pk_n = (size_t)total_pages * nkv * MTTS_PKU * 64 * 16;
+    DevBufs hb;
+    TRY(hb.get(&meta, MTTS_MAXR)); TRY(hb.get(&pt, hpt.size())); TRY(hb.get(&lens, R));
+    TRY(hb.get(&kc, cache_n)); TRY(hb.get(&vc, cache_n));
+    TRY(hb.get(&scores, (size_t)MTTS_MAXR * nq * max_pages * MTTS_PAGE));
+    TRY(hb.get(&stats, (size_t)MTTS_MAXR * nq * max_pages * 2));
+    TRY(hb.get(&opart, (size_t)MTTS_MAXR * nq * nch * MTTS_HD));
+    TRY(hb.get(&outp, (size_t)MTTS_MAXR * nq * MTTS_HD));
+    TRY(hb.get(&slabs, (size_t)ksplit * MTTS_PFCAP * Npad, false));
+    HIPCHK(hipMemcpyAsync(meta, hm.data(), hm.size() * sizeof(RowMeta), hipMemcpyHostToDevice, st));
+    HIPCHK(hipMemcpyAsync(pt, hpt.data(), hpt.size() * 4, hipMemcpyHostToDevice, st));
+    HIPCHK(hipMemcpyAsync(lens, cached.data(), R * 4, hipMemcpyHostToDevice, st));
+    for (int k = 0; k < ksplit; ++k)
+        HIPCHK(hipMemcpyAsync(slabs + (size_t)k * MTTS_PFCAP * Npad, dev_slabs + (size_t)k * R * Npad, (size_t)R * Npad * 4, hipMemcpyDeviceToDevice, st));
+    launch_pack_kv_pages(dev_k, dev_v, kc, vc, pt, lens, R, Lmax, nkv, max_pages, total_pages, st);
+    KvPack pk{nullptr, nullptr};
+    if (sealed) {
+        TRY(hb.get(&kp, pk_n)); TRY(hb.get(&vp, pk_n));
+        launch_kv_seal_all(kc, vc, kp, vp, total_pages, nkv, 1, nullptr, st);
+        pk = KvPack{kp, vp};
+    }
+    const QkvFuse fz{slabs, ksplit, Npad, (const uint16_t*)dev_qnw, (const uint16_t*)dev_knw, (const uint16_t*)dev_cos, (const uint16_t*)dev_sin, eps};
+    const float scale = 1.0f / sqrtf((float)MTTS_HD);
+    if (path == 1) {
+        if (attn_row_prepare()) return fail(MTTS_EINVAL, "attn_row_kernel: the dynamic LDS limit could not be raised");
+        if (!attn_row_fits(nq / nkv, &fz, sealed ? &pk : nullptr, pages_bound)) return fail(MTTS_EINVAL, "attn_section: the whole-row kernel does not take this shape");
+    }
+    if (const int rc = launch_attn(nullptr, kc, vc, pt, meta, scores, stats, opart, outp, MTTS_MAXR, pages_bound, max_pages, total_pages, nch,
+                                   nq, nkv, scale, &fz, path == 1 ? ATTN_ROW : ATTN_ALL, st, sealed ? &pk : nullptr))
+        return fail(MTTS_EINVAL, rc == -2 ? "attn_section: the whole-row kernel does not take this shape" : "attention group size not built (1, 2, 4)");
+    HIPCHK(hipGetLastError());
+    HIPCHK(hipMemcpyAsync(dev_out, outp, (size_t)MTTS_MAXR * nq * MTTS_HD * 2, hipMemcpyDeviceToDevice, st));
+    HIPCHK(hipMemcpyAsync(dev_kcache, kc, cache_n * 2, hipMemcpyDeviceToDevice, st));
+    HIPCHK(hipMemcpyAsync(dev_vcache, vc, cache_n * 2, hipMemcpyDeviceToDevice, st));
+    if (sealed && dev_kpack) HIPCHK(hipMemcpyAsync(dev_kpack, kp, pk_n, hipMemcpyDeviceToDevice, st));
+    if (sealed && dev_vpack) HIPCHK(hipMemcpyAsync(dev_vpack, vp, pk_n, hipMemcpyDeviceToDevice, st));
+    HIPCHK(hipStreamSynchronize(st));
+    return MTTS_OK;
+}
+int64_t mtts_debug_attn_row_launches(void) { return (int64_t)mtts_attn_row_launches(); }
+
 int32_t mtts_k_kv_seal(const void* dev_pages, int32_t npages, void* dev_sealed, int32_t as_k, void* stream) {
     if (!dev_pages || !dev_sealed || npages < 1) return fail(MTTS_EINVAL, "kv_seal: bad argument");
     launch_kv_seal_pages(dev_pages, dev_sealed, npages, as_k, S(stream));
@@ -252,7 +325,7 @@
 }
 
 int32_t mtts_k_attn_bench(MttsEngine* e, int32_t phase, int32_t iters, float* avg_ms, int64_t* bytes_per_launch) {
-    if (!e || !e->began || (phase != ATTN_SCORES && phase != ATTN_PV) || iters < 1 || !avg_ms) return fail(MTTS_EINVAL, "attn_bench: bad argument");
+    if (!e || !e->began || phase < ATTN_ALL || phase > ATTN_ROW || iters < 1 || !avg_ms) return fail(MTTS_EINVAL, "attn_bench: bad argument");
     if (e->f32) return fail(MTTS_EINVAL, "measurement hook of the bf16 engine");
     HIPCHK(hipSetDevice(e->device));
     HIPCHK(hipDeviceSynchronize());
@@ -260,6 +333,15 @@
     const int R = round_up(e->B, 32);
     const int len_bound = e->max_real + e->steps_issued + 1;
     const int pages_bound = (len_bound + MTTS_PAGE - 1) / MTTS_PAGE;
+    if (phase == ATTN_ROW) {
+        if (attn_row_prepare()) return fail(MTTS_EINVAL, "attn_row_kernel: the dynamic LDS limit could not be raised");
+        const QkvFuse f0{e->partial, e->p_qkv.ksplit, e->qkv_rows, nullptr, nullptr, nullptr, nullptr, 0.f};
+        for (int n = 0; n < e->L; ++n) {
+            const KvPack pk = layer_pack(e, n, pages_bound);
+            if (!attn_row_fits(e->nq / e->nkv, &f0, (pk.k || pk.v) ? &pk : nullptr, pages_bound))
+                return fail(MTTS_EINVAL, "attn_bench: the whole-row kernel does not take this shape");
+        }
+    }
     hipEvent_t e0, e1;
     hipEventCreate(&e0); hipEventCreate(&e1);
     auto run = [&](int n) {
@@ -271,7 +353,7 @@
                              (const uint16_t*)e->layers[layer].kn, e->rope_cos, e->rope_sin, e->cfg.rms_norm_eps};
             const KvPack pk = layer_pack(e, layer, pages_bound);
             launch_attn(e->qbuf, kc, vc, e->d_page_table, e->d_meta, e->scores, e->stats, e->opart, e->attn_p, R, pages_bound,
-                        e->max_pages, e->total_pages, e->nchunks_max, e->nq, e->nkv, scale, e->B * pages_bound <= e->fuse_qkv_max ? &fz : nullptr, (AttnPhase)phase, nullptr,
+                        e->max_pages, e->total_pages, e->nchunks_max, e->nq, e->nkv, scale, (phase == ATTN_ROW || e->B * pages_bound <= e->fuse_qkv_max) ? &fz : nullptr, (AttnPhase)phase, nullptr,
                         (pk.k || pk.v) ? &pk : nullptr);
         }
     };
@@ -288,7 +370,7 @@
         HIPCHK(hipMemcpy(m.data(), e->d_meta, m.size() * sizeof(RowMeta), hipMemcpyDeviceToHost));
         int64_t tok = 0;
         for (int b = 0; b < R; ++b) if (m[b].seq >= 0) tok += m[b].pos + 1;
-        *bytes_per_launch = tok * e->nkv * MTTS_HD * 2;
+        *bytes_per_launch = phase == ATTN_COMBINE ? 0 : tok * e->nkv * MTTS_HD * 2 * ((phase == ATTN_ALL || phase == ATTN_ROW) ? 2 : 1);
     }
     hipEventDestroy(e0); hipEventDestroy(e1);
     return MTTS_OK;
diff --git a/moss-ttsd_amd/csrc/launch.h b/moss-ttsd_amd/csrc/launch.h
--- a/moss-ttsd_amd/csrc/launch.h
+++ b/moss-ttsd_amd/csrc/launch.h
@@ -46,11 +46,16 @@
 void launch_unpack_rows(const void* packed, void* out, int R, int K, hipStream_t st);
 
 enum AttnPhase { ATTN_ALL = 0, ATTN_SCORES = 1, ATTN_PV = 2, ATTN_COMBINE = 3,
+                 ATTN_ROW = 4,
                  ATTN_PF_SCORES = 11, ATTN_PF_PV = 12, ATTN_PF_COMBINE = 13 };
 int launch_attn(const void* qbuf, void* kcache, void* vcache, const int32_t* page_table,
                 const RowMeta* meta, void* scores, float* stats, float* opart, void* out_packed, int R,
                 int pages_bound, int max_pages, int total_pages, int nchunks_max, int nq, int nkv, float scale,
                 const QkvFuse* fuse, AttnPhase phase, hipStream_t st, const KvPack* pack = nullptr);
+bool attn_row_fits(int G, const QkvFuse* fuse, const KvPack* pack, int pages_bound);
+int attn_row_prepare();
+int attn_row_lds_limit();
+long long mtts_attn_row_launches();
 void launch_kv_seal_rows(const void* kcache, const void* vcache, void* kpack, void* vpack, const int32_t* page_table,
                          const RowMeta* meta, int R, int max_pages, int total_pages, int nkv, int L, unsigned long long* cnt, hipStream_t st);
 void launch_kv_seal_all(const void* kcache, const void* vcache, void* kpack, void* vpack, int total_pages, int nkv, int L,
diff --git a/moss-ttsd_amd/mtts/capi.py b/moss-ttsd_amd/mtts/capi.py
--- a/moss-ttsd_amd/mtts/capi.py
+++ b/moss-ttsd_amd/mtts/capi.py
@@ -89,6 +89,9 @@
     "mtts_k_gemm_bf16": (C.c_int32, [C.c_void_p, C.c_void_p, C.c_void_p, C.c_int32, C.c_int32, C.c_int32,
                                      C.c_int32, C.c_void_p]),
     "mtts_debug_gemm_depth_launches": (C.c_int64, []),
+    "mtts_debug_attn_row_launches": (C.c_int64, []),
+    "mtts_k_attn_section": (C.c_int32, [C.c_void_p, C.c_int32] + [C.c_void_p] * 4 + [C.c_float] + [C.c_void_p] * 4 +
+                            [C.c_int32] * 6 + [C.c_void_p] * 6),
     "mtts_k_gemm_swiglu_bf16": (C.c_int32, [C.c_void_p, C.c_void_p, C.c_void_p, C.c_int32, C.c_int32, C.c_int32, C.c_void_p]),
     "mtts_k_rmsnorm": (C.c_int32, [C.c_void_p, C.c_void_p, C.c_void_p, C.c_int32, C.c_int32, C.c_float, C.c_void_p]),
     "mtts_k_rope_kvwrite": (C.c_int32, [C.c_void_p] * 6 + [C.c_int32, C.c_int32, C.c_int32, C.c_float] + [C.c_void_p] * 4),
```

After: 81720 codec_tokens/s, median of 6. +11.8%, better.
